# tychedelia/josefine

Hardware: NVIDIA H100
Metric: Raft-group ticks/sec @ 64Ki groups x 5 replicas (higher is better)
Workload: dtype u64

## Files before the change

josefine_b200/csrc/engine.cu:

```cuda
#include <algorithm>
#include <atomic>
#include <chrono>
#include <cstdarg>
#include <cstdio>
#include <cstdlib>
#include <cstring>
#include <condition_variable>
#include <mutex>
#include <new>
#include <thread>
#include <vector>

#include "raft_device.cuh"
#include "sym_fold.cuh"

using namespace jr;


#ifdef JR_EMU
#ifdef JR_EMU_BREAK_HANDOFF
#define JR_EMU_HANDOFF_ACQUIRE __ATOMIC_RELAXED
#define JR_EMU_HANDOFF_RELEASE __ATOMIC_RELAXED
#else
#define JR_EMU_HANDOFF_ACQUIRE __ATOMIC_ACQUIRE
// ... 1003 lines not shown
      if (last && id == last->id0 + last->count && addr == last->addr && last->count < FS_MAX_RUN &&
          (last->count == 1u || tok == last->tok0 + (unsigned long long)last->count * last->stride)) {
        if (last->count == 1u) last->stride = tok - last->tok0;
        last->count += 1u;
      } else {
        t[n++] = PnRun{id, 1u, addr, tok, 0ull};
        fit();
      }
    } else {
      while (a_e >= a_cnt && a_src <= d.R) {
        const uint32_t from = a_src < d.R ? a_src : r;
        if (a_k >= kept(from)) { ++a_src; a_k = 0; continue; }
        const uint4 h = rec_hdr(from, a_k++);
        if (mine(a_src, h)) { a_id0 = h.z; a_cnt = h.y >> 8; a_e = 0; }
      }
      if (a_e >= a_cnt) break;
      const uint32_t id = a_id0 + a_e++;
      if (id == 0u || skip) continue;
      const uint32_t k = find(id);
      if (k == n) continue;
      uint32_t addr;
      unsigned long long tok;
      take(k, id, addr, tok);
      if (o.count && id == o.id0 + o.count && addr == o.addr && o.count < FS_MAX_RUN &&
          (o.count == 1u || tok == o.tok0 + (unsigned long long)o.count * o.stride)) {
        if (o.count == 1u) o.stride = tok - o.tok0;
        o.count += 1u;
      } else {
        close();
        o = PnRun{id, 1u, addr, tok, 0ull};
      }
    }
  }
  close();
  for (uint32_t k = 0; k < n; ++k) {
    q.pn[(size_t)(2 * k) * plane + i] = make_uint4(t[k].id0, t[k].count, t[k].addr, 0u);
    q.pn[(size_t)(2 * k + 1) * plane + i] = make_uint4((uint32_t)t[k].tok0, (uint32_t)(t[k].tok0 >> 32), (uint32_t)t[k].stride,
                                                       (uint32_t)(t[k].stride >> 32));
  }
  q.pnc[i] = n;
  q.rc[i] = make_uint2(n_runs, n_resp);
  q.rd[i] = drop;
}

__global__ void fsm_copy_kernel(const uint4* __restrict__ src, const FsmHeader* __restrict__ hdr, uint4* __restrict__ dst,
                                FsmHeader* hdr_dst, uint32_t epoch) {
  const size_t n = (size_t)hdr->n_records * 2;
  for (size_t i = (size_t)blockIdx.x * blockDim.x + threadIdx.x; i < n; i += (size_t)gridDim.x * blockDim.x) dst[i] = src[i];
  if (blockIdx.x == 0 && threadIdx.x == 0) {
    FsmHeader h = *hdr;
    h.ready = epoch;
    *hdr_dst = h;
  }
}

__global__ void max_u32_kernel(const uint32_t* v, size_t n, uint32_t* out) {
  uint32_t m = 0;
  for (size_t i = (size_t)blockIdx.x * blockDim.x + threadIdx.x; i < n; i += (size_t)gridDim.x * blockDim.x)
    m = max(m, v[i]);
#ifndef JR_EMU
  for (int o = 16; o > 0; o >>= 1) m = max(m, __shfl_down_sync(0xffffffffu, m, o));
  if ((threadIdx.x & 31) == 0)
#endif
    atomicMax(out, m);
}


extern "C" { static jr_status stream_sums(jr_engine* e, uint64_t v[5]); }
static thread_local char g_err[512] = "";
static void set_err(const char* fmt, ...) {
  va_list ap;
  va_start(ap, fmt);
  vsnprintf(g_err, sizeof g_err, fmt, ap);
  va_end(ap);
}

#define CK(call)                                                                      \
  do {                                                                                \
    cudaError_t _e = (call);                                                          \
    if (_e != cudaSuccess) {                                                          \
      set_err("%s:%d %s: %s", __FILE__, __LINE__, #call, cudaGetErrorString(_e));     \
      return JR_E_CUDA;                                                               \
    }                                                                                 \
  } while (0)

struct jr_engine {
  jr_config cfg;
  Dev d;
  cudaStream_t stream = nullptr;
  cudaStream_t own_stream = nullptr;
  volatile uint32_t* h_scatter = nullptr;
  volatile uint32_t* h_unfolded = nullptr;
  uint32_t ticket_sum = 0;
  int force_sorted = 0;
  uint64_t launches_sorted = 0, launches_total = 0, launches_split = 0;
  uint32_t slots = 0;
  uint32_t sms = 0;
  uint32_t force_parts = 0;
  int cur = 0;
  uint64_t step_index = 0;
  std::vector<void*> allocs;
  unsigned long long* scratch = nullptr;
  jr_msg* inj_msgs = nullptr;
  uint4* inj_targets = nullptr;
  size_t inj_cap = 0;
  static constexpr int NBUF = JR_STAGING_DEPTH;
  jr_proposal* prop[NBUF] = {nullptr, nullptr};
  jr_leader_entry* leaders[NBUF] = {nullptr, nullptr};
  cudaStream_t h2d = nullptr, d2h = nullptr;
  cudaEvent_t prop_ready[NBUF] = {nullptr, nullptr};
  cudaEvent_t prop_free[NBUF] = {nullptr, nullptr};
  cudaEvent_t tab_ready[NBUF] = {nullptr, nullptr};
  cudaEvent_t tab_free[NBUF] = {nullptr, nullptr};
  bool prop_used[NBUF] = {false, false}, tab_used[NBUF] = {false, false};
  jr_proposal* batch[NBUF] = {nullptr, nullptr};
  size_t batch_cap[NBUF] = {0, 0};
  cudaEvent_t batch_ready[NBUF] = {nullptr, nullptr}, batch_free[NBUF] = {nullptr, nullptr};
  bool batch_used[NBUF] = {false, false};
  int batch_i = 0;
  unsigned long long* tokbuf[NBUF] = {nullptr, nullptr};
  size_t tok_cap[NBUF] = {0, 0};
  uint32_t* route = nullptr;
  int tab_pending[NBUF] = {0, 0};
  int tab_npending = 0;
  int prop_i = 0, tab_i = 0;
  void* many_buf = nullptr;
  size_t many_cap = 0;
  void* verify_buf = nullptr;
  size_t verify_cap = 0;
  static constexpr int NSLOT = NBUF + 1;
  unsigned long long* fsm_part = nullptr;
  uint32_t fsm_cap = 0;
  uint4* fsm_stage[NSLOT] = {};
  FsmHeader* fsm_stage_hdr[NSLOT] = {};
  uint4* fsm_host[NSLOT] = {};
  FsmHeader* fsm_host_hdr[NSLOT] = {};
  cudaEvent_t fsm_packed[NSLOT] = {};
  cudaEvent_t fsm_landed[NSLOT] = {};
  size_t fsm_copied[NSLOT] = {};
  size_t fsm_last_records = 0;
  int fsm_copy_by_sm = 0;
  bool fsm_used[NSLOT] = {};
  int fsm_i = 0, fsm_pending[NBUF] = {0, 0}, fsm_npending = 0;
  std::mutex qmu;
  uint32_t fsm_epoch = 0;
  RespPlanes rp = {nullptr, nullptr, nullptr, nullptr, nullptr, nullptr};
  uint32_t resp_cap = 0;
  size_t resp_copied[NSLOT] = {};
  size_t resp_last = 0;
  int resp_b = -1;
  uint8_t* symdone = nullptr;
  uint8_t* symblk = nullptr;
  uint32_t* symrec = nullptr;
  bool auto_trunc = false;
  uint32_t auto_trunc_margin = 0;
  int no_fold = 0;
  int no_parts_hint = 0;
  int sym_one_lane = 0;
  uint64_t launches_folded = 0;
  bool last_launch_folded = false;
};

template <typename T>
static jr_status dalloc(jr_engine* e, T** p, size_t n) {
  void* q = nullptr;
  cudaError_t err = cudaMalloc(&q, n * sizeof(T));
  if (err != cudaSuccess) {
    set_err("cudaMalloc(%zu bytes): %s", n * sizeof(T), cudaGetErrorString(err));
    return err == cudaErrorMemoryAllocation ? JR_E_NOMEM : JR_E_CUDA;
  }
  e->allocs.push_back(q);
  *p = (T*)q;
  return JR_OK;
}

#define DISPATCH_R(R_, CALL)           \
  switch (R_) {                        \
    case 1: { constexpr int RR = 1; CALL; } break; \
    case 2: { constexpr int RR = 2; CALL; } break; \
    case 3: { constexpr int RR = 3; CALL; } break; \
    case 4: { constexpr int RR = 4; CALL; } break; \
    case 5: { constexpr int RR = 5; CALL; } break; \
    case 6: { constexpr int RR = 6; CALL; } break; \
    case 7: { constexpr int RR = 7; CALL; } break; \
    default: { constexpr int RR = 8; CALL; } break; \
  }

template <int R>
static void launch_step_r(jr_engine* e, const StepParams& p, bool sorted, uint32_t grid, size_t smem) {
  auto kfn = sorted ? step_kernel<R, true> : step_kernel<R, false>;
  JR_LAUNCH_SMEM(kfn, grid, 32 * R, smem, e->stream, e->d, p);
}

template <int R>
static cudaError_t step_smem_attr_r(int smem) {
  cudaError_t a = cudaFuncSetAttribute(step_kernel<R, false>, cudaFuncAttributeMaxDynamicSharedMemorySize, smem);
  if (a != cudaSuccess) return a;
  return cudaFuncSetAttribute(step_kernel<R, true>, cudaFuncAttributeMaxDynamicSharedMemorySize, smem);
}

#ifndef JR_EMU
template <int R>
static cudaError_t step_occupancy_r(int* per_sm, int smem) {
  return cudaOccupancyMaxActiveBlocksPerMultiprocessor(per_sm, step_kernel<R, false>, 32 * R, (size_t)smem);
}
#endif

static size_t step_smem_bytes(const Dev& d) {
  return ((size_t)2 * d.Us + d.W) * d.R * 32 * sizeof(uint4) + (size_t)2 * d.R * 32 * sizeof(uint32_t) +
         (size_t)2 * d.R * d.R * 32 * sizeof(uint16_t);
}

static uint32_t choose_parts(const jr_engine* e, const StepParams& p, uint32_t n_blocks) {
  const uint32_t whole = PH_RESET_OUT | PH_DRAIN | PH_TICK;
  if ((p.phases & whole) != whole || p.n_ticks < 2) return 1;
  if (e->force_parts) return std::min<uint32_t>(e->force_parts, p.n_ticks);
  if (!e->slots || n_blocks <= e->slots) return 1;
  uint32_t best = 1;
  double best_rounds = (double)((n_blocks + e->slots - 1) / e->slots);
  for (uint32_t n = 2; n <= 8 && p.n_ticks / n >= 8; n *= 2) {
    const double rounds = (double)(((size_t)n_blocks * n + e->slots - 1) / e->slots) / n;
    if (rounds < best_rounds * 0.97) { best = n; best_rounds = rounds; }
  }
  return best;
}

static jr_status launch_step_once(jr_engine* e, const StepParams& p_in);

static jr_status launch_step(jr_engine* e, const StepParams& p_in) {
  const uint32_t limit = (e->d.flags & JR_F_CAPTURE_FSM) ? std::max(1u, e->d.Fr / 3u) : 0xffffffffu;
  if (p_in.n_ticks <= limit) return launch_step_once(e, p_in);
  StepParams p = p_in;
  for (uint32_t done = 0; done < p_in.n_ticks;) {
    p.n_ticks = std::min(limit, p_in.n_ticks - done);
    p.trunc = (p_in.trunc && done + p.n_ticks == p_in.n_ticks) ? 1u : 0u;
    jr_status st = launch_step_once(e, p);
    if (st != JR_OK) return st;
    done += p.n_ticks;
    p.now += (uint64_t)p.n_ticks * p.dt;
    p.step_index += p.n_ticks;
    p.cur ^= (int)(p.n_ticks & 1u);
    if (p.proposals) p.proposals += (size_t)p.n_ticks * p.prop_stride;
    p.tok_tick += p.n_ticks;
    p.phases = PH_RESET_OUT | PH_DRAIN | (p_in.phases & PH_PROPOSE) | PH_TICK;
  }
  return JR_OK;
}

template <int R>
static void launch_sym_r(jr_engine* e, const StepParams& p) {
  if constexpr (R >= 2) {
    JR_LAUNCH(sym_check_kernel<R>, (e->d.Gp + SYM_CHECK_THREADS - 1) / SYM_CHECK_THREADS, SYM_CHECK_THREADS, e->stream, e->d, p,
              e->symrec);
    if (e->sym_one_lane)
      JR_LAUNCH(sym_kernel<R>, (e->d.Gp + SYM_LANES - 1) / SYM_LANES, SYM_LANES, e->stream, e->d, p, e->symdone, e->symrec);
    else
      JR_LAUNCH_SMEM(sym2_kernel<R>, (e->d.Gp + SYM2_GROUPS - 1) / SYM2_GROUPS, 2 * SYM2_GROUPS,
                     (size_t)SYM2_UNITS * SYM2_GROUPS * sizeof(uint4), e->stream, e->d, p, e->symdone, e->symblk, e->symrec);
  }
}

static bool fold_eligible(const jr_engine* e, const StepParams& p) {
  const Dev& d = e->d;
  const uint32_t whole = PH_RESET_OUT | PH_DRAIN | PH_TICK;
  if (e->no_fold || (d.flags & (JR_F_STREAM_DIGEST | JR_F_SLED_COMMIT_KEY_STRICT | JR_F_NO_SYMMETRIC_FOLD))) return false;
  if (d.R < 2 || d.U < d.R + 7 || d.resident != 0xffu || p.dt == 0) return false;
  if ((p.phases & ~(uint32_t)PH_PROPOSE) != whole || p.n_ticks < 2) return false;
  if (p.proposals && p.prop_stride != d.G) return false;
  return true;
}

static jr_status launch_step_once(jr_engine* e, const StepParams& p_in) {
  const uint32_t n_blocks = e->d.Gp / GROUPS_PER_CTA;
  const size_t smem = step_smem_bytes(e->d);
  StepParams p = p_in;
  p.epoch = (uint32_t)(e->launches_total + 1) * 8u;
  if (fold_eligible(e, p)) {
    DISPATCH_R(e->cfg.n_replicas, (launch_sym_r<RR>(e, p)));
    CK(cudaGetLastError());
    if (e->sym_one_lane) {
      JR_LAUNCH(sym_blocks_kernel, (n_blocks + 127) / 128, 128, e->stream, e->symdone, e->symblk, n_blocks);
      CK(cudaGetLastError());
    }
    p.symdone = e->symdone;
    p.symblk = e->symblk;
    e->launches_folded += 1;
  }
  e->last_launch_folded = p.symdone != nullptr;
  p.n_parts = choose_parts(e, p, n_blocks);
  if (p.symdone && !e->sym_one_lane && e->h_unfolded && (*e->h_unfolded == 0 || p.epoch - *e->h_unfolded > 2u * 8u) && !e->force_parts)
    if (!e->no_parts_hint) p.n_parts = 1;
  p.part_ticks = (p.n_ticks + p.n_parts - 1) / p.n_parts;
  p.n_parts = (p.n_ticks + p.part_ticks - 1) / p.part_ticks;
  p.n_blocks = n_blocks;
  const uint32_t grid = n_blocks * p.n_parts;
  const bool sorted = e->force_sorted > 0 || (e->force_sorted == 0 && e->h_scatter && *e->h_scatter != 0 && p.epoch - *e->h_scatter <= 2u * 8u);
  p.ticket_base = e->ticket_sum;
  if (p.n_parts > 1) e->ticket_sum += grid;
  DISPATCH_R(e->cfg.n_replicas, (launch_step_r<RR>(e, p, sorted, grid, smem)));
  CK(cudaGetLastError());
  if (p.trunc) {
    JR_LAUNCH(truncate_kernel, (e->d.Gp + 127) / 128, 128, e->stream, e->d, p.trunc_margin,
              (const uint8_t*)((p.symdone && !e->sym_one_lane) ? p.symdone : nullptr));
    CK(cudaGetLastError());
  }
  e->launches_sorted += sorted ? 1 : 0;
  e->launches_split += p.n_parts > 1 ? 1 : 0;
  e->launches_total += 1;
  return JR_OK;
}

extern "C" {

#ifdef JR_EMU
int jr_is_emulation(void) { return 1; }
#endif

const char* jr_last_error(void) { return g_err; }

void jr_config_default(jr_config* cfg, uint32_t n_groups, uint32_t n_replicas) {
  if (!cfg) return;
  memset(cfg, 0, sizeof *cfg);
  cfg->abi_version = JR_ABI_VERSION;
  cfg->n_groups = n_groups;
  cfg->n_replicas = n_replicas;
  cfg->election_min_ms = 500;
  cfg->election_max_ms = 1000;
  cfg->heartbeat_ms = 100;
  cfg->chain_capacity = 4096;
  cfg->mailbox_units = 64;
  cfg->fsm_units = 64;
}

uint32_t jr_election_timeout(uint64_t seed, uint64_t group, uint32_t node, uint32_t draw, uint32_t mn,
                             uint32_t mx) {
  return election_timeout_draw(seed, group, node, draw, mn, mx);
}

jr_status jr_engine_create(const jr_config* cfg, jr_engine** out) {
  if (!cfg || !out) return JR_E_INVAL;
  if (cfg->abi_version != JR_ABI_VERSION) { set_err("abi_version mismatch"); return JR_E_INVAL; }
  if (cfg->n_replicas < 1 || cfg->n_replicas > JR_MAX_REPLICAS || cfg->n_groups < 1) { set_err("bad G/R"); return JR_E_INVAL; }
  if (cfg->election_max_ms <= cfg->election_min_ms) { set_err("empty election timeout range"); return JR_E_INVAL; }
  if (cfg->heartbeat_ms < 5) { set_err("heartbeat timeout is too low"); return JR_E_INVAL; }
  if (cfg->election_min_ms < 5) { set_err("election timeout is too low"); return JR_E_INVAL; }
  if (cfg->chain_capacity < 2 || cfg->chain_capacity > 0x40000000u) { set_err("chain_capacity out of range"); return JR_E_INVAL; }
  if (cfg->mailbox_units < 8 || cfg->fsm_units < 1) { set_err("mailbox_units >= 8, fsm_units >= 1"); return JR_E_INVAL; }
  if (cfg->fsm_units > (1u << 20) || cfg->fsm_raw_units > (1u << 20) || (cfg->fsm_raw_units && cfg->fsm_raw_units < 32)) {
    set_err("fsm_units <= 2^20, 32 <= fsm_raw_units <= 2^20");
    return JR_E_INVAL;
  }
  if ((cfg->flags & JR_F_CLIENT_RESPONSES) && !(cfg->flags & JR_F_CAPTURE_FSM)) {
    set_err("JR_F_CLIENT_RESPONSES requires JR_F_CAPTURE_FSM");
    return JR_E_INVAL;
  }
  int ndev = 0;
  if (cudaGetDeviceCount(&ndev) != cudaSuccess || ndev == 0) {
    set_err("no CUDA device; this library has no CPU fallback");
    return JR_E_NO_DEVICE;
  }
  if (cfg->device < 0 || cfg->device >= ndev) { set_err("device ordinal %d out of range", cfg->device); return JR_E_INVAL; }
  CK(cudaSetDevice(cfg->device));
  jr_engine* e = new (std::nothrow) jr_engine();
  if (!e) return JR_E_NOMEM;
  e->cfg = *cfg;
  Dev& d = e->d;
  memset(&d, 0, sizeof d);
  d.G = cfg->n_groups;
  d.Gp = (cfg->n_groups + GROUPS_PER_CTA - 1) / GROUPS_PER_CTA * GROUPS_PER_CTA;
  d.R = cfg->n_replicas;
  d.cap = cfg->chain_capacity;
  d.capm = 1;
  while (d.capm < d.cap) d.capm <<= 1;
  d.capm -= 1;
  d.U = cfg->mailbox_units;
  d.F = cfg->fsm_units;
  d.Fr = cfg->fsm_raw_units ? cfg->fsm_raw_units : 192u;
  d.flags = cfg->flags;
  d.emin = cfg->election_min_ms;
  d.emax = cfg->election_max_ms;
  d.hb = cfg->heartbeat_ms;
  d.seed = cfg->seed;
  d.goff = cfg->group_offset;
  d.Us = std::min<uint32_t>(cfg->mailbox_units, 6u);
  d.W = 4;
  d.use_index = getenv("JR_NO_INDEX") ? 0u : 1u;
  d.resident = cfg->resident_mask ? cfg->resident_mask : 0xffu;
  if (const char* ev = getenv("JR_SMEM_UNITS")) d.Us = std::min<uint32_t>(cfg->mailbox_units, (uint32_t)atoi(ev));
  if (const char* ev = getenv("JR_TABLE_CACHE")) { uint32_t w = (uint32_t)atoi(ev); d.W = (w & (w - 1)) ? 8 : w; }
  const size_t plane = (size_t)d.R * d.Gp;
  jr_status st = JR_OK;
#define A(ptr, n) if (st == JR_OK) st = dalloc(e, &(ptr), (n))
  A(d.p0, plane); A(d.p1, plane); A(d.p2, plane); A(d.p3, plane);
  A(d.pr, plane * ((d.R + 3) / 4));
  A(d.mk, plane);
  A(d.qt, plane * JR_CLIENT_QUEUE_CAP);
  A(d.dg, plane); A(d.cn, plane);
  A(d.cnext, plane * ((size_t)d.capm + 1));
  A(d.ctok, plane * ((size_t)d.capm + 1));
  A(d.ob[0], plane * (size_t)d.U); A(d.ob[1], plane * (size_t)d.U);
  A(d.oc[0], plane); A(d.oc[1], plane);
  A(d.fs, plane * (size_t)((d.flags & JR_F_CAPTURE_FSM) ? 2 * (size_t)d.F : 1));
  A(d.fc, plane);
  A(d.fq, plane);
  A(d.fr, plane * (size_t)((d.flags & JR_F_CAPTURE_FSM) ? d.Fr : 1));
  A(d.tb, d.Gp);
  A(e->symdone, d.Gp);
  A(e->symblk, d.Gp / GROUPS_PER_CTA);
  A(e->symrec, (size_t)sym_record_words(d.R) * d.Gp);
  if (d.flags & JR_F_CAPTURE_FSM) {
    const size_t reps = (size_t)cfg->n_groups * cfg->n_replicas;
    const size_t want = cfg->fsm_host_records ? cfg->fsm_host_records
                                              : std::max(3 * reps + 1024, std::min<size_t>(reps * cfg->fsm_units, 1u << 16));
    e->fsm_cap = (uint32_t)std::min<size_t>(want, 0x7fffffffu);
    if (d.flags & JR_F_CLIENT_RESPONSES) {
      e->resp_cap = e->fsm_cap;
      uint4* pn = nullptr;
      A(pn, pn_units(plane));
      e->rp.pn = pn;
      if (pn) {
        e->rp.pnc = reinterpret_cast<uint32_t*>(pn + 2 * (size_t)JR_NOTIFY_RUNS * plane);
        e->rp.rm = pn + 2 * (size_t)JR_NOTIFY_RUNS * plane + (plane + 3) / 4;
      }
      A(e->rp.rs, plane * 2 * (size_t)d.F);
      A(e->rp.rc, plane);
      A(e->rp.rd, plane);
    }
    const size_t n_hdr = e->resp_cap ? 2 : 1;
    A(e->fsm_part, 3 * plane);
    for (int i = 0; i < jr_engine::NSLOT; ++i) {
      A(e->fsm_stage[i], 2 * ((size_t)e->fsm_cap + e->resp_cap));
      A(e->fsm_stage_hdr[i], n_hdr);
    }
  }
  A(e->scratch, 8);
  A(d.scatter, 2);
  A(d.done, d.Gp / GROUPS_PER_CTA);
#ifdef JR_PROFILE
  A(d.prof, 3 * 16 * 2);
#endif
  for (int i = 0; i < jr_engine::NBUF; ++i) { A(e->prop[i], d.G); A(e->leaders[i], d.G); }
  A(e->route, d.G);
#undef A
  if (st != JR_OK) { jr_engine_destroy(e); return st; }
  if (cudaStreamCreateWithFlags(&e->own_stream, cudaStreamNonBlocking) != cudaSuccess) {
    set_err("cudaStreamCreate failed");
    jr_engine_destroy(e);
    return JR_E_CUDA;
  }
  e->stream = e->own_stream;
  {
    bool ok = cudaStreamCreateWithFlags(&e->h2d, cudaStreamNonBlocking) == cudaSuccess &&
              cudaStreamCreateWithFlags(&e->d2h, cudaStreamNonBlocking) == cudaSuccess;
    for (int i = 0; ok && i < jr_engine::NBUF; ++i)
      ok = cudaEventCreateWithFlags(&e->prop_ready[i], cudaEventDisableTiming) == cudaSuccess &&
           cudaEventCreateWithFlags(&e->prop_free[i], cudaEventDisableTiming) == cudaSuccess &&
           cudaEventCreateWithFlags(&e->tab_ready[i], cudaEventDisableTiming) == cudaSuccess &&
           cudaEventCreateWithFlags(&e->tab_free[i], cudaEventDisableTiming) == cudaSuccess &&
           cudaEventCreateWithFlags(&e->batch_ready[i], cudaEventDisableTiming) == cudaSuccess &&
           cudaEventCreateWithFlags(&e->batch_free[i], cudaEventDisableTiming) == cudaSuccess;
    for (int i = 0; ok && i < jr_engine::NSLOT; ++i)
      ok = cudaEventCreateWithFlags(&e->fsm_packed[i], cudaEventDisableTiming) == cudaSuccess &&
           cudaEventCreateWithFlags(&e->fsm_landed[i], cudaEventDisableTiming) == cudaSuccess;
    for (int i = 0; ok && e->fsm_cap && i < jr_engine::NSLOT; ++i)
      ok = cudaHostAlloc((void**)&e->fsm_host[i], ((size_t)e->fsm_cap + e->resp_cap) * sizeof(jr_fsm_record), cudaHostAllocMapped) == cudaSuccess &&
           cudaHostAlloc((void**)&e->fsm_host_hdr[i], (e->resp_cap ? 2 : 1) * sizeof(FsmHeader), cudaHostAllocMapped) == cudaSuccess;
    if (!ok) {
      set_err("copy streams / events could not be created");
      jr_engine_destroy(e);
      return JR_E_CUDA;
    }
  }
  {
    const int smem = (int)step_smem_bytes(d);
    cudaError_t aerr = cudaSuccess;
    DISPATCH_R(d.R, (aerr = step_smem_attr_r<RR>(smem)));
    if (aerr == cudaSuccess) aerr = cudaHostAlloc((void**)&e->h_scatter, sizeof(uint32_t), cudaHostAllocMapped);
    if (aerr == cudaSuccess) *e->h_scatter = 0;
    if (aerr == cudaSuccess) aerr = cudaHostGetDevicePointer((void**)&e->d.hscat, (void*)e->h_scatter, 0);
    if (aerr == cudaSuccess) aerr = cudaHostAlloc((void**)&e->h_unfolded, sizeof(uint32_t), cudaHostAllocMapped);
    if (aerr == cudaSuccess) *e->h_unfolded = 0;
    if (aerr == cudaSuccess) aerr = cudaHostGetDevicePointer((void**)&e->d.hunf, (void*)e->h_unfolded, 0);
    if (const char* ev = getenv("JR_NO_FOLD")) e->no_fold = atoi(ev);
    if (const char* ev = getenv("JR_SYM_ONE_LANE")) e->sym_one_lane = atoi(ev);
    if (const char* ev = getenv("JR_NO_PARTS_HINT")) e->no_parts_hint = atoi(ev);
    if (const char* ev = getenv("JR_FSM_COPY")) e->fsm_copy_by_sm = strcmp(ev, "sm") == 0;
    if (const char* ev = getenv("JR_PARTS")) e->force_parts = (uint32_t)std::min(std::max(atoi(ev), 0), 8);
#ifndef JR_EMU
    if (aerr == cudaSuccess) {
      int per_sm = 0, sms = 0;
      DISPATCH_R(d.R, (aerr = step_occupancy_r<RR>(&per_sm, smem)));
      if (aerr == cudaSuccess) aerr = cudaDeviceGetAttribute(&sms, cudaDevAttrMultiProcessorCount, cfg->device);
      e->slots = (uint32_t)(per_sm * sms);
      e->sms = (uint32_t)sms;
    }
#endif
    if (const char* ev = getenv("JR_STEP_VARIANT")) e->force_sorted = !strcmp(ev, "sorted") ? 1 : (!strcmp(ev, "plain") ? -1 : 0);
    if (aerr != cudaSuccess) {
      set_err("step kernel needs %d bytes of shared memory: %s", smem, cudaGetErrorString(aerr));
      jr_engine_destroy(e);
      return JR_E_CUDA;
    }
  }
  if (jr_engine_reset(e) != JR_OK) {
    jr_engine_destroy(e);
    return JR_E_CUDA;
  }
  *out = e;
  return JR_OK;
}

#ifdef JR_PROFILE
jr_status jr_profile_read(jr_engine* e, unsigned long long* out96) {
  if (!e || !out96) return JR_E_INVAL;
  CK(cudaStreamSynchronize(e->stream));
  CK(cudaMemcpyAsync(out96, e->d.prof, 96 * sizeof(unsigned long long), cudaMemcpyDeviceToHost, e->stream));
  CK(cudaMemsetAsync(e->d.prof, 0, 96 * sizeof(unsigned long long), e->stream));
  CK(cudaStreamSynchronize(e->stream));
  return JR_OK;
}
#endif

jr_status jr_engine_reset(jr_engine* e) {
  if (!e) return JR_E_INVAL;
  CK(cudaSetDevice(e->cfg.device));
  const Dev& d = e->d;
  const size_t plane = (size_t)d.R * d.Gp;
  CK(cudaMemsetAsync(d.cnext, 0xFF, plane * ((size_t)d.capm + 1) * sizeof(uint32_t), e->stream));
  CK(cudaMemsetAsync(d.pr, 0, plane * ((d.R + 3) / 4) * sizeof(uint4), e->stream));
  CK(cudaMemsetAsync(d.qt, 0, plane * JR_CLIENT_QUEUE_CAP * sizeof(uint4), e->stream));
  CK(cudaMemsetAsync(e->route, 0, (size_t)d.G * sizeof(uint32_t), e->stream));
  CK(cudaMemsetAsync(d.done, 0, (size_t)(d.Gp / GROUPS_PER_CTA) * sizeof(uint32_t), e->stream));
  CK(cudaMemsetAsync(d.scatter, 0, 2 * sizeof(uint32_t), e->stream));
  e->ticket_sum = 0;
  if (e->rp.pnc)
    CK(cudaMemsetAsync(e->rp.pnc, 0, ((plane + 3) / 4 + plane) * sizeof(uint4), e->stream));
  e->resp_b = -1;
  JR_LAUNCH(init_kernel, (unsigned)((plane + 255) / 256), 256, e->stream, d);
  CK(cudaGetLastError());
  CK(cudaStreamSynchronize(e->stream));
  e->cur = 0;
  e->step_index = 0;
#ifdef JR_PROFILE
  CK(cudaMemsetAsync(e->d.prof, 0, 96 * sizeof(unsigned long long), e->stream));
#endif
  return JR_OK;
}

void jr_engine_destroy(jr_engine* e) {
  if (!e) return;
  if (getenv("JR_DEBUG_VARIANT"))
    fprintf(stderr, "[jr] engine %p: %llu step launches, %llu role-sorted, %llu split, %llu offered to the fold; %u CTA slots\n",
            (void*)e, (unsigned long long)e->launches_total, (unsigned long long)e->launches_sorted,
            (unsigned long long)e->launches_split, (unsigned long long)e->launches_folded, e->slots);
  cudaSetDevice(e->cfg.device);
  if (e->stream) cudaStreamSynchronize(e->stream);
  for (void* p : e->allocs) cudaFree(p);
  if (e->inj_msgs) cudaFree(e->inj_msgs);
  if (e->inj_targets) cudaFree(e->inj_targets);
  if (e->many_buf) cudaFree(e->many_buf);
  if (e->verify_buf) cudaFree(e->verify_buf);
  if (e->h2d) { cudaStreamSynchronize(e->h2d); cudaStreamDestroy(e->h2d); }
  if (e->d2h) { cudaStreamSynchronize(e->d2h); cudaStreamDestroy(e->d2h); }
  for (int i = 0; i < jr_engine::NBUF; ++i) {
    if (e->prop_ready[i]) cudaEventDestroy(e->prop_ready[i]);
    if (e->prop_free[i]) cudaEventDestroy(e->prop_free[i]);
    if (e->tab_ready[i]) cudaEventDestroy(e->tab_ready[i]);
    if (e->tab_free[i]) cudaEventDestroy(e->tab_free[i]);
    if (e->batch_ready[i]) cudaEventDestroy(e->batch_ready[i]);
    if (e->batch_free[i]) cudaEventDestroy(e->batch_free[i]);
    if (e->batch[i]) cudaFree(e->batch[i]);
    if (e->tokbuf[i]) cudaFree(e->tokbuf[i]);
  }
  for (int i = 0; i < jr_engine::NSLOT; ++i) {
    if (e->fsm_packed[i]) cudaEventDestroy(e->fsm_packed[i]);
    if (e->fsm_landed[i]) cudaEventDestroy(e->fsm_landed[i]);
    if (e->fsm_host[i]) cudaFreeHost(e->fsm_host[i]);
    if (e->fsm_host_hdr[i]) cudaFreeHost(e->fsm_host_hdr[i]);
  }
  if (e->h_scatter) cudaFreeHost((void*)e->h_scatter);
  if (e->h_unfolded) cudaFreeHost((void*)e->h_unfolded);
  if (e->own_stream) cudaStreamDestroy(e->own_stream);
  delete e;
}

jr_status jr_engine_set_stream(jr_engine* e, void* s) {
  if (!e) return JR_E_INVAL;
  CK(cudaStreamSynchronize(e->stream));
  e->stream = s ? (cudaStream_t)s : e->own_stream;
  return JR_OK;
}

jr_status jr_engine_sync(jr_engine* e) {
  if (!e) return JR_E_INVAL;
  CK(cudaStreamSynchronize(e->h2d));
  CK(cudaStreamSynchronize(e->stream));
  CK(cudaStreamSynchronize(e->d2h));
  return JR_OK;
}


static void decode_unit(const uint4& h, uint32_t group, uint32_t sender, const uint4* blocks, size_t stride,
                        std::vector<jr_msg>& out) {
  const uint32_t kind = h.x & 15u, flag = (h.x >> 4) & 1u, aux = (h.x >> 8) & 255u, to = h.x >> 16;
  jr_msg m;
  memset(&m, 0, sizeof m);
  m.group = group;
  m.from_kind = JR_ADDR_PEER;
  m.from_id = sender;
  m.to_kind = to == TO_PEERS ? JR_ADDR_PEERS : (to == TO_CLIENT ? JR_ADDR_CLIENT : JR_ADDR_PEER);
  m.to_id = m.to_kind == JR_ADDR_PEER ? to : 0;
  m.kind = (uint8_t)kind;
  const uint64_t t = (uint64_t)h.y | ((uint64_t)h.z << 32);
  uint32_t copies = 1;
  switch (kind) {
    case JR_CMD_VOTE_REQUEST: m.term = t; m.node_id = sender; m.last_term = t; m.block = h.w; copies = aux; break;
    case JR_CMD_VOTE_RESPONSE: m.term = t; m.node_id = sender; m.flag = flag; break;
    case JR_CMD_APPEND_ENTRIES:
      m.term = t; m.node_id = sender; m.n_blocks = (uint8_t)aux;
      for (uint32_t k = 0; k < aux && k < JR_MAX_AE_BLOCKS; ++k) {
        const uint4& b = blocks[(size_t)k * stride];
        m.blocks[k] = jr_block{b.x, b.y, (uint64_t)b.z | ((uint64_t)b.w << 32)};
      }
      break;
    case JR_CMD_APPEND_RESPONSE: m.node_id = sender; m.term = t; m.block = h.w; m.flag = flag; break;
    case JR_CMD_HEARTBEAT: m.term = t; m.block = h.w; m.node_id = sender; break;
    case JR_CMD_HEARTBEAT_RESPONSE: m.block = h.w; m.flag = flag; break;
    case JR_CMD_CLIENT_REQUEST: m.token = t; m.client_kind = (uint8_t)(h.w >> 16); m.client_id = h.w & 0xffffu; break;
    case JR_CMD_CLIENT_RESPONSE: m.token = t; break;
    default: break;
  }
  for (uint32_t k = 0; k < copies; ++k) out.push_back(m);
}

static jr_status device_max(jr_engine* e, const uint32_t* v, size_t n, uint32_t* out) {
  uint32_t* s = reinterpret_cast<uint32_t*>(e->scratch);
  CK(cudaMemsetAsync(s, 0, sizeof(uint32_t), e->stream));
  JR_LAUNCH(max_u32_kernel, 64, 256, e->stream, v, n, s);
  CK(cudaGetLastError());
  CK(cudaMemcpyAsync(out, s, sizeof(uint32_t), cudaMemcpyDeviceToHost, e->stream));
  CK(cudaStreamSynchronize(e->stream));
  return JR_OK;
}

static jr_status capture_messages(jr_engine* e, int buf, std::vector<jr_msg>& out) {
  const Dev& d = e->d;
  const size_t plane = (size_t)d.R * d.Gp;
  uint32_t mx = 0;
  jr_status st = device_max(e, d.oc[buf], plane, &mx);
  if (st != JR_OK) return st;
  std::vector<uint32_t> cnt(plane);
  CK(cudaMemcpyAsync(cnt.data(), d.oc[buf], plane * sizeof(uint32_t), cudaMemcpyDeviceToHost, e->stream));
  std::vector<uint4> units((size_t)mx * plane);
  if (mx) CK(cudaMemcpyAsync(units.data(), d.ob[buf], units.size() * sizeof(uint4), cudaMemcpyDeviceToHost, e->stream));
  CK(cudaStreamSynchronize(e->stream));
  for (uint32_t g = 0; g < d.G; ++g)
    for (uint32_t r = 0; r < d.R; ++r) {
      const size_t i = (size_t)r * d.Gp + g;
      for (uint32_t u = 0; u < cnt[i];) {
        const uint4& h = units[(size_t)u * plane + i];
        const uint32_t kind = h.x & 15u, aux = (h.x >> 8) & 255u;
        const bool ae = kind == JR_CMD_APPEND_ENTRIES, ref = ae && ((h.x >> 4) & 1u);
        const uint32_t span = 1 + ((ae && !ref) ? aux : 0u);
        const uint32_t first = ref ? h.w : u + 1;
        decode_unit(h, g, r + 1, (ae && aux) ? &units[(size_t)first * plane + i] : nullptr, plane, out);
        u += span;
      }
    }
  return JR_OK;
}


static jr_status fsm_records_enqueue(jr_engine* e) {
  const Dev& d = e->d;
  if (!(d.flags & JR_F_CAPTURE_FSM)) { set_err("engine created without JR_F_CAPTURE_FSM"); return JR_E_INVAL; }
  size_t last_records, last_resp;
  {
    std::lock_guard<std::mutex> l(e->qmu);
    if (e->fsm_npending == jr_engine::NBUF) { set_err("%d batches outstanding: call jr_fsm_records_wait first", jr_engine::NBUF); return JR_E_INVAL; }
    last_records = e->fsm_last_records;
    last_resp = e->resp_last;
  }
  const int b = e->fsm_i;
  e->fsm_i = (b + 1) % jr_engine::NSLOT;
  const size_t plane = (size_t)d.R * d.Gp;
  if (e->fsm_used[b]) CK(cudaStreamWaitEvent(e->stream, e->fsm_landed[b], 0));
  const uint32_t epoch = ++e->fsm_epoch;
#ifdef JR_EMU
  const uint32_t T = 1, Ts = 1;
#else
  const uint32_t T = 256, Ts = SCAN_THREADS;
#endif
  const uint32_t n_ctas = (uint32_t)((plane + T - 1) / T);
  JR_LAUNCH(fsm_count_kernel, n_ctas, T, e->stream, d, d.fc, nullptr, e->fsm_part, n_ctas);
  CK(cudaGetLastError());
  JR_LAUNCH(fsm_scan_kernel, 1, Ts, e->stream, e->fsm_part, n_ctas, e->fsm_stage_hdr[b], e->fsm_cap, false);
  CK(cudaGetLastError());
  if (e->resp_cap) {
    JR_LAUNCH(fsm_respond_kernel, n_ctas, T, e->stream, d, e->rp, e->fsm_stage_hdr[b], e->fsm_cap);
    CK(cudaGetLastError());
  }
  JR_LAUNCH(fsm_pack_kernel, n_ctas, T, e->stream, d, d.fs, d.fc, e->fsm_part, e->fsm_stage_hdr[b], e->fsm_stage[b], e->fsm_cap,
            false);
  CK(cudaGetLastError());
  uint4* const resp_stage = e->fsm_stage[b] + 2 * (size_t)e->fsm_cap;
  if (e->resp_cap) {
    JR_LAUNCH(fsm_count_kernel, n_ctas, T, e->stream, d, e->rp.rc, e->rp.rd, e->fsm_part, n_ctas);
    CK(cudaGetLastError());
    JR_LAUNCH(fsm_scan_kernel, 1, Ts, e->stream, e->fsm_part, n_ctas, e->fsm_stage_hdr[b] + 1, e->resp_cap, true);
    CK(cudaGetLastError());
    JR_LAUNCH(fsm_pack_kernel, n_ctas, T, e->stream, d, e->rp.rs, e->rp.rc, e->fsm_part, e->fsm_stage_hdr[b] + 1, resp_stage,
              e->resp_cap, true);
    CK(cudaGetLastError());
  }
  CK(cudaEventRecord(e->fsm_packed[b], e->stream));
  CK(cudaStreamWaitEvent(e->d2h, e->fsm_packed[b], 0));
  if (e->fsm_copy_by_sm) {
    JR_LAUNCH(fsm_copy_kernel, 32, 256, e->d2h, e->fsm_stage[b], e->fsm_stage_hdr[b], e->fsm_host[b], e->fsm_host_hdr[b], epoch);
    CK(cudaGetLastError());
    e->fsm_copied[b] = e->fsm_cap;
    if (e->resp_cap) {
      JR_LAUNCH(fsm_copy_kernel, 32, 256, e->d2h, resp_stage, e->fsm_stage_hdr[b] + 1, e->fsm_host[b] + 2 * (size_t)e->fsm_cap,
                e->fsm_host_hdr[b] + 1, epoch);
      CK(cudaGetLastError());
      e->resp_copied[b] = e->resp_cap;
    }
  } else {
    const size_t guess = std::min<size_t>(e->fsm_cap, std::max<size_t>(last_records + last_records / 8 + 1024, 16384));
    if (guess) CK(cudaMemcpyAsync(e->fsm_host[b], e->fsm_stage[b], guess * sizeof(jr_fsm_record), cudaMemcpyDeviceToHost, e->d2h));
    CK(cudaMemcpyAsync(e->fsm_host_hdr[b], e->fsm_stage_hdr[b], sizeof(FsmHeader), cudaMemcpyDeviceToHost, e->d2h));
    e->fsm_copied[b] = guess;
    if (e->resp_cap) {
      const size_t rg = std::min<size_t>(e->resp_cap, std::max<size_t>(last_resp + last_resp / 8 + 1024, 16384));
      CK(cudaMemcpyAsync(e->fsm_host[b] + 2 * (size_t)e->fsm_cap, resp_stage, rg * sizeof(jr_fsm_record), cudaMemcpyDeviceToHost, e->d2h));
      CK(cudaMemcpyAsync(e->fsm_host_hdr[b] + 1, e->fsm_stage_hdr[b] + 1, sizeof(FsmHeader), cudaMemcpyDeviceToHost, e->d2h));
      e->resp_copied[b] = rg;
    }
  }
  CK(cudaEventRecord(e->fsm_landed[b], e->d2h));
  e->fsm_used[b] = true;
  std::lock_guard<std::mutex> l(e->qmu);
  e->fsm_pending[e->fsm_npending++] = b;
  return JR_OK;
}

static jr_status fsm_records_take(jr_engine* e, const jr_fsm_record** recs, jr_fsm_batch* batch) {
  int b;
  {
    std::lock_guard<std::mutex> l(e->qmu);
    if (e->fsm_npending == 0) { set_err("no batch outstanding"); return JR_E_INVAL; }
    b = e->fsm_pending[0];
    for (int k = 0; k + 1 < jr_engine::NBUF; ++k) e->fsm_pending[k] = e->fsm_pending[k + 1];
    --e->fsm_npending;
  }
  CK(cudaEventSynchronize(e->fsm_landed[b]));
  const FsmHeader& h = *e->fsm_host_hdr[b];
  if (h.n_records > e->fsm_copied[b]) {
    const size_t have = e->fsm_copied[b];
    CK(cudaMemcpyAsync(reinterpret_cast<jr_fsm_record*>(e->fsm_host[b]) + have, reinterpret_cast<const jr_fsm_record*>(e->fsm_stage[b]) + have,
                       ((size_t)h.n_records - have) * sizeof(jr_fsm_record), cudaMemcpyDeviceToHost, e->d2h));
    CK(cudaEventRecord(e->fsm_landed[b], e->d2h));
    CK(cudaEventSynchronize(e->fsm_landed[b]));
    e->fsm_copied[b] = h.n_records;
  }
  size_t n_resp = 0;
  if (e->resp_cap) {
    const FsmHeader& hr = e->fsm_host_hdr[b][1];
    n_resp = hr.n_records;
    if (hr.n_records > e->resp_copied[b]) {
      const size_t have = e->resp_copied[b];
      jr_fsm_record* dst = reinterpret_cast<jr_fsm_record*>(e->fsm_host[b] + 2 * (size_t)e->fsm_cap);
      const jr_fsm_record* src = reinterpret_cast<const jr_fsm_record*>(e->fsm_stage[b] + 2 * (size_t)e->fsm_cap);
      CK(cudaMemcpyAsync(dst + have, src + have, ((size_t)hr.n_records - have) * sizeof(jr_fsm_record), cudaMemcpyDeviceToHost, e->d2h));
      CK(cudaEventRecord(e->fsm_landed[b], e->d2h));
      CK(cudaEventSynchronize(e->fsm_landed[b]));
      e->resp_copied[b] = hr.n_records;
    }
  }
  {
    std::lock_guard<std::mutex> l(e->qmu);
    e->fsm_last_records = h.n_records;
    if (e->resp_cap) { e->resp_last = n_resp; e->resp_b = b; }
  }
  if (recs) *recs = reinterpret_cast<const jr_fsm_record*>(e->fsm_host[b]);
  if (batch) {
    memset(batch, 0, sizeof *batch);
    batch->n_records = h.n_records;
    batch->n_dropped = h.n_dropped;
    batch->n_instructions = h.n_instructions;
    for (uint32_t r = 0; r <= JR_MAX_REPLICAS; ++r) batch->node_offset[r] = r <= e->d.R ? h.node_offset[r] : h.node_offset[e->d.R];
  }
  if (h.n_dropped) {
    set_err("%llu Instruction records were dropped (raise fsm_units / fsm_host_records, or drain more often)",
            (unsigned long long)h.n_dropped);
    return JR_E_CAPACITY;
  }
  return JR_OK;
}

static jr_status capture_fsm(jr_engine* e, std::vector<jr_fsm_instr>& out) {
  const Dev& d = e->d;
  if (!(d.flags & JR_F_CAPTURE_FSM)) return JR_OK;
  if (e->fsm_npending) { set_err("jr_fsm_records_async batches are outstanding"); return JR_E_INVAL; }
  jr_status st = fsm_records_enqueue(e);
  if (st != JR_OK) return st;
  const jr_fsm_record* recs = nullptr;
  jr_fsm_batch batch;
  const jr_status took = fsm_records_take(e, &recs, &batch);
  if (took != JR_OK) return took;
  size_t n = 0;
  st = jr_fsm_expand(recs, batch.n_records, d.G, d.R, nullptr, 0, &n);
  if (st != JR_OK && st != JR_E_CAPACITY) return st;
  out.resize(n);
  if (n && (st = jr_fsm_expand(recs, batch.n_records, d.G, d.R, out.data(), n, &n)) != JR_OK) return st;
  return took;
}


jr_status jr_step(jr_engine* e, jr_step_args* a) {
  if (!e || !a) return JR_E_INVAL;
  CK(cudaSetDevice(e->cfg.device));
  const Dev& d = e->d;
  const uint32_t R = d.R, G = d.G;
  if (a->n_synth > 8) { set_err("n_synth <= 8"); return JR_E_INVAL; }
  if ((a->out_msgs && !(d.flags & JR_F_CAPTURE_MESSAGES)) || (a->out_fsm && !(d.flags & JR_F_CAPTURE_FSM))) {
    set_err("output buffer given but capture flag not set at create");
    return JR_E_INVAL;
  }
  std::vector<jr_msg> sorted;
  std::vector<uint4> targets;
  if (a->n_inject) {
    if (!a->inject) return JR_E_INVAL;
    std::vector<uint32_t> order(a->n_inject);
    for (size_t i = 0; i < a->n_inject; ++i) {
      const jr_msg& m = a->inject[i];
      if (m.group >= G || m.to_kind != JR_ADDR_PEER) { set_err("inject[%zu]: bad group / to_kind", i); return JR_E_INVAL; }
      if (m.to_id < 1 || m.to_id > R) return JR_E_UNKNOWN_NODE;
      if (m.node_id > JR_MAX_NODE_ID || m.from_id > JR_MAX_NODE_ID || m.client_id > JR_MAX_NODE_ID) return JR_E_INVAL;
      if (m.kind == JR_CMD_VOTE_RESPONSE && (m.node_id < 1 || m.node_id > 32)) return JR_E_UNKNOWN_NODE;
      if (m.n_blocks > JR_MAX_AE_BLOCKS) return JR_E_INVAL;
      if (m.block >= 0xffffffffull) { set_err("inject[%zu]: block id >= 2^32-1 (D4)", i); return JR_E_INVAL; }
      for (unsigned k = 0; k < m.n_blocks; ++k)
        if (m.blocks[k].id >= 0xffffffffull || m.blocks[k].next >= 0xffffffffull) return JR_E_INVAL;
      order[i] = (uint32_t)i;
    }
    std::stable_sort(order.begin(), order.end(), [&](uint32_t x, uint32_t y) {
      const jr_msg &p = a->inject[x], &q = a->inject[y];
      return p.group != q.group ? p.group < q.group : p.to_id < q.to_id;
    });
    sorted.reserve(a->n_inject);
    for (uint32_t idx : order) {
      const jr_msg& m = a->inject[idx];
      if (targets.empty() || targets.back().x != m.group || targets.back().y != m.to_id - 1)
        targets.push_back(make_uint4(m.group, m.to_id - 1, (uint32_t)sorted.size(), 0));
      targets.back().w++;
      sorted.push_back(m);
    }
  }
  if (a->proposals && !(a->flags & JR_STEP_TRUSTED_PROPOSALS))
    for (uint32_t g = 0; g < G; ++g)
      if (a->proposals[g].node > R) return JR_E_UNKNOWN_NODE;

  StepParams p;
  p.now = a->now_ms;
  p.step_index = e->step_index;
  p.n_synth = (a->flags & JR_STEP_SYNTH_PROPOSALS) ? a->n_synth : 0;
  p.cur = e->cur;
  p.n_ticks = 1;
  p.dt = 0;
  p.prop_stride = 0;
  p.proposals = nullptr;
  int staged = -1;
  if (a->proposals) {
    const int b = e->prop_i;
    e->prop_i = (b + 1) % jr_engine::NBUF;
    if (e->prop_used[b]) CK(cudaStreamWaitEvent(e->h2d, e->prop_free[b], 0));
    CK(cudaMemcpyAsync(e->prop[b], a->proposals, (size_t)G * sizeof(jr_proposal), cudaMemcpyHostToDevice, e->h2d));
    CK(cudaEventRecord(e->prop_ready[b], e->h2d));
    CK(cudaStreamWaitEvent(e->stream, e->prop_ready[b], 0));
    p.proposals = e->prop[b];
    staged = b;
  }
  if (e->rp.rm) {
    const size_t plane = (size_t)R * d.Gp;
    JR_LAUNCH(restart_marks_rebase_kernel, (unsigned)((plane + 255) / 256), 256, e->stream, d, e->rp.rm);
    CK(cudaGetLastError());
  }
  const uint32_t ph_first = PH_RESET_OUT | PH_RESET_FSM | ((a->flags & JR_STEP_DELIVER) ? PH_DRAIN : 0u);
  const uint32_t ph_last = ((p.proposals || p.n_synth) ? PH_PROPOSE : 0u) | ((a->flags & JR_STEP_TICK) ? PH_TICK : 0u);
  jr_status st;
  if (targets.empty()) {
    p.phases = ph_first | ph_last;
    if ((st = launch_step(e, p)) != JR_OK) return st;
  } else {
    if (sorted.size() > e->inj_cap) {
      if (e->inj_msgs) cudaFree(e->inj_msgs);
      if (e->inj_targets) cudaFree(e->inj_targets);
      e->inj_msgs = nullptr; e->inj_targets = nullptr;
      e->inj_cap = std::max<size_t>(sorted.size() * 2, 64);
      CK(cudaMalloc(&e->inj_msgs, e->inj_cap * sizeof(jr_msg)));
      CK(cudaMalloc(&e->inj_targets, e->inj_cap * sizeof(uint4)));
    }
    CK(cudaMemcpyAsync(e->inj_msgs, sorted.data(), sorted.size() * sizeof(jr_msg), cudaMemcpyHostToDevice, e->stream));
    CK(cudaMemcpyAsync(e->inj_targets, targets.data(), targets.size() * sizeof(uint4), cudaMemcpyHostToDevice, e->stream));
    p.phases = ph_first;
    if ((st = launch_step(e, p)) != JR_OK) return st;
    const uint32_t nt = (uint32_t)targets.size();
    DISPATCH_R(R, (JR_LAUNCH(inject_kernel<RR>, (nt + 63) / 64, 64, e->stream, e->d, p, e->inj_msgs, e->inj_targets, nt)));
    CK(cudaGetLastError());
    if (ph_last) {
      p.phases = ph_last;
      if ((st = launch_step(e, p)) != JR_OK) return st;
    }
    CK(cudaStreamSynchronize(e->stream));
  }
  if (staged >= 0) {
    CK(cudaEventRecord(e->prop_free[staged], e->stream));
    e->prop_used[staged] = true;
    CK(cudaEventSynchronize(e->prop_ready[staged]));
  }
  const int written = e->cur;
  e->cur ^= 1;
  e->step_index++;

  a->n_msgs = 0;
  a->n_fsm = 0;
  bool ovf = false;
  if (a->out_msgs) {
    std::vector<jr_msg> msgs;
    if ((st = capture_messages(e, written, msgs)) != JR_OK) return st;
    a->n_msgs = msgs.size();
    memcpy(a->out_msgs, msgs.data(), std::min(msgs.size(), a->cap_msgs) * sizeof(jr_msg));
    ovf |= msgs.size() > a->cap_msgs;
  }
  if (a->out_fsm) {
    std::vector<jr_fsm_instr> fsm;
    st = capture_fsm(e, fsm);
    if (st != JR_OK && st != JR_E_CAPACITY) return st;
    a->n_fsm = fsm.size();
    memcpy(a->out_fsm, fsm.data(), std::min(fsm.size(), a->cap_fsm) * sizeof(jr_fsm_instr));
    ovf |= fsm.size() > a->cap_fsm || st == JR_E_CAPACITY;
  }
  if (a->flags & JR_STEP_REPORT_FAULTS) {
    uint64_t v[5];
    if ((st = stream_sums(e, v)) != JR_OK) return st;
    a->n_faulted = v[4];
  }
  return ovf ? JR_E_CAPACITY : JR_OK;
}

jr_status jr_run(jr_engine* e, uint64_t now0, uint32_t dt, uint32_t n_steps, uint32_t n_synth) {
  if (!e) return JR_E_INVAL;
  if (n_synth > 8) { set_err("n_synth <= 8"); return JR_E_INVAL; }
  CK(cudaSetDevice(e->cfg.device));
  if (n_steps == 0) return JR_OK;
  StepParams p;
  p.now = now0;
  p.step_index = e->step_index;
  p.n_synth = n_synth;
  p.n_ticks = n_steps;
  p.dt = dt;
  p.cur = e->cur;
  p.proposals = nullptr;
  p.prop_stride = 0;
  p.phases = PH_RESET_OUT | PH_DRAIN | (n_synth ? PH_PROPOSE : 0u) | PH_TICK;
  p.trunc = e->auto_trunc ? 1u : 0u;
  p.trunc_margin = e->auto_trunc_margin;
  jr_status st = launch_step(e, p);
  if (st != JR_OK) return st;
  e->cur ^= (int)(n_steps & 1u);
  e->step_index += n_steps;
  return JR_OK;
}

static jr_status batch_reserve(jr_engine* e, int b, size_t n) {
  if (e->batch_used[b]) CK(cudaStreamWaitEvent(e->h2d, e->batch_free[b], 0));
  if (n > e->batch_cap[b]) {
    if (e->batch_used[b]) CK(cudaEventSynchronize(e->batch_free[b]));
    if (e->batch[b]) cudaFree(e->batch[b]);
    e->batch[b] = nullptr;
    e->batch_cap[b] = 0;
    CK(cudaMalloc(&e->batch[b], n * sizeof(jr_proposal)));
    e->batch_cap[b] = n;
  }
  return JR_OK;
}

static jr_status batch_launch(jr_engine* e, int b, uint64_t now0, uint32_t dt, uint32_t n_steps) {
  StepParams p;
  p.now = now0;
  p.step_index = e->step_index;
  p.n_synth = 0;
  p.n_ticks = n_steps;
  p.dt = dt;
  p.cur = e->cur;
  p.proposals = e->batch[b];
  p.prop_stride = e->d.G;
  p.phases = PH_RESET_OUT | PH_DRAIN | PH_PROPOSE | PH_TICK;
  p.trunc = e->auto_trunc ? 1u : 0u;
  p.trunc_margin = e->auto_trunc_margin;
  jr_status st = launch_step(e, p);
  if (st != JR_OK) return st;
  CK(cudaEventRecord(e->batch_free[b], e->stream));
  e->batch_used[b] = true;
  e->cur ^= (int)(n_steps & 1u);
  e->step_index += n_steps;
  return JR_OK;
}

jr_status jr_run_proposals(jr_engine* e, uint64_t now0, uint32_t dt, uint32_t n_steps, const jr_proposal* proposals,
                           uint32_t flags) {
  if (!e || !proposals) return JR_E_INVAL;
  if (n_steps == 0) return JR_OK;
  CK(cudaSetDevice(e->cfg.device));
  const uint32_t G = e->d.G, R = e->d.R;
  const size_t n = (size_t)n_steps * G;
  if (!(flags & JR_STEP_TRUSTED_PROPOSALS))
    for (size_t i = 0; i < n; ++i)
      if (proposals[i].node > R) return JR_E_UNKNOWN_NODE;
  const int b = e->batch_i;
  e->batch_i = (b + 1) % jr_engine::NBUF;
  jr_status st = batch_reserve(e, b, n);
  if (st != JR_OK) return st;
  CK(cudaMemcpyAsync(e->batch[b], proposals, n * sizeof(jr_proposal), cudaMemcpyHostToDevice, e->h2d));
  CK(cudaEventRecord(e->batch_ready[b], e->h2d));
  CK(cudaStreamWaitEvent(e->stream, e->batch_ready[b], 0));
  return batch_launch(e, b, now0, dt, n_steps);
}

jr_status jr_run_tokens(jr_engine* e, uint64_t now0, uint32_t dt, uint32_t n_steps, const uint64_t* tokens) {
  if (!e || !tokens) return JR_E_INVAL;
  if (n_steps == 0) return JR_OK;
  CK(cudaSetDevice(e->cfg.device));
  const uint32_t G = e->d.G;
  const size_t n = (size_t)n_steps * G;
  const int b = e->batch_i;
  e->batch_i = (b + 1) % jr_engine::NBUF;
  jr_status st = batch_reserve(e, b, n);
  if (st != JR_OK) return st;
  if (n > e->tok_cap[b]) {
    if (e->batch_used[b]) CK(cudaEventSynchronize(e->batch_free[b]));
    if (e->tokbuf[b]) cudaFree(e->tokbuf[b]);
    e->tokbuf[b] = nullptr;
    e->tok_cap[b] = 0;
    CK(cudaMalloc(&e->tokbuf[b], n * sizeof(unsigned long long)));
    e->tok_cap[b] = n;
  }
  CK(cudaMemcpyAsync(e->tokbuf[b], tokens, n * sizeof(unsigned long long), cudaMemcpyHostToDevice, e->h2d));
  CK(cudaEventRecord(e->batch_ready[b], e->h2d));
  CK(cudaStreamWaitEvent(e->stream, e->batch_ready[b], 0));
  const unsigned blocks = (unsigned)std::min<size_t>((n + 255) / 256, (size_t)std::max(e->sms, 1u) * 16);
  JR_LAUNCH(route_tokens_kernel, blocks, 256, e->stream, e->tokbuf[b], e->route, e->batch[b], G, n);
  CK(cudaGetLastError());
  return batch_launch(e, b, now0, dt, n_steps);
}

jr_status jr_run_token_runs(jr_engine* e, uint64_t now0, uint32_t dt, uint32_t n_steps, const jr_token_run* runs) {
  if (!e || !runs) return JR_E_INVAL;
  if (n_steps == 0) return JR_OK;
  CK(cudaSetDevice(e->cfg.device));
  const uint32_t G = e->d.G;
  const int b = e->batch_i;
  e->batch_i = (b + 1) % jr_engine::NBUF;
  jr_status st = batch_reserve(e, b, G);
  if (st != JR_OK) return st;
  CK(cudaMemcpyAsync(e->batch[b], runs, (size_t)G * sizeof(jr_token_run), cudaMemcpyHostToDevice, e->h2d));
  CK(cudaEventRecord(e->batch_ready[b], e->h2d));
  CK(cudaStreamWaitEvent(e->stream, e->batch_ready[b], 0));
  StepParams p;
  p.now = now0;
  p.step_index = e->step_index;
  p.n_synth = 0;
  p.n_ticks = n_steps;
  p.dt = dt;
  p.cur = e->cur;
  p.proposals = nullptr;
  p.prop_stride = 0;
  p.tok_runs = reinterpret_cast<const uint4*>(e->batch[b]);
  p.tok_route = e->route;
  p.tok_tick = 0;
  p.phases = PH_RESET_OUT | PH_DRAIN | PH_PROPOSE | PH_TICK;
  p.trunc = e->auto_trunc ? 1u : 0u;
  p.trunc_margin = e->auto_trunc_margin;
  st = launch_step(e, p);
  if (st != JR_OK) return st;
  CK(cudaEventRecord(e->batch_free[b], e->stream));
  e->batch_used[b] = true;
  e->cur ^= (int)(n_steps & 1u);
  e->step_index += n_steps;
  return JR_OK;
}

jr_status jr_drain_fsm(jr_engine* e, jr_fsm_instr* out, size_t cap, size_t* n) {
  if (!e || !n) return JR_E_INVAL;
  CK(cudaSetDevice(e->cfg.device));
  if (!(e->d.flags & JR_F_CAPTURE_FSM)) { *n = 0; return JR_OK; }
  std::vector<jr_fsm_instr> fsm;
  jr_status st = capture_fsm(e, fsm);
  if (st != JR_OK && st != JR_E_CAPACITY) return st;
  *n = fsm.size();
  if (out) memcpy(out, fsm.data(), std::min(fsm.size(), cap) * sizeof(jr_fsm_instr));
  return ((out && fsm.size() > cap) || st == JR_E_CAPACITY) ? JR_E_CAPACITY : JR_OK;
}

jr_status jr_fsm_fold(const jr_fsm_record* recs, size_t n, uint32_t G, uint32_t R, uint32_t* applied_hi, uint64_t* totals) {
  if ((!recs && n) || !applied_hi || !totals || R < 1 || R > JR_MAX_REPLICAS) return JR_E_INVAL;
  uint64_t na = 0, nn = 0;
  for (size_t i = 0; i < n; ++i) {
    const jr_fsm_record& rc = recs[i];
    const uint32_t kind = JR_FSMR_KIND(rc.hdr), node = JR_FSMR_NODE(rc.hdr), count = JR_FSMR_COUNT(rc.hdr);
    if (rc.group >= G || node > R) return JR_E_INVAL;
    if (kind == JR_FSMR_APPLY) {
      if (rc.addr) {
        if (rc.addr >> R) return JR_E_INVAL;
        for (uint32_t n = 0; n < R; ++n)
          if ((rc.addr >> n) & 1u) {
            uint32_t& hi = applied_hi[(size_t)n * G + rc.group];
            hi = std::max(hi, rc.id0 + count - 1);
            na += count;
          }
      } else {
        uint32_t& hi = applied_hi[(size_t)(node - 1) * G + rc.group];
        hi = std::max(hi, rc.id0 + count - 1);
        na += count;
      }
    } else if (kind == JR_FSMR_NOTIFY) {
      nn += count;
    }
  }
  totals[0] += na;
  totals[1] += nn;
  totals[2] += n;
  return JR_OK;
}

namespace {
struct FoldJob {
  const jr_fsm_record* recs = nullptr;
  size_t n = 0;
  uint32_t G = 0, R = 0, parts = 0;
  uint32_t* applied = nullptr;
  size_t sec[JR_MAX_REPLICAS + 1];
  uint64_t na[64], nn[64];
  int bad[64];
};
inline uint64_t rec_key(const jr_fsm_record& rc) { return ((uint64_t)JR_FSMR_NODE(rc.hdr) << 32) | rc.group; }
size_t lower_bound_key(const jr_fsm_record* recs, size_t lo, size_t hi, uint64_t key) {
  while (lo < hi) {
    const size_t mid = lo + (hi - lo) / 2;
    if (rec_key(recs[mid]) < key) lo = mid + 1;
    else hi = mid;
  }
  return lo;
}
void fold_slice(FoldJob& j, uint32_t t) {
  const uint32_t g_lo = (uint32_t)((uint64_t)j.G * t / j.parts), g_hi = (uint32_t)((uint64_t)j.G * (t + 1) / j.parts);
  uint64_t na = 0, nn = 0;
  for (uint32_t node = 1; node <= j.R; ++node) {
    const size_t lo = lower_bound_key(j.recs, j.sec[node - 1], j.sec[node], ((uint64_t)node << 32) | g_lo);
    const size_t hi = lower_bound_key(j.recs, lo, j.sec[node], ((uint64_t)node << 32) | g_hi);
    for (size_t i = lo; i < hi; ++i) {
      const jr_fsm_record& rc = j.recs[i];
      const uint32_t kind = JR_FSMR_KIND(rc.hdr), count = JR_FSMR_COUNT(rc.hdr);
      if (kind == JR_FSMR_APPLY) {
        if (rc.addr) {
          if (rc.addr >> j.R) { j.bad[t] = 1; return; }
          for (uint32_t k = 0; k < j.R; ++k)
            if ((rc.addr >> k) & 1u) {
              uint32_t& hi_w = j.applied[(size_t)k * j.G + rc.group];
              hi_w = std::max(hi_w, rc.id0 + count - 1);
              na += count;
            }
        } else {
          uint32_t& hi_w = j.applied[(size_t)(node - 1) * j.G + rc.group];
          hi_w = std::max(hi_w, rc.id0 + count - 1);
          na += count;
        }
      } else if (kind == JR_FSMR_NOTIFY) {
        nn += count;
      }
    }
  }
  j.na[t] = na;
  j.nn[t] = nn;
}
class FoldPool {
  static constexpr long long SPIN_NS = 2'000'000;
 public:
  static FoldPool& get() { static FoldPool* p = new FoldPool(); return *p; }
  void run(FoldJob& j) {
    {
      std::lock_guard<std::mutex> l(m_);
      while (n_workers_ + 1 < j.parts) {
        const uint32_t k = n_workers_++;
        std::thread th([this, k] { loop(k); });
        th.detach();
      }
      job_ = &j;
      left_.store(j.parts - 1, std::memory_order_relaxed);
      state_.store(((state_.load(std::memory_order_relaxed) >> 8) + 1) << 8 | j.parts, std::memory_order_release);
    }
    if (sleepers_.load(std::memory_order_acquire)) cv_.notify_all();
    fold_slice(j, 0);
    const auto t0 = std::chrono::steady_clock::now();
    while (left_.load(std::memory_order_acquire) != 0) {
      if (std::chrono::steady_clock::now() - t0 > std::chrono::nanoseconds(SPIN_NS)) {
        std::unique_lock<std::mutex> l(m_);
        done_.wait(l, [this] { return left_.load(std::memory_order_acquire) == 0; });
        break;
      }
      cpu_relax();
    }
  }
 private:
  static void cpu_relax() {
#if defined(__x86_64__) || defined(__i386__)
    __builtin_ia32_pause();
#endif
  }
  void loop(uint32_t k) {
    uint64_t seen = 0;
    for (;;) {
      uint64_t st = state_.load(std::memory_order_acquire);
      const auto t0 = std::chrono::steady_clock::now();
      while ((st >> 8) == seen) {
        if (std::chrono::steady_clock::now() - t0 > std::chrono::nanoseconds(SPIN_NS)) {
          std::unique_lock<std::mutex> l(m_);
          sleepers_.fetch_add(1, std::memory_order_acq_rel);
          cv_.wait(l, [&] { return (state_.load(std::memory_order_acquire) >> 8) != seen; });
          sleepers_.fetch_sub(1, std::memory_order_acq_rel);
        } else {
          cpu_relax();
        }
        st = state_.load(std::memory_order_acquire);
      }
      seen = st >> 8;
      if (k + 1 >= (uint32_t)(st & 255u)) continue;
      fold_slice(*job_, k + 1);
      if (left_.fetch_sub(1, std::memory_order_acq_rel) == 1) {
        std::lock_guard<std::mutex> l(m_);
        done_.notify_all();
      }
    }
  }
  std::mutex m_;
  std::condition_variable cv_, done_;
  uint32_t n_workers_ = 0;
  FoldJob* job_ = nullptr;
  std::atomic<uint32_t> left_{0}, sleepers_{0};
  std::atomic<uint64_t> state_{0};
};
}

jr_status jr_fsm_fold_mt(const jr_fsm_record* recs, size_t n, uint32_t G, uint32_t R, uint32_t* applied_hi, uint64_t* totals,
                         uint32_t n_threads) {
  if (n_threads <= 1 || n < 4096) return jr_fsm_fold(recs, n, G, R, applied_hi, totals);
  if ((!recs && n) || !applied_hi || !totals || R < 1 || R > JR_MAX_REPLICAS) return JR_E_INVAL;
  FoldJob j;
  j.recs = recs; j.n = n; j.G = G; j.R = R; j.applied = applied_hi;
  j.parts = std::min<uint32_t>(n_threads, 64);
  j.sec[0] = 0;
  for (uint32_t node = 1; node <= R; ++node) j.sec[node] = lower_bound_key(recs, j.sec[node - 1], n, (uint64_t)(node + 1) << 32);
  bool sorted = j.sec[R] == n && recs[n - 1].group < G;
  for (size_t probe = 1; sorted && probe < 64; ++probe) {
    const size_t i = n * probe / 64;
    sorted = i == 0 || rec_key(recs[i - 1]) <= rec_key(recs[i]);
  }
  if (!sorted) return jr_fsm_fold(recs, n, G, R, applied_hi, totals);
  static std::mutex* one_at_a_time = new std::mutex();
  std::lock_guard<std::mutex> guard(*one_at_a_time);
  for (uint32_t t = 0; t < j.parts; ++t) { j.na[t] = j.nn[t] = 0; j.bad[t] = 0; }
  FoldPool::get().run(j);
  for (uint32_t t = 0; t < j.parts; ++t) {
    if (j.bad[t]) return JR_E_INVAL;
    totals[0] += j.na[t];
    totals[1] += j.nn[t];
  }
  totals[2] += n;
  return JR_OK;
}

jr_status jr_fsm_records_async(jr_engine* e) {
  if (!e) return JR_E_INVAL;
  CK(cudaSetDevice(e->cfg.device));
  return fsm_records_enqueue(e);
}

jr_status jr_fsm_records_wait(jr_engine* e, const jr_fsm_record** records, jr_fsm_batch* batch) {
  if (!e) return JR_E_INVAL;
  CK(cudaSetDevice(e->cfg.device));
  return fsm_records_take(e, records, batch);
}

jr_status jr_fsm_responses(jr_engine* e, const jr_fsm_record** responses, jr_fsm_batch* batch) {
  if (!e) return JR_E_INVAL;
  if (!e->resp_cap) { set_err("engine created without JR_F_CLIENT_RESPONSES"); return JR_E_INVAL; }
  int b;
  { std::lock_guard<std::mutex> l(e->qmu); b = e->resp_b; }
  if (b < 0) { set_err("no batch has been taken yet"); return JR_E_INVAL; }
  const FsmHeader& h = e->fsm_host_hdr[b][1];
  if (responses) *responses = reinterpret_cast<const jr_fsm_record*>(e->fsm_host[b] + 2 * (size_t)e->fsm_cap);
  if (batch) {
    memset(batch, 0, sizeof *batch);
    batch->n_records = h.n_records;
    batch->n_dropped = h.n_dropped;
    batch->n_instructions = h.n_instructions;
    for (uint32_t r = 0; r <= JR_MAX_REPLICAS; ++r) batch->node_offset[r] = r <= e->d.R ? h.node_offset[r] : h.node_offset[e->d.R];
  }
  if (h.n_dropped) {
    set_err("%llu notifications / responses were dropped (JR_NOTIFY_RUNS, fsm_units or lost records)", (unsigned long long)h.n_dropped);
    return JR_E_CAPACITY;
  }
  return JR_OK;
}

jr_status jr_fsm_expand(const jr_fsm_record* recs, size_t n_records, uint32_t G, uint32_t R, jr_fsm_instr* out, size_t cap,
                        size_t* n_out) {
  if (!n_out || (!recs && n_records) || R < 1 || R > JR_MAX_REPLICAS || G < 1) return JR_E_INVAL;
  const size_t nb = (size_t)G * R;
  std::vector<uint32_t> start(nb + 1, 0u);
  auto masked = [&](const jr_fsm_record& rc) { return JR_FSMR_KIND(rc.hdr) == JR_FSMR_APPLY && rc.addr != 0; };
  for (size_t i = 0; i < n_records; ++i) {
    const uint32_t node = JR_FSMR_NODE(recs[i].hdr);
    if (recs[i].group >= G || node > R || JR_FSMR_KIND(recs[i].hdr) > JR_FSMR_PATTERN) return JR_E_INVAL;
    if (masked(recs[i])) {
      if (recs[i].addr >> R) return JR_E_INVAL;
      for (uint32_t n = 0; n < R; ++n)
        if ((recs[i].addr >> n) & 1u) ++start[(size_t)recs[i].group * R + n + 1];
    } else {
      ++start[(size_t)recs[i].group * R + (node - 1) + 1];
    }
  }
  for (size_t b = 0; b < nb; ++b) start[b + 1] += start[b];
  std::vector<uint32_t> order(start[nb]), fill(start.begin(), start.end() - 1);
  for (int pass = 0; pass < 2; ++pass)
    for (size_t i = 0; i < n_records; ++i) {
      if (masked(recs[i]) != (pass == 0)) continue;
      if (pass == 0) {
        for (uint32_t n = 0; n < R; ++n)
          if ((recs[i].addr >> n) & 1u) order[fill[(size_t)recs[i].group * R + n]++] = (uint32_t)i;
      } else {
        order[fill[(size_t)recs[i].group * R + (JR_FSMR_NODE(recs[i].hdr) - 1)]++] = (uint32_t)i;
      }
    }
  size_t k = 0;
  std::vector<uint64_t> is_notify;
  for (size_t b = 0; b < nb; ++b) {
    const uint32_t lo = start[b], hi = start[b + 1];
    if (lo == hi) continue;
    const uint32_t g = (uint32_t)(b / R), node = (uint32_t)(b % R) + 1;
    size_t n_apply = 0, n_note = 0;
    for (uint32_t j = lo; j < hi; ++j) {
      const jr_fsm_record& rc = recs[order[j]];
      if (JR_FSMR_KIND(rc.hdr) == JR_FSMR_APPLY) n_apply += JR_FSMR_COUNT(rc.hdr);
      else if (JR_FSMR_KIND(rc.hdr) == JR_FSMR_NOTIFY) n_note += JR_FSMR_COUNT(rc.hdr);
    }
    const size_t total = n_apply + n_note;
    is_notify.assign((total + 63) / 64, 0ull);
    size_t marked = 0;
    for (uint32_t j = lo; j < hi; ++j) {
      const jr_fsm_record& rc = recs[order[j]];
      if (JR_FSMR_KIND(rc.hdr) != JR_FSMR_PATTERN) continue;
      const uint32_t nbits = JR_FSMR_COUNT(rc.hdr);
      if (nbits > 160) return JR_E_INVAL;
      for (uint32_t bit = 0; bit < nbits; ++bit)
        if ((bit < 64 ? rc.tok0 >> bit : bit < 128 ? rc.stride >> (bit - 64) : (uint64_t)rc.addr >> (bit - 128)) & 1ull) {
          const size_t pos = (size_t)rc.id0 + bit;
          if (pos >= total || ((is_notify[pos >> 6] >> (pos & 63)) & 1ull)) return JR_E_INVAL;
          is_notify[pos >> 6] |= 1ull << (pos & 63);
          ++marked;
        }
    }
    if (marked != n_note) return JR_E_INVAL;
    uint32_t ja = lo, jn = lo, ia = 0, in_ = 0;
    for (size_t pos = 0; pos < total; ++pos) {
      const bool note = (is_notify[pos >> 6] >> (pos & 63)) & 1ull;
      uint32_t& j = note ? jn : ja;
      uint32_t& i = note ? in_ : ia;
      const uint32_t want = note ? JR_FSMR_NOTIFY : JR_FSMR_APPLY;
      while (JR_FSMR_KIND(recs[order[j]].hdr) != want || i >= JR_FSMR_COUNT(recs[order[j]].hdr)) { ++j; i = 0; }
      const jr_fsm_record& rc = recs[order[j]];
      if (out && k < cap) {
        jr_fsm_instr f;
        memset(&f, 0, sizeof f);
        f.group = g;
        f.node = node;
        if (note) {
          f.kind = JR_FSM_NOTIFY;
          f.client_kind = (uint8_t)(rc.addr >> 16);
          f.client_id = rc.addr & 0xffffu;
          f.block = jr_block{(uint64_t)(rc.id0 + i), 0, rc.tok0 + (uint64_t)i * rc.stride};
        } else {
          f.kind = JR_FSM_APPLY;
          const uint32_t bid = rc.id0 + i;
          if (JR_FSMR_COUNT(rc.hdr) == 1) f.block = jr_block{bid, (uint32_t)rc.stride, rc.tok0};
          else f.block = jr_block{bid, bid - 1u, rc.tok0 + (uint64_t)i * rc.stride};
        }
        out[k] = f;
      }
      ++k;
      ++i;
    }
  }
  *n_out = k;
  return (out && k > cap) || (!out && k) ? JR_E_CAPACITY : JR_OK;
}


static jr_status scratch_reserve(void** buf, size_t* cap, size_t bytes) {
  if (bytes <= *cap) return JR_OK;
  if (*buf) cudaFree(*buf);
  *buf = nullptr;
  *cap = 0;
  const size_t want = std::max<size_t>(bytes * 2, 4096);
  CK(cudaMalloc(buf, want));
  *cap = want;
  return JR_OK;
}

static jr_status many_reserve(jr_engine* e, size_t bytes) { return scratch_reserve(&e->many_buf, &e->many_cap, bytes); }

jr_status jr_query_many(jr_engine* e, const uint32_t* groups, const uint32_t* nodes, size_t n, jr_replica_state* out) {
  if (!e || !out || !groups || !nodes) return JR_E_INVAL;
  if (n == 0) return JR_OK;
  if (n > 0x7fffffffu) return JR_E_INVAL;
  for (size_t i = 0; i < n; ++i)
    if (groups[i] >= e->d.G || nodes[i] < 1 || nodes[i] > e->d.R) return JR_E_INVAL;
  CK(cudaSetDevice(e->cfg.device));
  const size_t idx = ((n * 2 * sizeof(uint32_t)) + 15) / 16 * 16;
  jr_status st = many_reserve(e, idx + n * sizeof(jr_replica_state));
  if (st != JR_OK) return st;
  uint32_t* dg = (uint32_t*)e->many_buf;
  uint32_t* dn = dg + n;
  jr_replica_state* ds = (jr_replica_state*)((char*)e->many_buf + idx);
  CK(cudaMemcpyAsync(dg, groups, n * sizeof(uint32_t), cudaMemcpyHostToDevice, e->stream));
  CK(cudaMemcpyAsync(dn, nodes, n * sizeof(uint32_t), cudaMemcpyHostToDevice, e->stream));
  JR_LAUNCH(query_kernel, (unsigned)((n + 127) / 128), 128, e->stream, e->d, dg, dn, (uint32_t)n, ds);
  CK(cudaGetLastError());
  CK(cudaMemcpyAsync(out, ds, n * sizeof(jr_replica_state), cudaMemcpyDeviceToHost, e->stream));
  CK(cudaStreamSynchronize(e->stream));
  return JR_OK;
}

jr_status jr_query(jr_engine* e, uint32_t group, uint32_t node, jr_replica_state* out) {
  return jr_query_many(e, &group, &node, 1, out);
}

jr_status jr_chain_read_many(jr_engine* e, const uint32_t* groups, const uint32_t* nodes, const uint64_t* first_id,
                             const uint32_t* count, size_t n, jr_block* out, uint8_t* present) {
  if (!e || !groups || !nodes || !first_id || !count) return JR_E_INVAL;
  if (n == 0) return JR_OK;
  if (n > 0x7fffffffu) return JR_E_INVAL;
  std::vector<uint4> reqs(n);
  size_t total = 0;
  for (size_t i = 0; i < n; ++i) {
    if (groups[i] >= e->d.G || nodes[i] < 1 || nodes[i] > e->d.R) return JR_E_INVAL;
    if (first_id[i] + count[i] > 0xffffffffull) return JR_E_INVAL;
    reqs[i] = make_uint4(groups[i], nodes[i] - 1, (uint32_t)first_id[i], (uint32_t)total);
    total += count[i];
    if (total > 0xffffffffull) return JR_E_INVAL;
  }
  if (total == 0) return JR_OK;
  CK(cudaSetDevice(e->cfg.device));
  const size_t o_cnt = n * sizeof(uint4), o_blk = (o_cnt + n * sizeof(uint32_t) + 15) / 16 * 16;
  const size_t o_pre = o_blk + total * sizeof(jr_block);
  jr_status st = many_reserve(e, o_pre + total);
  if (st != JR_OK) return st;
  char* base = (char*)e->many_buf;
  CK(cudaMemcpyAsync(base, reqs.data(), n * sizeof(uint4), cudaMemcpyHostToDevice, e->stream));
  CK(cudaMemcpyAsync(base + o_cnt, count, n * sizeof(uint32_t), cudaMemcpyHostToDevice, e->stream));
  JR_LAUNCH(chain_read_kernel, (unsigned)n, 128, e->stream, e->d, (const uint4*)base, (const uint32_t*)(base + o_cnt),
            (jr_block*)(base + o_blk), (uint8_t*)(base + o_pre));
  CK(cudaGetLastError());
  if (out) CK(cudaMemcpyAsync(out, base + o_blk, total * sizeof(jr_block), cudaMemcpyDeviceToHost, e->stream));
  if (present) CK(cudaMemcpyAsync(present, base + o_pre, total, cudaMemcpyDeviceToHost, e->stream));
  CK(cudaStreamSynchronize(e->stream));
  return JR_OK;
}

jr_status jr_chain_read(jr_engine* e, uint32_t group, uint32_t node, uint64_t first, uint32_t n, jr_block* out,
                        uint8_t* present) {
  if (n == 0) return (!e || group >= e->d.G || node < 1 || node > e->d.R) ? JR_E_INVAL : JR_OK;
  return jr_chain_read_many(e, &group, &node, &first, &n, 1, out, present);
}

jr_status jr_state_digest(jr_engine* e, uint64_t* out) {
  if (!e || !out) return JR_E_INVAL;
  CK(cudaSetDevice(e->cfg.device));
  const size_t plane = (size_t)e->d.R * e->d.Gp;
  CK(cudaMemsetAsync(e->scratch, 0, 8 * sizeof(unsigned long long), e->stream));
  JR_LAUNCH(state_digest_kernel, (unsigned)((plane + 255) / 256), 256, e->stream, e->d, e->scratch);
  CK(cudaGetLastError());
  CK(cudaMemcpyAsync(out, e->scratch, sizeof(uint64_t), cudaMemcpyDeviceToHost, e->stream));
  CK(cudaStreamSynchronize(e->stream));
  return JR_OK;
}

static jr_status stream_sums(jr_engine* e, uint64_t v[5]) {
  CK(cudaSetDevice(e->cfg.device));
  const size_t plane = (size_t)e->d.R * e->d.Gp;
  CK(cudaMemsetAsync(e->scratch, 0, 8 * sizeof(unsigned long long), e->stream));
  JR_LAUNCH(stream_digest_kernel, (unsigned)((plane + 255) / 256), 256, e->stream, e->d, e->scratch);
  CK(cudaGetLastError());
  CK(cudaMemcpyAsync(v, e->scratch, 5 * sizeof(uint64_t), cudaMemcpyDeviceToHost, e->stream));
  CK(cudaStreamSynchronize(e->stream));
  return JR_OK;
}

jr_status jr_stream_digest(jr_engine* e, uint64_t* md, uint64_t* fd, uint64_t* nm, uint64_t* nf) {
  if (!e) return JR_E_INVAL;
  if (!(e->d.flags & JR_F_STREAM_DIGEST)) { set_err("engine created without JR_F_STREAM_DIGEST"); return JR_E_INVAL; }
  uint64_t v[5];
  jr_status st = stream_sums(e, v);
  if (st != JR_OK) return st;
  if (md) *md = v[0];
  if (fd) *fd = v[1];
  if (nm) *nm = v[2];
  if (nf) *nf = v[3];
  return JR_OK;
}

jr_status jr_fold_count(jr_engine* e, uint64_t* n) {
  if (!e || !n) return JR_E_INVAL;
  *n = 0;
  if (!e->last_launch_folded) return JR_OK;
  CK(cudaSetDevice(e->cfg.device));
  std::vector<uint8_t> h(e->d.Gp);
  CK(cudaMemcpyAsync(h.data(), e->symdone, h.size(), cudaMemcpyDeviceToHost, e->stream));
  CK(cudaStreamSynchronize(e->stream));
  for (uint32_t g = 0; g < e->d.G; ++g) *n += h[g];
  return JR_OK;
}

jr_status jr_fault_count(jr_engine* e, uint64_t* n) {
  if (!e || !n) return JR_E_INVAL;
  uint64_t v[5];
  jr_status st = stream_sums(e, v);
  if (st != JR_OK) return st;
  *n = v[4];
  return JR_OK;
}


jr_status jr_compact(jr_engine* e) {
  if (!e) return JR_E_INVAL;
  CK(cudaSetDevice(e->cfg.device));
  const size_t plane = (size_t)e->d.R * e->d.Gp;
  JR_LAUNCH(compact_kernel, (unsigned)((plane + 127) / 128), 128, e->stream, e->d);
  CK(cudaGetLastError());
  return JR_OK;
}

jr_status jr_truncate(jr_engine* e, uint32_t margin) {
  if (!e) return JR_E_INVAL;
  CK(cudaSetDevice(e->cfg.device));
  JR_LAUNCH(truncate_kernel, (e->d.Gp + 127) / 128, 128, e->stream, e->d, margin, (const uint8_t*)nullptr);
  CK(cudaGetLastError());
  return JR_OK;
}

jr_status jr_host_alloc(size_t bytes, void** out) {
  if (!out || !bytes) return JR_E_INVAL;
  *out = nullptr;
  cudaError_t err = cudaHostAlloc(out, bytes, 0);
  if (err != cudaSuccess) {
    set_err("cudaHostAlloc(%zu bytes): %s", bytes, cudaGetErrorString(err));
    return err == cudaErrorMemoryAllocation ? JR_E_NOMEM : JR_E_CUDA;
  }
  return JR_OK;
}

void jr_host_free(void* p) {
  if (p) cudaFreeHost(p);
}

jr_status jr_set_auto_truncate(jr_engine* e, int enabled, uint32_t margin) {
  if (!e) return JR_E_INVAL;
  e->auto_trunc = enabled != 0;
  e->auto_trunc_margin = margin;
  return JR_OK;
}

jr_status jr_chain_export_many(jr_engine* e, const uint32_t* groups, const uint32_t* nodes, size_t n,
                               jr_persisted_chain* out, jr_block* blocks, size_t cap_blocks, size_t* n_blocks) {
  if (!e || !n_blocks || (n && (!groups || !nodes || !out))) return JR_E_INVAL;
  *n_blocks = 0;
  if (n == 0) return JR_OK;
  if (n > 0x7fffffffu) return JR_E_INVAL;
  std::vector<uint2> targets(n);
  for (size_t k = 0; k < n; ++k) {
    if (groups[k] >= e->d.G || nodes[k] < 1 || nodes[k] > e->d.R) {
      set_err("target %zu: group or node out of range", k);
      return JR_E_INVAL;
    }
    targets[k] = make_uint2(groups[k], nodes[k] - 1);
  }
  CK(cudaSetDevice(e->cfg.device));
  const size_t o_desc = (n * sizeof(uint2) + 15) / 16 * 16;
  jr_status st = many_reserve(e, o_desc + n * sizeof(jr_persisted_chain));
  if (st != JR_OK) return st;
  char* base = (char*)e->many_buf;
  CK(cudaMemcpyAsync(base, targets.data(), n * sizeof(uint2), cudaMemcpyHostToDevice, e->stream));
  JR_LAUNCH(export_count_kernel, (unsigned)((n + 127) / 128), 128, e->stream, e->d, (const uint2*)base, (uint32_t)n,
            (jr_persisted_chain*)(base + o_desc));
  CK(cudaGetLastError());
  CK(cudaMemcpyAsync(out, base + o_desc, n * sizeof(jr_persisted_chain), cudaMemcpyDeviceToHost, e->stream));
  CK(cudaStreamSynchronize(e->stream));
  uint64_t total = 0;
  for (size_t k = 0; k < n; ++k) {
    out[k].first_block = total;
    total += out[k].n_blocks;
  }
  *n_blocks = (size_t)total;
  if (!blocks || cap_blocks < total) return JR_E_CAPACITY;
  if (total == 0) return JR_OK;
  const size_t o_blk = (n * sizeof(jr_persisted_chain) + 15) / 16 * 16;
  if ((st = many_reserve(e, o_blk + total * sizeof(jr_block))) != JR_OK) return st;
  base = (char*)e->many_buf;
  CK(cudaMemcpyAsync(base, out, n * sizeof(jr_persisted_chain), cudaMemcpyHostToDevice, e->stream));
  JR_LAUNCH(export_pack_kernel, (unsigned)((n + 127) / 128), 128, e->stream, e->d, (const jr_persisted_chain*)base,
            (uint32_t)n, (jr_block*)(base + o_blk));
  CK(cudaGetLastError());
  CK(cudaMemcpyAsync(blocks, base + o_blk, total * sizeof(jr_block), cudaMemcpyDeviceToHost, e->stream));
  CK(cudaStreamSynchronize(e->stream));
  return JR_OK;
}

jr_status jr_node_restart_many(jr_engine* e, uint64_t now_ms, const jr_persisted_chain* chains, size_t n,
                               const jr_block* blocks, size_t n_blocks) {
  if (!e || (n && !chains) || (n_blocks && !blocks)) return JR_E_INVAL;
  if (n == 0) return JR_OK;
  if (n > 0x7fffffffu) return JR_E_INVAL;
  const Dev& d = e->d;
  uint32_t g_lo = 0xffffffffu, g_hi = 0;
  for (size_t k = 0; k < n; ++k) {
    if (chains[k].group >= d.G || chains[k].node < 1 || chains[k].node > d.R) {
      set_err("chains[%zu]: group or node out of range", k);
      return JR_E_INVAL;
    }
    g_lo = std::min(g_lo, chains[k].group);
    g_hi = std::max(g_hi, chains[k].group);
  }
  const size_t span = (size_t)g_hi - g_lo + 1;
  std::vector<uint8_t> seen(span * d.R, 0);
  bool host_blocks = false;
  for (size_t k = 0; k < n; ++k) {
    const jr_persisted_chain& c = chains[k];
    uint8_t& s = seen[(size_t)(c.node - 1) * span + (c.group - g_lo)];
    if (s) {
      set_err("chains[%zu]: replica (%u, %u) appears twice", k, c.group, c.node);
      return JR_E_INVAL;
    }
    s = 1;
    if (c.n_blocks == JR_RESTART_IN_PLACE) continue;
    if (c.n_blocks > d.cap || c.first_block > n_blocks || n_blocks - c.first_block < c.n_blocks || c.commit >= 0xffffffffull) {
      set_err("chains[%zu]: slice outside blocks[0, %zu), more than chain_capacity blocks, or commit >= 2^32-1", k, n_blocks);
      return JR_E_INVAL;
    }
    host_blocks |= c.n_blocks > 0;
  }
  CK(cudaSetDevice(e->cfg.device));
  if (host_blocks) {
    std::vector<uint32_t> floor(span);
    CK(cudaMemcpyAsync(floor.data(), d.tb + g_lo, span * sizeof(uint32_t), cudaMemcpyDeviceToHost, e->stream));
    CK(cudaStreamSynchronize(e->stream));
    for (size_t k = 0; k < n; ++k) {
      const jr_persisted_chain& c = chains[k];
      if (c.n_blocks == JR_RESTART_IN_PLACE) continue;
      const uint64_t lo = floor[c.group - g_lo];
      for (uint32_t j = 0; j < c.n_blocks; ++j) {
        const jr_block& b = blocks[c.first_block + j];
        if (b.id < lo || b.id - lo >= d.cap || b.next >= 0xffffffffull || (j && b.id <= blocks[c.first_block + j - 1].id)) {
          set_err("chains[%zu] block %u: id not ascending or outside [floor, floor + chain_capacity), or next >= 2^32-1 (D4, D7)", k, j);
          return JR_E_INVAL;
        }
      }
    }
  }
  const size_t o_blk = (n * sizeof(jr_persisted_chain) + 15) / 16 * 16;
  jr_status st = many_reserve(e, o_blk + n_blocks * sizeof(jr_block));
  if (st != JR_OK) return st;
  char* base = (char*)e->many_buf;
  CK(cudaMemcpyAsync(base, chains, n * sizeof(jr_persisted_chain), cudaMemcpyHostToDevice, e->stream));
  if (n_blocks) CK(cudaMemcpyAsync(base + o_blk, blocks, n_blocks * sizeof(jr_block), cudaMemcpyHostToDevice, e->stream));
  JR_LAUNCH(node_restart_kernel, (unsigned)((n + 127) / 128), 128, e->stream, d, now_ms, (const jr_persisted_chain*)base,
            (uint32_t)n, (const jr_block*)(base + o_blk), e->rp.rm);
  CK(cudaGetLastError());
  CK(cudaStreamSynchronize(e->stream));
  return JR_OK;
}

jr_status jr_node_restart(jr_engine* e, uint32_t group, uint32_t node, uint64_t now_ms, const jr_block* blocks,
                          size_t n_blocks, uint64_t commit, int commit_key) {
  if (!e || group >= e->d.G || node < 1 || node > e->d.R || (n_blocks && !blocks)) return JR_E_INVAL;
  if (n_blocks > e->d.cap || commit >= 0xffffffffull) return JR_E_INVAL;
  std::vector<jr_block> v(blocks, blocks + n_blocks);
  std::stable_sort(v.begin(), v.end(), [](const jr_block& a, const jr_block& b) { return a.id < b.id; });
  size_t m = 0;
  for (size_t k = 0; k < v.size(); ++k)
    if (k + 1 == v.size() || v[k + 1].id != v[k].id) v[m++] = v[k];
  jr_persisted_chain c;
  c.group = group;
  c.node = node;
  c.commit = commit;
  c.first_block = 0;
  c.n_blocks = (uint32_t)m;
  c.commit_key = commit_key ? 1u : 0u;
  return jr_node_restart_many(e, now_ms, &c, 1, v.data(), m);
}

jr_status jr_verify_groups(jr_engine* e, const uint32_t* groups, size_t n_groups, jr_verify_report* report,
                           jr_verify_finding* findings, size_t cap, size_t* n_findings) {
  if (!e || !report || !n_findings || (n_groups && !groups)) return JR_E_INVAL;
  const Dev& d = e->d;
  const size_t n = groups ? n_groups : d.G;
  std::vector<uint32_t> list;
  if (groups) {
    std::vector<uint8_t> seen(d.G, 0);
    for (size_t k = 0; k < n; ++k) {
      if (groups[k] >= d.G || seen[groups[k]]) {
        set_err("groups[%zu]: out of range or named twice", k);
        return JR_E_INVAL;
      }
      seen[groups[k]] = 1;
    }
    list.assign(groups, groups + n);
    std::sort(list.begin(), list.end());
  }
  memset(report, 0, sizeof *report);
  report->groups_checked = n;
  *n_findings = 0;
  if (n == 0) return JR_OK;
  CK(cudaSetDevice(e->cfg.device));
#ifdef JR_EMU
  const uint32_t T = 1;
#else
  const uint32_t T = 256;
#endif
  const size_t reps = (size_t)d.R * n;
  const uint32_t n_ctas = (uint32_t)((n + T - 1) / T);
  const size_t o_part = 16 * sizeof(unsigned long long), o_list = o_part + ((size_t)n_ctas * 8 + 15) / 16 * 16;
  const size_t o_vw = o_list + (n * 4 + 15) / 16 * 16, o_vf = o_vw + reps * sizeof(uint2);
  jr_status st = scratch_reserve(&e->verify_buf, &e->verify_cap, o_vf + reps * sizeof(uint2));
  if (st != JR_OK) return st;
  char* base = (char*)e->verify_buf;
  unsigned long long* rep = (unsigned long long*)base;
  unsigned long long* part = (unsigned long long*)(base + o_part);
  const uint32_t* dlist = groups ? (const uint32_t*)(base + o_list) : nullptr;
  uint2* vw = (uint2*)(base + o_vw);
  uint2* vf = (uint2*)(base + o_vf);
  CK(cudaMemsetAsync(rep, 0, VERIFY_COUNTS * sizeof(unsigned long long), e->stream));
  if (groups) CK(cudaMemcpyAsync(base + o_list, list.data(), n * 4, cudaMemcpyHostToDevice, e->stream));
  const unsigned grid = (unsigned)((reps + 255) / 256);
  JR_LAUNCH(verify_walk_kernel, grid, 256, e->stream, d, dlist, (uint32_t)n, vw);
  CK(cudaGetLastError());
  JR_LAUNCH(verify_judge_kernel, grid, 256, e->stream, d, dlist, (uint32_t)n, (const uint2*)vw, vf, rep);
  CK(cudaGetLastError());
  unsigned long long cnt[VERIFY_COUNTS];
  CK(cudaMemcpyAsync(cnt, rep, sizeof cnt, cudaMemcpyDeviceToHost, e->stream));
  CK(cudaStreamSynchronize(e->stream));
  report->replicas_checked = cnt[0];
  report->replicas_skipped = cnt[1];
  report->below_floor = cnt[2];
  report->commit_absent = cnt[3];
  report->chain_broken = cnt[4];
  report->diverged = cnt[5];
  report->leader_conflicts = cnt[6];
  const size_t total = (size_t)(cnt[2] + cnt[3] + cnt[4] + cnt[5] + cnt[6]);
  *n_findings = total;
  if (total == 0) return JR_OK;
  if (!findings || cap < total) return JR_E_CAPACITY;
  if ((st = many_reserve(e, total * sizeof(jr_verify_finding))) != JR_OK) return st;
  jr_verify_finding* out = (jr_verify_finding*)e->many_buf;
  JR_LAUNCH(verify_count_kernel, n_ctas, T, e->stream, d, (uint32_t)n, (const uint2*)vf, part);
  CK(cudaGetLastError());
  JR_LAUNCH(verify_scan_kernel, 1, 1, e->stream, part, n_ctas);
  CK(cudaGetLastError());
  JR_LAUNCH(verify_pack_kernel, n_ctas, T, e->stream, d, dlist, (uint32_t)n, (const uint2*)vf, (const unsigned long long*)part, out);
  CK(cudaGetLastError());
  CK(cudaMemcpyAsync(findings, out, total * sizeof(jr_verify_finding), cudaMemcpyDeviceToHost, e->stream));
  CK(cudaStreamSynchronize(e->stream));
  return JR_OK;
}

namespace {
struct SaveHeader {
  uint64_t magic, bytes;
  jr_config cfg;
  uint32_t cur, route_valid;
  uint64_t step_index;
};
constexpr uint64_t SAVE_MAGIC = 0x4a52454e47494e32ull;
struct Segment { void* p; size_t n; };
std::vector<Segment> save_segments(jr_engine* e) {
  const Dev& d = e->d;
  const size_t plane = (size_t)d.R * d.Gp;
  const size_t rows = (size_t)d.capm + 1;
  std::vector<Segment> v = {
      {d.p0, plane * sizeof(uint4)}, {d.p1, plane * sizeof(uint4)}, {d.p2, plane * sizeof(uint4)}, {d.p3, plane * sizeof(uint4)},
      {d.pr, plane * ((d.R + 3) / 4) * sizeof(uint4)}, {d.mk, plane * sizeof(uint32_t)},
      {d.qt, plane * JR_CLIENT_QUEUE_CAP * sizeof(uint4)}, {d.dg, plane * sizeof(uint4)}, {d.cn, plane * sizeof(uint2)},
      {d.cnext, plane * rows * sizeof(uint32_t)}, {d.ctok, plane * rows * sizeof(unsigned long long)},
      {d.ob[0], plane * (size_t)d.U * sizeof(uint4)}, {d.ob[1], plane * (size_t)d.U * sizeof(uint4)},
      {d.oc[0], plane * sizeof(uint32_t)}, {d.oc[1], plane * sizeof(uint32_t)},
      {d.fs, plane * ((d.flags & JR_F_CAPTURE_FSM) ? 2 * (size_t)d.F : 1) * sizeof(uint4)}, {d.fc, plane * sizeof(uint2)},
      {d.tb, (size_t)d.Gp * sizeof(uint32_t)}, {e->route, (size_t)d.G * sizeof(uint32_t)}};
  if (e->rp.pn)
    v.push_back({e->rp.pn, pn_units(plane) * sizeof(uint4)});
  return v;
}
}

jr_status jr_engine_save_size(jr_engine* e, size_t* bytes) {
  if (!e || !bytes) return JR_E_INVAL;
  size_t n = sizeof(SaveHeader);
  for (const Segment& sg : save_segments(e)) n += sg.n;
  *bytes = n;
  return JR_OK;
}

jr_status jr_engine_save(jr_engine* e, void* buf, size_t cap) {
  if (!e || !buf) return JR_E_INVAL;
  size_t need = 0;
  jr_engine_save_size(e, &need);
  if (cap < need) return JR_E_CAPACITY;
  CK(cudaSetDevice(e->cfg.device));
  jr_status st = jr_engine_sync(e);
  if (st != JR_OK) return st;
  SaveHeader h;
  memset(&h, 0, sizeof h);
  h.magic = SAVE_MAGIC;
  h.bytes = need;
  h.cfg = e->cfg;
  h.cur = (uint32_t)e->cur;
  h.step_index = e->step_index;
  memcpy(buf, &h, sizeof h);
  char* at = (char*)buf + sizeof h;
  for (const Segment& sg : save_segments(e)) {
    CK(cudaMemcpyAsync(at, sg.p, sg.n, cudaMemcpyDeviceToHost, e->stream));
    at += sg.n;
  }
  CK(cudaStreamSynchronize(e->stream));
  return JR_OK;
}

jr_status jr_engine_restore(jr_engine* e, const void* buf, size_t bytes) {
  if (!e || !buf || bytes < sizeof(SaveHeader)) return JR_E_INVAL;
  SaveHeader h;
  memcpy(&h, buf, sizeof h);
  size_t need = 0;
  jr_engine_save_size(e, &need);
  jr_config a = h.cfg, b = e->cfg;
  a.device = b.device = 0;
  if (h.magic != SAVE_MAGIC || h.bytes != need || bytes < need || memcmp(&a, &b, sizeof a) != 0) {
    set_err("checkpoint does not match this engine's configuration");
    return JR_E_INVAL;
  }
  CK(cudaSetDevice(e->cfg.device));
  jr_status st = jr_engine_sync(e);
  if (st != JR_OK) return st;
  const char* at = (const char*)buf + sizeof h;
  for (const Segment& sg : save_segments(e)) {
    CK(cudaMemcpyAsync(sg.p, at, sg.n, cudaMemcpyHostToDevice, e->stream));
    at += sg.n;
  }
  CK(cudaStreamSynchronize(e->stream));
  e->cur = (int)h.cur;
  e->step_index = h.step_index;
  e->fsm_npending = 0;
  e->resp_b = -1;
  return JR_OK;
}

jr_status jr_set_alive(jr_engine* e, uint32_t group, uint32_t node, int alive) {
  if (!e || group >= e->d.G || node < 1 || node > e->d.R) return JR_E_INVAL;
  CK(cudaSetDevice(e->cfg.device));
  JR_LAUNCH(set_alive_kernel, 1, 1, e->stream, e->d, group, node - 1, alive);
  CK(cudaGetLastError());
  return JR_OK;
}

jr_status jr_kill_leaders(jr_engine* e, uint64_t salt, uint32_t permille, uint64_t* n_killed) {
  if (!e) return JR_E_INVAL;
  CK(cudaSetDevice(e->cfg.device));
  CK(cudaMemsetAsync(e->scratch, 0, sizeof(unsigned long long), e->stream));
  JR_LAUNCH(kill_leaders_kernel, (e->d.G + 127) / 128, 128, e->stream, e->d, mix64(e->d.seed ^ salt), permille, e->scratch);
  CK(cudaGetLastError());
  uint64_t k = 0;
  CK(cudaMemcpyAsync(&k, e->scratch, sizeof k, cudaMemcpyDeviceToHost, e->stream));
  CK(cudaStreamSynchronize(e->stream));
  if (n_killed) *n_killed = k;
  return JR_OK;
}

jr_status jr_leader_table_device(jr_engine* e, void* dev_out) {
  if (!e || !dev_out) return JR_E_INVAL;
  CK(cudaSetDevice(e->cfg.device));
  JR_LAUNCH(leader_table_kernel, (e->d.G + 127) / 128, 128, e->stream, e->d, (jr_leader_entry*)dev_out, e->route);
  CK(cudaGetLastError());
  return JR_OK;
}

jr_status jr_leader_table_async(jr_engine* e, jr_leader_entry* host_out) {
  if (!e || !host_out) return JR_E_INVAL;
  const int b = e->tab_i;
  e->tab_i = (b + 1) % jr_engine::NBUF;
  if (e->tab_used[b]) CK(cudaStreamWaitEvent(e->stream, e->tab_free[b], 0));
  jr_status st = jr_leader_table_device(e, e->leaders[b]);
  if (st != JR_OK) return st;
  CK(cudaEventRecord(e->tab_ready[b], e->stream));
  CK(cudaStreamWaitEvent(e->d2h, e->tab_ready[b], 0));
  CK(cudaMemcpyAsync(host_out, e->leaders[b], (size_t)e->d.G * sizeof(jr_leader_entry), cudaMemcpyDeviceToHost, e->d2h));
  CK(cudaEventRecord(e->tab_free[b], e->d2h));
  e->tab_used[b] = true;
  std::lock_guard<std::mutex> l(e->qmu);
  if (e->tab_npending == jr_engine::NBUF) {
    for (int k = 0; k + 1 < jr_engine::NBUF; ++k) e->tab_pending[k] = e->tab_pending[k + 1];
    --e->tab_npending;
  }
  e->tab_pending[e->tab_npending++] = b;
  return JR_OK;
}

jr_status jr_leader_table_wait(jr_engine* e) {
  if (!e) return JR_E_INVAL;
  CK(cudaSetDevice(e->cfg.device));
  int b;
  {
    std::lock_guard<std::mutex> l(e->qmu);
    if (e->tab_npending == 0) return JR_OK;
    b = e->tab_pending[0];
    for (int k = 0; k + 1 < jr_engine::NBUF; ++k) e->tab_pending[k] = e->tab_pending[k + 1];
    --e->tab_npending;
  }
  CK(cudaEventSynchronize(e->tab_free[b]));
  return JR_OK;
}

jr_status jr_leader_table(jr_engine* e, jr_leader_entry* host_out) {
  jr_status st = jr_leader_table_async(e, host_out);
  if (st != JR_OK) return st;
  CK(cudaStreamSynchronize(e->d2h));
  std::lock_guard<std::mutex> l(e->qmu);
  e->tab_npending = 0;
  return JR_OK;
}

}
```

josefine_b200/csrc/raft_device.cuh:

```cuda
#pragma once
#include <stdint.h>

#include "jr_cuda.h"

#include "../../include/josefine_raft_abi.h"

namespace jr {

constexpr uint32_t ABSENT = 0xFFFFFFFFu;
constexpr uint32_t TO_PEERS = 0u;
constexpr uint32_t TO_CLIENT = 0xFFFFu;
constexpr uint32_t GROUPS_PER_CTA = 32;

enum : uint32_t {
  PH_RESET_OUT = 1u << 0,
  PH_RESET_FSM = 1u << 1,
  PH_DRAIN = 1u << 2,
  PH_PROPOSE = 1u << 3,
  PH_TICK = 1u << 4
};

__host__ __device__ inline uint32_t unit_hdr(uint32_t kind, uint32_t flag, uint32_t aux, uint32_t to) {
  return (kind & 15u) | ((flag & 1u) << 4) | ((aux & 255u) << 8) | (to << 16);
}

struct Dev {
  uint4 *p0, *p1, *p2, *p3, *pr;
  uint32_t* mk;
  uint4* qt;
  uint4* dg;
  uint2* cn;
  uint32_t* cnext;
  unsigned long long* ctok;
  uint32_t* tb;
  uint4* ob[2];
  uint32_t* oc[2];
  uint4* fs;
  uint4* fr;
  uint2* fc;
  uint32_t* fq;
  uint32_t G, Gp, R, cap, capm, U, F, Fr, flags;
  uint32_t emin, emax, hb;
  uint32_t Us, W;
  uint32_t use_index;
  uint32_t resident;
  uint32_t* hunf;
  uint32_t* hscat;
  uint32_t* scatter;
  uint32_t* done;
  unsigned long long* prof;
  uint64_t seed, goff;
};

struct Local {
  uint4* in;
  uint4* out;
  uint32_t* cin;
  uint32_t* cout;
  uint4* tc;
  uint16_t* mk_in;
  uint16_t* mk_out;
  uint32_t Us, W, lane;
};
constexpr uint32_t MK_SCAN = 0x8000u;
constexpr uint32_t MK_SLOTS = 15u;

struct StepParams {
  uint64_t now;
  uint64_t step_index;
  uint32_t phases;
  uint32_t n_synth;
  uint32_t n_ticks;
  uint32_t dt;
  int cur;
  const jr_proposal* proposals;
  uint32_t prop_stride;
  uint32_t n_parts = 1, part_ticks = 0, n_blocks = 0, epoch = 0;
  uint32_t trunc = 0, trunc_margin = 0;
  uint32_t ticket_base = 0;
  const uint8_t* symdone = nullptr;
  const uint8_t* symblk = nullptr;
  const uint4* tok_runs = nullptr;
  const uint32_t* tok_route = nullptr;
  uint32_t tok_tick = 0;
};

__host__ __device__ inline uint64_t mix64(uint64_t x) {
  x += 0x9e3779b97f4a7c15ull;
  x = (x ^ (x >> 30)) * 0xbf58476d1ce4e5b9ull;
  x = (x ^ (x >> 27)) * 0x94d049bb133111ebull;
  return x ^ (x >> 31);
}
__host__ __device__ inline uint64_t fold(uint64_t h, uint64_t w) { return mix64(h ^ w); }

__host__ __device__ inline uint32_t election_timeout_draw(uint64_t seed, uint64_t group, uint32_t node,
                                                          uint32_t draw, uint32_t mn, uint32_t mx) {
  uint64_t x = mix64(seed ^ 0x6a09e667f3bcc908ull);
  x = mix64(x + group);
  x = mix64(x + (((uint64_t)node << 32) | draw));
  return mn + (uint32_t)(((x >> 32) * (uint64_t)(mx - mn)) >> 32);
}

__host__ __device__ inline uint64_t synth_token(uint64_t step_index, uint32_t i, uint64_t g_global) {
  return ((step_index * 8 + i + 1) << 32) | (g_global & 0xffffffffull);
}

struct Cmd {
  uint32_t kind, flag, node_id, nblk;
  uint32_t block;
  uint64_t term;
  uint64_t last_term;
  uint32_t blk_s, blk_at;
  const jr_msg* host_msg;
};

#ifdef JR_DEVICE_CODE

__device__ __noinline__ uint64_t digest_message_fn(uint64_t h, uint32_t kind, uint32_t to, uint32_t flag,
                                                   uint32_t nblk, uint32_t node_id, uint64_t t,
                                                   uint64_t last_term, uint64_t block, uint64_t token,
                                                   uint32_t addr) {
  uint32_t to_kind = to == TO_PEERS ? JR_ADDR_PEERS : (to == TO_CLIENT ? JR_ADDR_CLIENT : JR_ADDR_PEER);
  uint32_t to_id = to_kind == JR_ADDR_PEER ? to : 0u;
  h = fold(h, (uint64_t)kind | ((uint64_t)to_kind << 8) | ((uint64_t)(flag & 1u) << 16) |
                  ((uint64_t)nblk << 24) | ((uint64_t)to_id << 32));
  h = fold(h, node_id);
  h = fold(h, t);
  h = fold(h, last_term);
  h = fold(h, block);
  h = fold(h, token);
  h = fold(h, (uint64_t)(addr >> 16) | ((uint64_t)(addr & 0xffffu) << 8));
  return h;
}

__device__ __noinline__ uint64_t digest_send_fn(uint64_t h, uint32_t self, uint32_t kind, uint32_t to,
                                                uint32_t flag, uint32_t aux, uint64_t t, uint32_t w,
                                                uint32_t* n_out) {
  uint32_t n = 1;
  switch (kind) {
    case JR_CMD_VOTE_REQUEST:
      n = aux;
      for (uint32_t k = 0; k < aux; ++k) h = digest_message_fn(h, kind, to, 0, 0, self, t, t, w, 0, 0);
      break;
    case JR_CMD_VOTE_RESPONSE: h = digest_message_fn(h, kind, to, flag, 0, self, t, 0, 0, 0, 0); break;
    case JR_CMD_APPEND_RESPONSE: h = digest_message_fn(h, kind, to, flag, 0, self, t, 0, w, 0, 0); break;
    case JR_CMD_HEARTBEAT: h = digest_message_fn(h, kind, to, 0, 0, self, t, 0, w, 0, 0); break;
    case JR_CMD_HEARTBEAT_RESPONSE: h = digest_message_fn(h, kind, to, flag, 0, 0, 0, 0, w, 0, 0); break;
    case JR_CMD_CLIENT_REQUEST: h = digest_message_fn(h, kind, to, 0, 0, 0, 0, 0, 0, t, w); break;
    default: h = digest_message_fn(h, kind, to, 0, 0, 0, 0, 0, 0, t, 0); break;
  }
  *n_out = n;
  return h;
}

__device__ __noinline__ uint64_t digest_fsm_fn(uint64_t h, bool notify, uint32_t bid, uint32_t next_or_addr,
                                               uint64_t tok) {
  if (notify) {
    h = fold(h, (uint64_t)JR_FSM_NOTIFY | ((uint64_t)(next_or_addr >> 16) << 8) |
                    ((uint64_t)(next_or_addr & 0xffffu) << 32));
    h = fold(h, bid);
    h = fold(h, 0);
  } else {
    h = fold(h, (uint64_t)JR_FSM_APPLY);
    h = fold(h, bid);
    h = fold(h, next_or_addr);
  }
  return fold(h, tok);
}

#ifdef JR_PROFILE
__device__ __forceinline__ unsigned long long* jr_prof_smem() {
  __shared__ unsigned long long acc[8 * 3 * 16 * 2];
  return acc;
}
#define JR_PROF_T0(var) long long var = clock64()
#define JR_PROF_ADD(role, slot, var) do { long long _n = clock64(); if ((threadIdx.x & 31u) == 0) { unsigned long long* _p = jr_prof_smem() + (((threadIdx.x >> 5) * 3 + (role)) * 16 + (slot)) * 2; _p[0] += (unsigned long long)(_n - var); _p[1] += 1ull; } var = clock64(); } while (0)
#else
#define JR_PROF_T0(var) do { } while (0)
#define JR_PROF_ADD(role, slot, var) do { } while (0)
#endif


constexpr uint32_t FSR_APPLY = 0u, FSR_NOTIFY = 1u, FSR_PATTERN = 2u;
constexpr uint32_t FSR_CLIENT = (uint32_t)JR_ADDR_CLIENT << 16;
constexpr uint32_t FS_MAX_RUN = 0xffffffu;
constexpr uint32_t FS_PATTERN_BITS = 160u;
constexpr uint32_t FS_NOTIFY_BIT = 0x80000000u;

struct FsmOut {
  uint4* slot0;
  size_t plane;
  uint32_t F, g, r;
  uint32_t mask = 0;
};

struct FsmRun {
  uint32_t next_id, count;
  uint64_t last, stride;
};

__device__ __forceinline__ uint32_t fsm_put_record(uint32_t nrec, const FsmOut& o, uint32_t kind, uint32_t count, uint32_t id0,
                                                   uint32_t addr, uint64_t tok0, uint64_t stride) {
  if (nrec < o.F) {
    o.slot0[(size_t)(2 * nrec) * o.plane] = make_uint4(o.g, kind | (o.r << 2) | (count << 8), id0, addr);
    o.slot0[(size_t)(2 * nrec + 1) * o.plane] =
        make_uint4((uint32_t)tok0, (uint32_t)(tok0 >> 32), (uint32_t)stride, (uint32_t)(stride >> 32));
  }
  return nrec + 1;
}

__device__ __forceinline__ uint32_t fsm_close_run(uint32_t nrec, const FsmOut& o, bool notify, const FsmRun& run) {
  const uint32_t c = run.count;
  if (!c) return nrec;
  const uint64_t tok0 = c > 1 ? run.last - (uint64_t)(c - 1) * run.stride : run.last;
  const uint32_t addr = notify ? (c > 1 ? FSR_CLIENT : (uint32_t)run.stride) : o.mask;
  return fsm_put_record(nrec, o, notify ? FSR_NOTIFY : FSR_APPLY, c, run.next_id - c, addr, tok0,
                        (notify && c == 1) ? 0ull : run.stride);
}

struct FsmEnc {
  uint32_t nrec, seq;
  uint32_t wseq, pb2;
  uint64_t pb0, pb1;
  FsmRun ra, rn;
};

__device__ __forceinline__ void fsm_enc_begin(FsmEnc& s, uint2 c) {
  s.nrec = c.x; s.seq = s.wseq = c.y;
  s.pb0 = s.pb1 = 0; s.pb2 = 0;
  s.ra = FsmRun{0, 0, 0, 0};
  s.rn = FsmRun{0, 0, 0, 0};
}

template <bool NOTIFY>
// ... 898 lines not shown
```

josefine_b200/csrc/sym_fold.cuh:

```cuda
#pragma once
#include "raft_device.cuh"

namespace jr {
#ifdef JR_DEVICE_CODE

struct SymMail {
  uint32_t hb, hb_commit;
  uint32_t ae, ae_nb, ae_id[JR_MAX_AE_BLOCKS];
  uint32_t mk;
  uint32_t hbr, hbr_commit, hbr_has;
  uint32_t ar, ar_head;
  __device__ __forceinline__ uint32_t id(uint32_t k) const {
    uint32_t v = ae_id[0];
#pragma unroll
    for (uint32_t j = 1; j < JR_MAX_AE_BLOCKS; ++j)
      if (k == j) v = ae_id[j];
    return v;
  }
  __device__ __forceinline__ void set_id(uint32_t k, uint32_t v) {
#pragma unroll
    for (uint32_t j = 0; j < JR_MAX_AE_BLOCKS; ++j)
      if (k == j) ae_id[j] = v;
  }
};

constexpr uint32_t SYM_ROWS = 8;
#ifndef JR_SYM_LANES
#define JR_SYM_LANES 128
#endif
constexpr uint32_t SYM_LANES = JR_SYM_LANES;
constexpr uint32_t SYM_ENC_L = 5, SYM_ENC_F = 3;
constexpr uint32_t SYM_SMEM_UNITS = 2 * SYM_ROWS + SYM_ENC_L + SYM_ENC_F;
constexpr uint32_t SYM2_GROUPS = 64;
constexpr uint32_t SYM2_UNITS = SYM_SMEM_UNITS + 2 * 2 + 2 * 1;
constexpr uint32_t SYM2_ABORT = 1u << 8, SYM2_IDS = 1u << 9, SYM2_MODE = 1u << 10;
enum : uint32_t {
  SP_MAIL_IN = 0,
  SP_AR = 1,
  SP_CLIENT = 2,
  SP_ENC_NOTIFY = 3,
  SP_ENC_APPLY = 4,
  SP_MAIL_OUT = 5,
  SP_BARRIER = 6,
  SP_HB = 7,
  SP_SCAN = 8,
  SP_EXTEND = 9,
  SP_ENTER = 10, SP_FILL = 11, SP_LEAVE = 12, SP_TRUNC = 13,
};

template <int R, bool SPLIT = false, bool CHECK = false>
struct SymGroup {
  static constexpr uint32_t STRIDE = SPLIT ? SYM2_GROUPS : SYM_LANES;
  const Dev& d;
  const uint32_t g;
  const size_t plane;
  uint32_t L;
  uint32_t F0;
  uint64_t term, hbtime, now;
  uint32_t head, commit, idgen, maxkey, ckey, ph_self, mode_self, ph_f, mode_f;
  uint32_t fhead, fcommit, fmaxkey, fckey;
  uint32_t n_hb;
  uint64_t last_hb;
  uint32_t tbase;
  uint32_t flo;
  uint4* rows;
  uint4* enc;
  uint32_t lcnt, fcnt;
  uint32_t lwend, fwend;
  uint32_t n_app;
  bool abort;
  bool share;
#ifdef JR_PROFILE
  long long pt;
  uint32_t prole, pslot;
  __device__ __forceinline__ uint32_t phase(uint32_t slot) {
    const uint32_t o = pslot;
    if constexpr (SPLIT) {
      JR_PROF_ADD(prole, o, pt);
      pslot = slot;
    }
    return o;
  }
#else
  __device__ __forceinline__ uint32_t phase(uint32_t) const { return 0; }
#endif

  __device__ __forceinline__ SymGroup(const Dev& dv, uint32_t g_) : d(dv), g(g_), plane((size_t)R * dv.Gp) {
#ifdef JR_PROFILE
    pt = 0; prole = JR_ROLE_CANDIDATE; pslot = 0;
#endif
  }
  __device__ __forceinline__ size_t rg(uint32_t r) const { return (size_t)r * d.Gp + g; }
  __device__ __forceinline__ size_t row(uint32_t r, uint32_t bid) const { return (size_t)(bid & d.capm) * plane + rg(r); }
  __device__ __forceinline__ bool in_window(uint32_t bid) const { return bid - tbase < d.cap; }
  __device__ __forceinline__ uint4& slot(uint32_t r, uint32_t bid) const { return rows[((r == L ? 0u : SYM_ROWS) + (bid % SYM_ROWS)) * STRIDE]; }
  __device__ __forceinline__ void cache_put(uint32_t r, uint32_t bid, uint32_t nx, uint64_t tk) const {
    slot(r, bid) = make_uint4(bid, nx, (uint32_t)tk, (uint32_t)(tk >> 32));
  }
  __device__ __forceinline__ void fetch(uint32_t r, uint32_t bid, uint32_t& next, uint64_t& tok) {
    if (!in_window(bid)) { next = ABSENT; tok = 0; return; }
    if (CHECK) { next = d.cnext[row(r, bid)]; tok = d.ctok[row(r, bid)]; return; }
    const uint4 e = slot(r, bid);
    if (e.x == bid) { next = e.y; tok = (uint64_t)e.z | ((uint64_t)e.w << 32); return; }
    next = __ldcg(d.cnext + row(r, bid));
    tok = __ldcg(d.ctok + row(r, bid));
    if (!SPLIT) cache_put(r, bid, next, tok);
  }
  __device__ __forceinline__ void fetch_sent(uint32_t bid, uint32_t mk_sent, uint32_t n_app, uint32_t& next, uint64_t& tok) {
    if (!SPLIT) { fetch(L, bid, next, tok); return; }
    if (!in_window(bid)) { next = ABSENT; tok = 0; return; }
    if (bid + SYM_ROWS > mk_sent + n_app) {
      const uint4 e = slot(L, bid);
      if (e.x == bid) { next = e.y; tok = (uint64_t)e.z | ((uint64_t)e.w << 32); return; }
    }
    next = __ldcg(d.cnext + row(L, bid));
    tok = __ldcg(d.ctok + row(L, bid));
  }
  __device__ __forceinline__ void cache_clear(uint32_t first = 0, uint32_t n = 2 * SYM_ROWS) const {
#pragma unroll
    for (uint32_t k = 0; k < 2 * SYM_ROWS; ++k)
      if (k >= first && k < first + n) rows[k * STRIDE] = make_uint4(ABSENT, ABSENT, 0u, 0u);
  }
  __device__ __forceinline__ void cache_fill(uint32_t r, uint32_t top) const {
    uint32_t nx[SYM_ROWS];
    uint64_t tk[SYM_ROWS];
#pragma unroll
    for (uint32_t j = 0; j < SYM_ROWS; ++j)
      if (j <= top && in_window(top - j)) {
        nx[j] = d.cnext[row(r, top - j)];
        tk[j] = d.ctok[row(r, top - j)];
      }
#pragma unroll
    for (uint32_t j = 0; j < SYM_ROWS; ++j)
      if (j <= top && in_window(top - j)) cache_put(r, top - j, nx[j], tk[j]);
  }
  __device__ __forceinline__ bool has(uint32_t r, uint32_t bid) {
    uint32_t n; uint64_t t;
    fetch(r, bid, n, t);
    return n != ABSENT;
  }
  __device__ __forceinline__ void fetch_f(uint32_t bid, uint32_t& next, uint64_t& tok) {
    if (in_window(bid) && bid < flo) { abort = true; next = ABSENT; tok = 0; return; }
    fetch(F0, bid, next, tok);
  }
  __device__ __forceinline__ bool has_f(uint32_t bid) {
    uint32_t n; uint64_t t;
    fetch_f(bid, n, t);
    return n != ABSENT;
  }

  __device__ __forceinline__ uint4& eq(uint32_t k) const { return enc[k * STRIDE]; }
  __device__ __forceinline__ FsmOut leader_out() const { return FsmOut{d.fs + rg(L), plane, d.F, g, L}; }
  __device__ __forceinline__ FsmOut followers_out() const {
    return FsmOut{d.fs + rg(F0), plane, d.F, g, F0, ((1u << R) - 1u) & ~(1u << L)};
  }
  __device__ __forceinline__ void enc_init_leader(uint2 leader_fc) {
    eq(0) = make_uint4(leader_fc.x, leader_fc.y, leader_fc.y, 0u);
#pragma unroll
    for (uint32_t k = 1; k < SYM_ENC_L; ++k) eq(k) = make_uint4(0u, 0u, 0u, 0u);
    lwend = FS_PATTERN_BITS;
  }
  __device__ __forceinline__ void enc_init_followers() {
#pragma unroll
    for (uint32_t k = SYM_ENC_L; k < SYM_ENC_L + SYM_ENC_F; ++k) eq(k) = make_uint4(0u, 0u, 0u, 0u);
    fwend = FS_PATTERN_BITS;
  }
  template <bool NOTIFY>
  __device__ __forceinline__ bool run_extend(uint4& q, uint2& qs, uint32_t bid, uint32_t nxa, uint64_t tok) const {
    const uint4 r = q;
    if (!r.y || bid != r.x || r.y >= FS_MAX_RUN || nxa != (NOTIFY ? FSR_CLIENT : bid - 1u)) return false;
    const uint2 st = qs;
    const uint64_t step = tok - ((uint64_t)r.z | ((uint64_t)r.w << 32));
    if (r.y == 1u) {
      if (st.x != (NOTIFY ? FSR_CLIENT : bid - 2u)) return false;
      qs = make_uint2((uint32_t)step, (uint32_t)(step >> 32));
    } else if (step != ((uint64_t)st.x | ((uint64_t)st.y << 32))) {
      return false;
    }
    q = make_uint4(bid + 1u, r.y + 1u, (uint32_t)tok, (uint32_t)(tok >> 32));
    return true;
  }
  template <bool NOTIFY>
  __device__ __forceinline__ void emit_leader(uint32_t bid, uint32_t nxa, uint64_t tok) {
    if (!(d.flags & JR_F_CAPTURE_FSM)) return;
    if (lcnt >= d.Fr) { abort = true; return; }
    const uint32_t outer = phase(NOTIFY ? SP_ENC_NOTIFY : SP_ENC_APPLY);
    if (lcnt + 1u != lwend &&
        run_extend<NOTIFY>(eq(NOTIFY ? 4 : 2), reinterpret_cast<uint2*>(&eq(3))[NOTIFY ? 1 : 0], bid, nxa, tok)) {
      if (NOTIFY) {
        const uint32_t b = lcnt + FS_PATTERN_BITS - lwend;
        uint32_t* w = b < 128u ? reinterpret_cast<uint32_t*>(&eq(1)) + (b >> 5) : &eq(0).w;
        *w |= 1u << (b & 31u);
      }
      ++lcnt;
      phase(outer);
      return;
    }
    FsmEnc e;
    const uint4 q0 = eq(0);
    e.nrec = q0.x; e.seq = q0.y + lcnt; e.wseq = q0.z; e.pb2 = q0.w;
    ++lcnt;
    const bool window = NOTIFY || e.seq + 1u - e.wseq == FS_PATTERN_BITS;
    uint4 q1 = make_uint4(0u, 0u, 0u, 0u);
    if (window) q1 = eq(1);
    e.pb0 = (uint64_t)q1.x | ((uint64_t)q1.y << 32);
    e.pb1 = (uint64_t)q1.z | ((uint64_t)q1.w << 32);
    const uint4 qr = eq(NOTIFY ? 4 : 2), qs = eq(3);
    FsmRun& run = NOTIFY ? e.rn : e.ra;
    run.next_id = qr.x; run.count = qr.y;
    run.last = (uint64_t)qr.z | ((uint64_t)qr.w << 32);
    run.stride = NOTIFY ? ((uint64_t)qs.z | ((uint64_t)qs.w << 32)) : ((uint64_t)qs.x | ((uint64_t)qs.y << 32));
    fsm_enc_push<NOTIFY>(e, leader_out(), bid, nxa, tok);
    if (e.nrec != q0.x || e.wseq != q0.z || e.pb2 != q0.w) eq(0) = make_uint4(e.nrec, q0.y, e.wseq, e.pb2);
    if (window) eq(1) = make_uint4((uint32_t)e.pb0, (uint32_t)(e.pb0 >> 32), (uint32_t)e.pb1, (uint32_t)(e.pb1 >> 32));
    eq(NOTIFY ? 4 : 2) = make_uint4(run.next_id, run.count, (uint32_t)run.last, (uint32_t)(run.last >> 32));
    uint2* st = reinterpret_cast<uint2*>(&eq(3)) + (NOTIFY ? 1 : 0);
    *st = make_uint2((uint32_t)run.stride, (uint32_t)(run.stride >> 32));
// ... 20 lines not shown
      FsmEnc e;
      const uint4 q0 = eq(SYM_ENC_L), q1 = eq(SYM_ENC_L + 1);
      const uint2 q2 = *reinterpret_cast<const uint2*>(&eq(SYM_ENC_L + 2));
      e.nrec = q0.x; e.seq = q0.y + fcnt; e.wseq = q0.z; e.pb2 = 0;
      e.pb0 = e.pb1 = 0;
      e.ra = FsmRun{q1.x, q1.y, (uint64_t)q1.z | ((uint64_t)q1.w << 32), (uint64_t)q2.x | ((uint64_t)q2.y << 32)};
      fsm_enc_push<false>(e, followers_out(), bid, next, tok);
      if (e.nrec != q0.x || e.wseq != q0.z) eq(SYM_ENC_L) = make_uint4(e.nrec, q0.y, e.wseq, 0u);
      eq(SYM_ENC_L + 1) = make_uint4(e.ra.next_id, e.ra.count, (uint32_t)e.ra.last, (uint32_t)(e.ra.last >> 32));
      *reinterpret_cast<uint2*>(&eq(SYM_ENC_L + 2)) = make_uint2((uint32_t)e.ra.stride, (uint32_t)(e.ra.stride >> 32));
      fwend = e.wseq - q0.y + FS_PATTERN_BITS;
    } else {
      const uint4 e = make_uint4(bid, next, (uint32_t)tok, (uint32_t)(tok >> 32));
#pragma unroll
      for (int r = 0; r < R; ++r)
        if ((uint32_t)r != L) d.fr[(size_t)fcnt * plane + rg(r)] = e;
    }
    ++fcnt;
    phase(outer);
  }
  __device__ __forceinline__ uint2 followers_end() {
    FsmEnc e;
    const uint4 q0 = eq(SYM_ENC_L), q1 = eq(SYM_ENC_L + 1), q2 = eq(SYM_ENC_L + 2);
    e.nrec = q0.x; e.seq = q0.y + fcnt; e.wseq = q0.z; e.pb2 = 0;
    e.pb0 = e.pb1 = 0;
    e.ra = FsmRun{q1.x, q1.y, (uint64_t)q1.z | ((uint64_t)q1.w << 32), (uint64_t)q2.x | ((uint64_t)q2.y << 32)};
    e.rn = FsmRun{0, 0, 0, 0};
    return fsm_enc_end(e, followers_out());
  }

  __device__ __forceinline__ uint32_t committed_index(uint32_t v_new, uint32_t n_new, uint32_t v_old) const {
    uint32_t v[R];
    v[0] = ph_self;
#pragma unroll
    for (int i = 1; i < R; ++i) v[i] = (uint32_t)i <= n_new ? v_new : v_old;
#pragma unroll
    for (int i = 0; i < R; ++i)
#pragma unroll
      for (int j = 0; j + 1 < R - i; ++j) {
        const uint32_t a = v[j], b = v[j + 1];
        v[j] = max(a, b);
        v[j + 1] = min(a, b);
      }
    return v[R / 2];
  }
  __device__ __forceinline__ void leader_commit(uint32_t v_new, uint32_t n_new, uint32_t v_old) {
    const uint32_t above = (ph_self > commit ? 1u : 0u) + (v_new > commit ? n_new : 0u) + (v_old > commit ? (uint32_t)(R - 1) - n_new : 0u);
    if (above < (uint32_t)(R / 2 + 1)) return;
    const uint32_t q = committed_index(v_new, n_new, v_old);
    if (q <= commit) return;
    if (!has(L, q)) { abort = true; return; }
    const uint32_t prev = commit;
    ckey = 1;
    commit = q;
    bool first = true;
    for (uint32_t b = max(prev, tbase); b <= q; ++b) {
      uint32_t nx; uint64_t tk;
      fetch(L, b, nx, tk);
      if (nx == ABSENT) continue;
      if (first) { first = false; continue; }
      emit_leader<false>(b, nx, tk);
    }
  }
  __device__ __forceinline__ void client_request(uint64_t tok) {
    const uint32_t bid = idgen++;
    if (!(bid > head) || !in_window(bid)) { abort = true; return; }
    d.cnext[row(L, bid)] = head;
    d.ctok[row(L, bid)] = tok;
    cache_put(L, bid, head, tok);
    if (bid > maxkey) maxkey = bid;
    head = bid;
    emit_leader<true>(bid, FSR_CLIENT, tok);
    mode_self = ph_self < head ? 1u : 0u;
    if (ph_self < head) ph_self = head;
    leader_commit(ph_f, R - 1, ph_f);
  }

  __device__ __forceinline__ void leader_tick(const SymMail& in, SymMail& out, uint64_t dense_tok, uint32_t n_synth,
                                              uint64_t step_index) {
    if (in.hbr && !in.hbr_has && in.hbr_commit > 0) { abort = true; return; }
    if (in.ar) {
      phase(SP_AR);
      const uint32_t old = ph_f, v = in.ar_head;
      const bool inc = old < v;
      const uint32_t nw = inc ? v : old;
      for (uint32_t j = 1; j <= (uint32_t)(R - 1) && !abort; ++j) leader_commit(nw, j, old);
      ph_f = nw;
      mode_f = inc ? 1u : 0u;
      if (abort) return;
    }
    phase(SP_CLIENT);
    if (dense_tok) client_request(dense_tok);
    for (uint32_t i = 0; i < n_synth && !abort; ++i) client_request(synth_token(step_index, i, d.goff + g));
    if (abort) return;
    phase(SP_MAIL_OUT);
    const uint64_t el = now >= hbtime ? now - hbtime : 0;
    if (el > (uint64_t)d.hb) {
      out.hb = 1;
      out.hb_commit = commit;
      hbtime = now;
    }
    out.ae = 1;
    out.mk = maxkey;
    if (!SPLIT) replicate(ph_f, mode_f, maxkey, out);
  }
  __device__ __forceinline__ void replicate(uint32_t phf, uint32_t modef, uint32_t mk, SymMail& out) {
    const uint32_t take = modef ? JR_MAX_AE_BLOCKS : 1u;
    uint32_t bid = max(phf, tbase), pulled = 0, nb = 0;
    while (pulled < 1 + take) {
      uint32_t nx = ABSENT; uint64_t tk = 0;
      while (bid <= mk) {
        fetch(L, bid, nx, tk);
        if (nx != ABSENT) break;
        ++bid;
      }
      if (bid > mk) break;
      if (pulled >= 1) out.set_id(nb++, bid);
      ++pulled;
      ++bid;
    }
    out.ae_nb = nb;
  }

  __device__ __forceinline__ void follower_heartbeat(const SymMail& in, SymMail& out) {
    phase(SP_HB);
    ++n_hb;
    last_hb = now;
    const uint32_t c = in.hb_commit;
    const bool hasc = has_f(c);
    if (hasc && c > fcommit) {
      const uint32_t prev = fcommit;
      fckey = 1;
      fcommit = c;
      for (uint32_t b = max(prev, tbase); b < c; ++b) {
        uint32_t nx; uint64_t tk;
        fetch_f(b, nx, tk);
        if (nx != ABSENT) emit_followers(b, nx, tk);
      }
    }
    out.hbr = 1;
    out.hbr_commit = fcommit;
    out.hbr_has = hasc ? 1u : 0u;
  }
  __device__ __forceinline__ void follower_extend(uint32_t bid, uint32_t nx, uint64_t tk) {
    const uint32_t outer = phase(SP_EXTEND);
    if (nx == ABSENT || !has_f(nx) || !in_window(bid)) { abort = true; return; }
#pragma unroll
    for (int r = 0; r < R; ++r)
      if ((uint32_t)r != L) {
        d.cnext[row(r, bid)] = nx;
        d.ctok[row(r, bid)] = tk;
      }
    cache_put(F0, bid, nx, tk);
    if (bid > fmaxkey) fmaxkey = bid;
    fhead = bid;
    phase(outer);
  }
  __device__ __forceinline__ void follower_tick(const SymMail& in, SymMail& out) {
    if (in.hb) follower_heartbeat(in, out);
    if (in.ae) {
      phase(SP_SCAN);
      for (uint32_t k = 0; k < in.ae_nb && !abort; ++k) {
        const uint32_t bid = in.id(k);
        uint32_t nx; uint64_t tk;
        fetch_sent(bid, in.mk, n_app, nx, tk);
        follower_extend(bid, nx, tk);
      }
      if (abort) return;
      if (in.ae_nb) {
        out.ar = 1;
        out.ar_head = fhead;
      }
    }
  }
  __device__ __forceinline__ void follower_tick_view(const SymMail& in, uint32_t phf, uint32_t modef, uint32_t mk, SymMail& out) {
    if (in.hb) follower_heartbeat(in, out);
    if (!in.ae || abort) return;
    phase(SP_SCAN);
    const uint32_t take = modef ? JR_MAX_AE_BLOCKS : 1u;
    uint32_t bid = max(phf, tbase), pulled = 0, nb = 0;
    while (pulled < 1 + take) {
      uint32_t nx = ABSENT; uint64_t tk = 0;
      while (bid <= mk) {
        fetch_sent(bid, mk, n_app, nx, tk);
        if (nx != ABSENT) break;
        ++bid;
      }
      if (bid > mk) break;
      if (pulled >= 1) {
        follower_extend(bid, nx, tk);
        if (abort) return;
        ++nb;
      }
      ++pulled;
      ++bid;
    }
    if (nb) {
      out.ar = 1;
      out.ar_head = fhead;
    }
  }
};

template <int R>
__device__ __forceinline__ bool sym_enter(SymGroup<R, false, true>& s, SymMail& m, const StepParams& p, int prv) {
  const Dev& d = s.d;
  if (s.g >= d.G) return false;
  uint32_t L = R, nlead = 0;
  uint4 p2[R];
#pragma unroll
  for (int r = 0; r < R; ++r) {
    p2[r] = d.p2[s.rg(r)];
    const uint32_t meta = p2[r].w;
    if (((meta >> 8) & 255u) || ((meta >> 27) & 1u)) return false;
    if ((meta & 255u) == JR_ROLE_LEADER) { L = r; ++nlead; }
    else if ((meta & 255u) != JR_ROLE_FOLLOWER) return false;
    if ((meta >> 24) & 7u) return false;
  }
  if (nlead != 1) return false;
  s.L = L;
  s.F0 = L == 0 ? 1u : 0u;
  const uint4 l0 = d.p0[s.rg(L)];
  s.term = (uint64_t)l0.x | ((uint64_t)l0.y << 32);
  s.tbase = d.tb[s.g];
  uint4 pl = p2[0], pf = p2[0];
  const uint32_t f0i = L == 0 ? 1u : 0u;
#pragma unroll
  for (int r = 0; r < R; ++r) {
    if ((uint32_t)r == L) pl = p2[r];
    if ((uint32_t)r == f0i) pf = p2[r];
  }
  s.head = pl.x; s.commit = pl.y; s.idgen = pl.z;
  s.ckey = (pl.w >> 28) & 1u;
  s.maxkey = d.mk[s.rg(L)];
  if (!(s.idgen > s.head)) return false;
  const uint4 l3 = d.p3[s.rg(L)];
  s.hbtime = (uint64_t)l3.x | ((uint64_t)l3.y << 32);
  const uint32_t f0 = s.F0;
  s.fhead = pf.x; s.fcommit = pf.y; s.fckey = (pf.w >> 28) & 1u;
  s.fmaxkey = d.mk[s.rg(f0)];
  const uint64_t hbgap = ((uint64_t)d.hb / p.dt + 1) * p.dt;
#pragma unroll
  for (int r = 0; r < R; ++r) {
    if ((uint32_t)r == L) continue;
    const uint4 a = d.p0[s.rg(r)];
    if (((uint64_t)a.x | ((uint64_t)a.y << 32)) != s.term || a.z != L + 1 || a.w != L + 1) return false;
    if (p2[r].x != s.fhead || p2[r].y != s.fcommit || ((p2[r].w >> 28) & 1u) != s.fckey) return false;
    if (d.mk[s.rg(r)] != s.fmaxkey) return false;
  }
  if ((uint64_t)d.emin <= hbgap || s.hbtime > p.now) return false;
  uint32_t ph[R];
#pragma unroll
  for (int q = 0; q < (R + 3) / 4; ++q) {
    const uint4 v = d.pr[(size_t)q * s.plane + s.rg(L)];
    if (q * 4 + 0 < R) ph[q * 4 + 0] = v.x;
    if (q * 4 + 1 < R) ph[q * 4 + 1] = v.y;
    if (q * 4 + 2 < R) ph[q * 4 + 2] = v.z;
    if (q * 4 + 3 < R) ph[q * 4 + 3] = v.w;
  }
  const uint32_t prmask = (pl.w >> 16) & 255u;
  s.ph_self = 0; s.ph_f = 0;
#pragma unroll
  for (int r = 0; r < R; ++r) {
    if ((uint32_t)r == L) s.ph_self = ph[r];
    if ((uint32_t)r == f0) s.ph_f = ph[r];
  }
  s.mode_self = (prmask >> L) & 1u;
  s.mode_f = (prmask >> f0) & 1u;
#pragma unroll
  for (int r = 0; r < R; ++r)
    if ((uint32_t)r != L && (ph[r] != s.ph_f || ((prmask >> r) & 1u) != s.mode_f)) return false;
  constexpr uint32_t SYM_WINDOW = 16;
  const uint32_t top = min(s.maxkey, s.fmaxkey);
  const uint32_t lo_min = max(top > SYM_WINDOW - 1u ? top - (SYM_WINDOW - 1u) : 0u, s.tbase);
  if (top < s.tbase || s.ph_f < lo_min || s.fcommit < lo_min || s.commit < lo_min || s.fhead < lo_min || s.fmaxkey > s.maxkey) return false;
  const uint32_t lo = min(min(s.ph_f, s.fcommit), min(s.commit, s.fhead));
  s.flo = lo;
  const uint64_t grow = (uint64_t)p.n_ticks * (1u + p.n_synth) + 2u;
  if ((uint64_t)s.maxkey + grow >= (uint64_t)s.tbase + d.cap || (uint64_t)s.maxkey + grow >= FS_NOTIFY_BIT) return false;
  {
    constexpr uint32_t B = 4;
    bool same = true;
    for (uint32_t b0 = lo; b0 <= s.fmaxkey && same; b0 += B) {
      uint32_t n0[B];
      unsigned long long t0[B];
#pragma unroll
      for (uint32_t j = 0; j < B; ++j) {
        const uint32_t b = min(b0 + j, s.fmaxkey);
        n0[j] = d.cnext[s.row(f0, b)];
        t0[j] = d.ctok[s.row(f0, b)];
      }
#pragma unroll
      for (int r = 0; r < R; ++r) {
        if ((uint32_t)r == L || (uint32_t)r == f0) continue;
#pragma unroll
        for (uint32_t j = 0; j < B; ++j) {
          const uint32_t b = min(b0 + j, s.fmaxkey);
          const uint32_t n = d.cnext[s.row(r, b)];
          const unsigned long long t = d.ctok[s.row(r, b)];
          same = same && n == n0[j] && (n0[j] == ABSENT || t == t0[j]);
        }
      }
    }
    if (!same) return false;
  }
  m = SymMail{};
  if (p.phases & PH_DRAIN) {
  {
    const uint32_t cnt = d.oc[prv][s.rg(L)];
    uint32_t u = 0;
    auto unit = [&](uint32_t k) { return d.ob[prv][((size_t)k * R + L) * d.Gp + s.g]; };
    if (cnt > (uint32_t)(1 + JR_MAX_AE_BLOCKS + R)) return false;
    if (u < cnt) {
      const uint4 h = unit(u);
      if ((h.x & 15u) == JR_CMD_HEARTBEAT) {
        if ((h.x >> 16) != TO_PEERS || ((uint64_t)h.y | ((uint64_t)h.z << 32)) != s.term) return false;
        m.hb = 1; m.hb_commit = h.w;
        ++u;
      }
    }
    if (u < cnt) {
      uint32_t first = 0;
      for (int r = 0; r < R; ++r) {
        if ((uint32_t)r == L) continue;
        if (u >= cnt) return false;
        const uint4 h = unit(u);
        if ((h.x & 15u) != JR_CMD_APPEND_ENTRIES || (h.x >> 16) != (uint32_t)r + 1u ||
            ((uint64_t)h.y | ((uint64_t)h.z << 32)) != s.term) return false;
        const uint32_t nb = (h.x >> 8) & 255u, ref = (h.x >> 4) & 1u;
        if (!m.ae) {
          if (ref || nb > JR_MAX_AE_BLOCKS || h.w != u + 1 || u + 1 + nb > cnt) return false;
          m.ae = 1; m.ae_nb = nb; first = u + 1;
          for (uint32_t k = 0; k < nb; ++k) {
            const uint4 bu = unit(first + k);
            uint32_t nx; uint64_t tk;
            s.fetch(L, bu.x, nx, tk);
            if (nx != bu.y || tk != ((uint64_t)bu.z | ((uint64_t)bu.w << 32))) return false;
            m.set_id(k, bu.x);
          }
          u += 1 + nb;
        } else {
          if (!ref || nb != m.ae_nb || h.w != first) return false;
          ++u;
        }
      }
    }
    if (u != cnt) return false;
  }
  {
    const uint32_t cnt = d.oc[prv][s.rg(f0)];
    if (cnt > 2) return false;
    uint4 want[2] = {make_uint4(0, 0, 0, 0), make_uint4(0, 0, 0, 0)};
    for (uint32_t u = 0; u < cnt; ++u) want[u] = d.ob[prv][((size_t)u * R + f0) * d.Gp + s.g];
#pragma unroll
    for (int r = 0; r < R; ++r) {
      if ((uint32_t)r == L || (uint32_t)r == f0) continue;
      if (d.oc[prv][s.rg(r)] != cnt) return false;
      for (uint32_t u = 0; u < cnt; ++u) {
        const uint4 v = d.ob[prv][((size_t)u * R + r) * d.Gp + s.g];
        if (v.x != want[u].x || v.y != want[u].y || v.z != want[u].z || v.w != want[u].w) return false;
      }
    }
    uint32_t u = 0;
    if (u < cnt && (want[u].x & 15u) == JR_CMD_HEARTBEAT_RESPONSE) {
      if ((want[u].x >> 16) != L + 1) return false;
      m.hbr = 1; m.hbr_has = (want[u].x >> 4) & 1u; m.hbr_commit = want[u].w;
      ++u;
    }
    if (u < cnt && (want[u].x & 15u) == JR_CMD_APPEND_RESPONSE) {
      if ((want[u].x >> 16) != L + 1 || ((uint64_t)want[u].y | ((uint64_t)want[u].z << 32)) != s.term) return false;
      m.ar = 1; m.ar_head = want[u].w;
      ++u;
    }
    if (u != cnt) return false;
  }
  }
  uint64_t t_arr = 0;
  if (!m.hb) {
    const uint64_t due = s.hbtime + (uint64_t)d.hb + 1;
    t_arr = (due > p.now ? (due - p.now + p.dt - 1) / p.dt : 0) + 1;
  }
  const uint64_t checked = t_arr < p.n_ticks ? t_arr : p.n_ticks;
  if (checked) {
    const uint64_t t_last = p.now + (checked - 1) * p.dt;
#pragma unroll
    for (int r = 0; r < R; ++r) {
      if ((uint32_t)r == L) continue;
      const uint4 b = d.p1[s.rg(r)];
      const uint64_t etime = (uint64_t)b.x | ((uint64_t)b.y << 32);
      if (t_last >= etime && t_last - etime > (uint64_t)b.z) return false;
    }
  }
  return true;
}

enum : uint32_t {
  SR_FLAGS = 0, SR_TBASE,
  SR_HEAD, SR_COMMIT, SR_IDGEN, SR_MAXKEY, SR_PH_SELF, SR_PH_F, SR_HBTIME, SR_HB_COMMIT = SR_HBTIME + 2,
  SR_AE_ID, SR_FC_L = SR_AE_ID + JR_MAX_AE_BLOCKS,
  SR_FHEAD = SR_FC_L + 2, SR_FCOMMIT, SR_FMAXKEY, SR_FLO, SR_HBR_COMMIT, SR_AR_HEAD,
  SR_TERM, SR_P2W = SR_TERM + 2,
};
__host__ __device__ constexpr uint32_t sr_draws(uint32_t R) { return SR_P2W + (R + 1) / 2; }
__host__ __device__ constexpr uint32_t sr_idgen(uint32_t R) { return sr_draws(R) + R - 1; }
__host__ __device__ constexpr uint32_t sym_record_words(uint32_t R) { return sr_idgen(R) + R - 1; }

#ifndef JR_SYM_CHECK_MINCTAS
#define JR_SYM_CHECK_MINCTAS 5
#endif
constexpr uint32_t SYM_CHECK_THREADS = 128;
template <int R>
__global__ void __launch_bounds__(SYM_CHECK_THREADS, JR_SYM_CHECK_MINCTAS) sym_check_kernel(const Dev d, const StepParams p, uint32_t* rec) {
  const uint32_t g = blockIdx.x * blockDim.x + threadIdx.x;
  if (g >= d.Gp) return;
  const size_t n = d.Gp;
  uint32_t* w = rec + g;
  SymGroup<R, false, true> s(d, g);
  SymMail m;
  if (!sym_enter(s, m, p, 1 - p.cur)) { w[SR_FLAGS * n] = 0u; return; }
  const uint32_t L = s.L;
  const bool cap = (d.flags & JR_F_CAPTURE_FSM) != 0;
  bool share = cap;
  uint32_t hw[(R + 1) / 2];
#pragma unroll
  for (int k = 0; k < (R + 1) / 2; ++k) hw[k] = 0;
#pragma unroll
  for (int r = 0; r < R; ++r) {
    const uint4 c = d.p2[s.rg(r)];
    hw[r / 2] |= ((c.w >> 16) & ~(1u << 12)) << (16 * (r & 1));
    if ((uint32_t)r == L) continue;
    const uint32_t k = (uint32_t)r - ((uint32_t)r > L ? 1u : 0u);
    const uint2 fc = d.fc[s.rg(r)];
    if (fc.x | fc.y) share = false;
    w[(sr_draws(R) + k) * n] = d.p1[s.rg(r)].w;
    w[(sr_idgen(R) + k) * n] = c.z;
  }
  const uint2 fcl = cap ? d.fc[s.rg(L)] : make_uint2(0u, 0u);
  w[SR_FLAGS * n] = 1u | (L << 1) | (s.ckey << 4) | (s.fckey << 5) | (s.mode_self << 6) | (s.mode_f << 7) | (m.hb << 8) |
                    (m.ae << 9) | (m.ae_nb << 10) | (m.hbr << 13) | (m.hbr_has << 14) | (m.ar << 15) | ((share ? 1u : 0u) << 16);
  w[SR_TBASE * n] = s.tbase;
  w[SR_HEAD * n] = s.head; w[SR_COMMIT * n] = s.commit; w[SR_IDGEN * n] = s.idgen; w[SR_MAXKEY * n] = s.maxkey;
  w[SR_PH_SELF * n] = s.ph_self; w[SR_PH_F * n] = s.ph_f;
  w[SR_HBTIME * n] = (uint32_t)s.hbtime; w[(SR_HBTIME + 1) * n] = (uint32_t)(s.hbtime >> 32);
  w[SR_HB_COMMIT * n] = m.hb_commit;
#pragma unroll
  for (uint32_t k = 0; k < JR_MAX_AE_BLOCKS; ++k) w[(SR_AE_ID + k) * n] = m.ae_id[k];
  w[SR_FC_L * n] = fcl.x; w[(SR_FC_L + 1) * n] = fcl.y;
  w[SR_FHEAD * n] = s.fhead; w[SR_FCOMMIT * n] = s.fcommit; w[SR_FMAXKEY * n] = s.fmaxkey; w[SR_FLO * n] = s.flo;
  w[SR_HBR_COMMIT * n] = m.hbr_commit; w[SR_AR_HEAD * n] = m.ar_head;
  w[SR_TERM * n] = (uint32_t)s.term; w[(SR_TERM + 1) * n] = (uint32_t)(s.term >> 32);
#pragma unroll
  for (int k = 0; k < (R + 1) / 2; ++k) w[(SR_P2W + k) * n] = hw[k];
}

template <bool LEAD, bool FOLLOW, int R, bool SPLIT>
__device__ __forceinline__ bool sym_load(SymGroup<R, SPLIT>& s, SymMail& m, const uint32_t* rec, uint2& fc) {
  const uint32_t* w = rec + s.g;
  const size_t n = s.d.Gp;
  const uint32_t f = __ldg(w + SR_FLAGS * n);
  uint32_t v[SR_TERM];
  if (LEAD) {
#pragma unroll
    for (uint32_t k = SR_TBASE; k < SR_FHEAD; ++k) v[k] = __ldg(w + k * n);
  }
  if (FOLLOW) {
#pragma unroll
    for (uint32_t k = SR_FHEAD; k < SR_TERM; ++k) v[k] = __ldg(w + k * n);
    if (!LEAD) v[SR_TBASE] = __ldg(w + SR_TBASE * n);
  }
  if (!(f & 1u)) return false;
  s.L = (f >> 1) & 7u;
  s.F0 = s.L == 0 ? 1u : 0u;
  s.tbase = v[SR_TBASE];
  m = SymMail{};
  if (LEAD) {
    s.ckey = (f >> 4) & 1u; s.mode_self = (f >> 6) & 1u; s.mode_f = (f >> 7) & 1u;
    s.head = v[SR_HEAD]; s.commit = v[SR_COMMIT]; s.idgen = v[SR_IDGEN]; s.maxkey = v[SR_MAXKEY];
    s.ph_self = v[SR_PH_SELF]; s.ph_f = v[SR_PH_F];
    s.hbtime = (uint64_t)v[SR_HBTIME] | ((uint64_t)v[SR_HBTIME + 1] << 32);
    m.hb = (f >> 8) & 1u; m.ae = (f >> 9) & 1u; m.ae_nb = (f >> 10) & 7u;
    m.hb_commit = v[SR_HB_COMMIT];
#pragma unroll
    for (uint32_t k = 0; k < JR_MAX_AE_BLOCKS; ++k) m.ae_id[k] = v[SR_AE_ID + k];
    fc = make_uint2(v[SR_FC_L], v[SR_FC_L + 1]);
  }
  if (FOLLOW) {
    s.fckey = (f >> 5) & 1u;
    s.share = (f >> 16) & 1u;
    s.fhead = v[SR_FHEAD]; s.fcommit = v[SR_FCOMMIT]; s.fmaxkey = v[SR_FMAXKEY]; s.flo = v[SR_FLO];
    m.hbr = (f >> 13) & 1u; m.hbr_has = (f >> 14) & 1u; m.ar = (f >> 15) & 1u;
    m.hbr_commit = v[SR_HBR_COMMIT]; m.ar_head = v[SR_AR_HEAD];
  }
  return true;
}

template <int R, bool SPLIT>
__device__ __forceinline__ void sym_leave_leader(SymGroup<R, SPLIT>& s, const SymMail& last, int cur_last, const uint32_t* rec) {
  const Dev& d = s.d;
  const uint32_t L = s.L;
  {
    const size_t i = s.rg(L);
    const uint32_t* w = rec + s.g;
    const size_t n = d.Gp;
    const uint32_t t0 = __ldg(w + SR_TERM * n), t1 = __ldg(w + (SR_TERM + 1) * n), hw = __ldg(w + (SR_P2W + L / 2) * n);
    s.term = (uint64_t)t0 | ((uint64_t)t1 << 32);
    uint32_t prmask = 0;
#pragma unroll
    for (int r = 0; r < R; ++r) prmask |= (((uint32_t)r == L ? s.mode_self : s.mode_f) & 1u) << r;
    const uint32_t keep = (JR_ROLE_LEADER | (((hw >> (16 * (L & 1u))) & 0xffffu) << 16)) & ~((255u << 16) | (1u << 28));
    d.p2[i] = make_uint4(s.head, s.commit, s.idgen, keep | (prmask << 16) | (s.ckey << 28));
    d.p3[i] = make_uint4((uint32_t)s.hbtime, (uint32_t)(s.hbtime >> 32), 0u, 0u);
#pragma unroll
    for (int q = 0; q < (R + 3) / 4; ++q) {
      uint32_t v[4] = {0, 0, 0, 0};
#pragma unroll
      for (int k = 0; k < 4; ++k)
        if (q * 4 + k < R) v[k] = (uint32_t)(q * 4 + k) == L ? s.ph_self : s.ph_f;
      d.pr[(size_t)q * s.plane + i] = make_uint4(v[0], v[1], v[2], v[3]);
    }
    d.mk[i] = s.maxkey;
    uint32_t u = 0;
    auto put = [&](uint32_t k, uint4 v) { d.ob[cur_last][((size_t)k * R + L) * d.Gp + s.g] = v; };
    if (last.hb) put(u++, make_uint4(unit_hdr(JR_CMD_HEARTBEAT, 0, 0, TO_PEERS), (uint32_t)s.term, (uint32_t)(s.term >> 32), last.hb_commit));
    if (last.ae) {
      uint32_t first = 0;
      bool have = false;
#pragma unroll
      for (int r = 0; r < R; ++r) {
        if ((uint32_t)r == L) continue;
        if (!have) {
          first = u + 1;
          put(u, make_uint4(unit_hdr(JR_CMD_APPEND_ENTRIES, 0, last.ae_nb, r + 1), (uint32_t)s.term, (uint32_t)(s.term >> 32), first));
          for (uint32_t k = 0; k < last.ae_nb; ++k) {
            const uint32_t bid = last.id(k);
            uint32_t nx; uint64_t tk;
            s.fetch(L, bid, nx, tk);
            put(first + k, make_uint4(bid, nx, (uint32_t)tk, (uint32_t)(tk >> 32)));
          }
          u += 1 + last.ae_nb;
          have = true;
        } else {
          put(u++, make_uint4(unit_hdr(JR_CMD_APPEND_ENTRIES, 1, last.ae_nb, r + 1), (uint32_t)s.term, (uint32_t)(s.term >> 32), first));
        }
      }
    }
    d.oc[cur_last][i] = u;
    if ((d.flags & JR_F_CAPTURE_FSM) && s.lcnt) d.fc[i] = s.leader_end();
  }
}

template <int R, bool SPLIT>
__device__ __forceinline__ void sym_leave_followers(SymGroup<R, SPLIT>& s, const SymMail& last, int cur_last, const uint32_t* rec) {
  const Dev& d = s.d;
  const uint32_t L = s.L;
  const bool shared_records = s.share;
  const uint32_t* w = rec + s.g;
  const size_t n = d.Gp;
  const uint32_t t0 = __ldg(w + SR_TERM * n), t1 = __ldg(w + (SR_TERM + 1) * n);
  uint32_t hw[(R + 1) / 2], draws0[R], idgen[R];
#pragma unroll
  for (int k = 0; k < (R + 1) / 2; ++k) hw[k] = __ldg(w + (SR_P2W + k) * n);
#pragma unroll
  for (int r = 0; r < R; ++r) {
    if ((uint32_t)r == L) continue;
    const uint32_t k = (uint32_t)r - ((uint32_t)r > L ? 1u : 0u);
    draws0[r] = __ldg(w + (sr_draws(R) + k) * n);
    idgen[r] = __ldg(w + (sr_idgen(R) + k) * n);
  }
  s.term = (uint64_t)t0 | ((uint64_t)t1 << 32);
#pragma unroll
  for (int r = 0; r < R; ++r) {
    if ((uint32_t)r == L) continue;
    const size_t i = s.rg(r);
    if (s.n_hb) {
      const uint32_t draws = draws0[r] + s.n_hb;
      d.p1[i] = make_uint4((uint32_t)s.last_hb, (uint32_t)(s.last_hb >> 32),
                           election_timeout_draw(d.seed, d.goff + s.g, r + 1, draws - 1, d.emin, d.emax), draws);
    }
    const uint32_t upper = (hw[r / 2] >> (16 * (r & 1))) & 0xffffu;
    d.p2[i] = make_uint4(s.fhead, s.fcommit, idgen[r], (JR_ROLE_FOLLOWER | (upper << 16)) | (s.fckey << 28));
    d.mk[i] = s.fmaxkey;
    uint32_t u = 0;
    if (last.hbr)
      d.ob[cur_last][((size_t)u++ * R + r) * d.Gp + s.g] =
          make_uint4(unit_hdr(JR_CMD_HEARTBEAT_RESPONSE, last.hbr_has, 0, L + 1), 0u, 0u, last.hbr_commit);
    if (last.ar)
      d.ob[cur_last][((size_t)u++ * R + r) * d.Gp + s.g] =
          make_uint4(unit_hdr(JR_CMD_APPEND_RESPONSE, 1, 0, L + 1), (uint32_t)s.term, (uint32_t)(s.term >> 32), last.ar_head);
    d.oc[cur_last][i] = u;
    if ((d.flags & JR_F_CAPTURE_FSM) && s.fcnt) {
      if (!shared_records) fsm_flush(d.fr + i, s.fcnt, d.Fr, FsmOut{d.fs + i, s.plane, d.F, s.g, (uint32_t)r}, d.fc + i);
      else if ((uint32_t)r == s.F0) d.fc[i] = s.followers_end();
      else d.fc[i] = make_uint2(0u, s.fcnt);
    }
  }
}

template <int R>
__global__ void __launch_bounds__(SYM_LANES, 512 / SYM_LANES) sym_kernel(const Dev d, const StepParams p, uint8_t* symdone,
                                                                        const uint32_t* rec) {
  const uint32_t g = blockIdx.x * blockDim.x + threadIdx.x;
  if (g >= d.Gp) return;
  SymGroup<R> s(d, g);
  SymMail a, b;
  s.abort = false;
  s.lcnt = s.fcnt = 0;
  s.n_hb = 0;
  s.last_hb = 0;
  s.share = false;
  s.n_app = 1u + p.n_synth;
  __shared__ uint4 lane_smem[SYM_SMEM_UNITS * SYM_LANES];
  s.rows = lane_smem + threadIdx.x;
  s.enc = lane_smem + 2 * SYM_ROWS * SYM_LANES + threadIdx.x;
  s.cache_clear();
  uint2 fcl;
  bool ok = sym_load<true, true>(s, a, rec, fcl);
  if (ok) {
    s.cache_fill(s.L, s.maxkey);
    s.cache_fill(s.F0, s.fmaxkey);
    s.enc_init_leader(fcl);
    s.enc_init_followers();
    const jr_proposal* props = p.proposals;
    s.now = p.now;
    for (uint32_t t = 0; t < p.n_ticks && !s.abort; ++t) {
      b = SymMail{};
      uint64_t tok = 0;
      if ((p.phases & PH_PROPOSE) && (props || p.tok_runs)) {
        uint4 pr;
        if (p.tok_runs) {
          const uint4 rn = __ldg(p.tok_runs + g);
          const uint64_t base = (uint64_t)rn.x | ((uint64_t)rn.y << 32);
          const uint64_t tk = base + (uint64_t)(p.tok_tick + t) * ((uint64_t)rn.z | ((uint64_t)rn.w << 32));
          pr = make_uint4((uint32_t)tk, (uint32_t)(tk >> 32), base ? __ldg(p.tok_route + g) : 0u, 0u);
        } else {
          pr = __ldg(reinterpret_cast<const uint4*>(props) + g);
          props += p.prop_stride;
        }
        if (pr.z == s.L + 1) tok = (uint64_t)pr.x | ((uint64_t)pr.y << 32);
        else if (pr.z != 0) s.abort = true;
      }
      if (s.abort) break;
      s.leader_tick(a, b, tok, (p.phases & PH_PROPOSE) ? p.n_synth : 0u, p.step_index + t);
      if (s.abort) break;
      s.follower_tick(a, b);
      a = b;
      s.now += p.dt;
    }
    ok = !s.abort;
    if (ok) {
      const int cur_last = p.cur ^ (int)((p.n_ticks - 1) & 1u);
      sym_leave_leader(s, a, cur_last, rec);
      sym_leave_followers(s, a, cur_last, rec);
    }
  }
  symdone[g] = ok ? 1 : 0;
}

#ifndef JR_SYM2_MINCTAS
#define JR_SYM2_MINCTAS 4
#endif
#ifndef JR_SYM2_ROLES
#define JR_SYM2_ROLES 3
#endif
template <int R>
__global__ void __launch_bounds__(2 * SYM2_GROUPS, JR_SYM2_MINCTAS) sym2_kernel(const Dev d, const StepParams p, uint8_t* symdone, uint8_t* symblk,
                                                                                      const uint32_t* rec) {
  JR_DYN_SMEM(uint4, smem);
  auto pair_sync = [] { __syncthreads(); };
  constexpr uint32_t S = SYM2_GROUPS;
  const uint32_t w = threadIdx.x >> 5, lane = threadIdx.x & 31u;
  const bool lead = ((w ^ blockIdx.x) & 1u) == 0;
  const uint32_t gi = (w >> 1) * 32u + lane;
  const uint32_t g = blockIdx.x * S + gi;
  SymGroup<R, true> s(d, g);
  s.abort = false;
  s.lcnt = s.fcnt = 0;
  s.n_hb = 0;
  s.last_hb = 0;
  s.share = false;
  s.n_app = 1u + p.n_synth;
  s.rows = smem + gi;
  s.enc = smem + 2 * SYM_ROWS * S + gi;
  uint4* mail = smem + SYM_SMEM_UNITS * S + gi;
#ifdef JR_PROFILE
  for (uint32_t i = threadIdx.x; i < 8 * 3 * 16 * 2; i += blockDim.x) jr_prof_smem()[i] = 0;
  s.prole = lead ? JR_ROLE_LEADER : JR_ROLE_FOLLOWER;
  s.pslot = SP_ENTER;
  s.pt = clock64();
#endif
  s.cache_clear(lead ? 0u : SYM_ROWS, SYM_ROWS);
  const uint32_t blk = g / GROUPS_PER_CTA;
  if (lead && lane == 0 && g < d.Gp) symblk[blk] = 1;
  SymMail a;
  uint2 fcl;
  bool dead = g >= d.Gp || !(lead ? sym_load<true, false>(s, a, rec, fcl) : sym_load<false, true>(s, a, rec, fcl));
  s.phase(SP_FILL);
  if (!dead) {
    if (lead) {
      s.cache_fill(s.L, s.maxkey);
      s.enc_init_leader(fcl);
      mail[2 * S] = make_uint4(a.hb | (a.ae << 1) | (a.ae_nb << 4) | SYM2_IDS, a.hb_commit, s.maxkey, a.ae_id[0]);
      mail[3 * S] = make_uint4(a.ae_id[1], a.ae_id[2], a.ae_id[3], a.ae_id[4]);
    } else {
      s.cache_fill(s.F0, s.fmaxkey);
      s.enc_init_followers();
      mail[5 * S] = make_uint4(a.hbr | (a.hbr_has << 1) | (a.ar << 2), a.hbr_commit, a.ar_head, 0u);
    }
  }
  pair_sync();
  const jr_proposal* props = p.proposals;
  s.now = p.now;
  uint32_t cur = 0;
  for (uint32_t t = 0; t < p.n_ticks; ++t) {
    s.phase(SP_MAIL_IN);
    if (lead && (JR_SYM2_ROLES & 1)) {
      if (!dead) {
        const uint4 c = mail[(4 + (1 - cur)) * S];
        if (c.x & SYM2_ABORT) dead = true;
        else {
          SymMail in{}, out{};
          in.hbr = c.x & 1u; in.hbr_has = (c.x >> 1) & 1u; in.ar = (c.x >> 2) & 1u;
          in.hbr_commit = c.y; in.ar_head = c.z;
          uint64_t tok = 0;
          if ((p.phases & PH_PROPOSE) && (props || p.tok_runs)) {
            uint4 pr;
            if (p.tok_runs) {
              const uint4 rn = __ldg(p.tok_runs + g);
              const uint64_t base = (uint64_t)rn.x | ((uint64_t)rn.y << 32);
              const uint64_t tk = base + (uint64_t)(p.tok_tick + t) * ((uint64_t)rn.z | ((uint64_t)rn.w << 32));
              pr = make_uint4((uint32_t)tk, (uint32_t)(tk >> 32), base ? __ldg(p.tok_route + g) : 0u, 0u);
            } else {
              pr = __ldg(reinterpret_cast<const uint4*>(props + (size_t)t * p.prop_stride) + g);
            }
            if (pr.z == s.L + 1) tok = (uint64_t)pr.x | ((uint64_t)pr.y << 32);
            else if (pr.z != 0) s.abort = true;
          }
          if (!s.abort) s.leader_tick(in, out, tok, (p.phases & PH_PROPOSE) ? p.n_synth : 0u, p.step_index + t);
          if (s.abort) dead = true;
          else {
            mail[(2 * cur) * S] = make_uint4(out.hb | (out.ae << 1) | (s.mode_f ? SYM2_MODE : 0u), s.commit, s.maxkey, s.ph_f);
          }
        }
      }
      if (dead) mail[(2 * cur) * S] = make_uint4(SYM2_ABORT, 0u, 0u, 0u);
    } else if (!lead && (JR_SYM2_ROLES & 2)) {
      if (!dead) {
        const uint4 ma = mail[(2 * (1 - cur)) * S];
        if (ma.x & SYM2_ABORT) dead = true;
        else {
          SymMail in{}, out{};
          in.hb = ma.x & 1u; in.ae = (ma.x >> 1) & 1u;
          in.hb_commit = ma.y; in.mk = ma.z;
          if (ma.x & SYM2_IDS) {
            const uint4 mb = mail[(2 * (1 - cur) + 1) * S];
            in.ae_nb = (ma.x >> 4) & 15u;
            in.ae_id[0] = ma.w; in.ae_id[1] = mb.x; in.ae_id[2] = mb.y; in.ae_id[3] = mb.z; in.ae_id[4] = mb.w;
            s.follower_tick(in, out);
          } else {
            s.follower_tick_view(in, ma.w, (ma.x & SYM2_MODE) ? 1u : 0u, ma.z, out);
          }
          s.phase(SP_MAIL_OUT);
          if (s.abort) dead = true;
          else mail[(4 + cur) * S] = make_uint4(out.hbr | (out.hbr_has << 1) | (out.ar << 2), out.hbr_commit, out.ar_head, 0u);
        }
      }
      if (dead) mail[(4 + cur) * S] = make_uint4(SYM2_ABORT, 0u, 0u, 0u);
    }
    s.now += p.dt;
    s.phase(SP_BARRIER);
    pair_sync();
    cur ^= 1u;
  }
  s.phase(SP_LEAVE);
  const uint32_t lastb = cur ^ 1u;
  const uint4 la = mail[(2 * lastb) * S], lc = mail[(4 + lastb) * S];
  const bool ok = !dead && !((la.x | lc.x) & SYM2_ABORT);
  if (ok) {
    const int cur_last = p.cur ^ (int)((p.n_ticks - 1) & 1u);
    SymMail last{};
    if (lead) {
      last.hb = la.x & 1u; last.ae = (la.x >> 1) & 1u;
      last.hb_commit = la.y;
      if (last.ae) s.replicate(s.ph_f, s.mode_f, s.maxkey, last);
      sym_leave_leader(s, last, cur_last, rec);
    } else {
      last.hbr = lc.x & 1u; last.hbr_has = (lc.x >> 1) & 1u; last.ar = (lc.x >> 2) & 1u;
      last.hbr_commit = lc.y; last.ar_head = lc.z;
      sym_leave_followers(s, last, cur_last, rec);
    }
  }
  s.phase(SP_TRUNC);
  if (p.trunc) {
    pair_sync();
    if (ok && !lead) {
      const uint32_t lo = min(s.fcommit, la.y);
      const uint32_t floor = lo > p.trunc_margin ? lo - p.trunc_margin : 0u;
      if (floor > s.tbase) {
        for (uint32_t b = s.tbase; b < floor && b - s.tbase < d.cap; ++b)
#pragma unroll
          for (int r = 0; r < R; ++r) d.cnext[s.row(r, b)] = ABSENT;
        d.tb[g] = floor;
      }
    }
  }
  if (lead && g < d.Gp) {
    symdone[g] = ok ? 1 : 0;
    if (!ok) {
      symblk[blk] = 0;
      if (g < d.G) *(volatile uint32_t*)d.hunf = p.epoch;
    }
  }
#ifdef JR_PROFILE
  s.phase(SP_TRUNC);
  __syncthreads();
  if (d.prof)
    for (uint32_t i = threadIdx.x; i < 4 * 3 * 16 * 2; i += blockDim.x) {
      const unsigned long long v = jr_prof_smem()[i];
      if (v) atomicAdd(d.prof + (i % (3 * 16 * 2)), v);
    }
#endif
}

__global__ void sym_blocks_kernel(const uint8_t* symdone, uint8_t* symblk, uint32_t n_blocks) {
  const uint32_t b = blockIdx.x * blockDim.x + threadIdx.x;
  if (b >= n_blocks) return;
  const uint4* v = reinterpret_cast<const uint4*>(symdone + (size_t)b * GROUPS_PER_CTA);
  const uint4 x = v[0], y = v[1];
  const uint32_t all = 0x01010101u;
  symblk[b] = (x.x == all && x.y == all && x.z == all && x.w == all && y.x == all && y.y == all && y.z == all && y.w == all) ? 1 : 0;
}

#endif
}
```

Baseline: 11.88 billion.

## Carry symmetric-fold records across consecutive launches to skip re-entry checks

Double-buffers the symmetric-fold record array. At the end of sym2_kernel, each group writes its leader and follower state into the next buffer, tagged with the launch epoch, but only when an exit condition proves the state is consistent. On the next consecutive launch, sym_check_kernel can rebuild its record from the carried state and skip the full sym_enter scan of the per-replica planes. Any other API call clears the carry epoch so stale records are never used. The cost is twice the record memory, extra writes at kernel exit, and more complex invariants around validating the carry.

```diff
diff --git a/josefine_b200/csrc/engine.cu b/josefine_b200/csrc/engine.cu
--- a/josefine_b200/csrc/engine.cu
+++ b/josefine_b200/csrc/engine.cu
@@ -1179,6 +1179,8 @@
   uint8_t* symdone = nullptr;
   uint8_t* symblk = nullptr;
   uint32_t* symrec = nullptr;
+  int symrec_k = 0;
+  uint32_t carry_epoch = 0;
   bool auto_trunc = false;
   uint32_t auto_trunc_margin = 0;
   int no_fold = 0;
@@ -1277,13 +1279,16 @@
 template <int R>
 static void launch_sym_r(jr_engine* e, const StepParams& p) {
   if constexpr (R >= 2) {
+    const size_t words = (size_t)sym_record_alloc_words(R) * e->d.Gp;
+    uint32_t* rec = e->symrec + (size_t)e->symrec_k * words;
+    uint32_t* nxt = e->symrec + (size_t)(e->symrec_k ^ 1) * words;
     JR_LAUNCH(sym_check_kernel<R>, (e->d.Gp + SYM_CHECK_THREADS - 1) / SYM_CHECK_THREADS, SYM_CHECK_THREADS, e->stream, e->d, p,
-              e->symrec);
+              rec, nxt);
     if (e->sym_one_lane)
-      JR_LAUNCH(sym_kernel<R>, (e->d.Gp + SYM_LANES - 1) / SYM_LANES, SYM_LANES, e->stream, e->d, p, e->symdone, e->symrec);
+      JR_LAUNCH(sym_kernel<R>, (e->d.Gp + SYM_LANES - 1) / SYM_LANES, SYM_LANES, e->stream, e->d, p, e->symdone, rec);
     else
       JR_LAUNCH_SMEM(sym2_kernel<R>, (e->d.Gp + SYM2_GROUPS - 1) / SYM2_GROUPS, 2 * SYM2_GROUPS,
-                     (size_t)SYM2_UNITS * SYM2_GROUPS * sizeof(uint4), e->stream, e->d, p, e->symdone, e->symblk, e->symrec);
+                     (size_t)SYM2_UNITS * SYM2_GROUPS * sizeof(uint4), e->stream, e->d, p, e->symdone, e->symblk, rec, nxt);
   }
 }
 
@@ -1302,9 +1307,14 @@
   const size_t smem = step_smem_bytes(e->d);
   StepParams p = p_in;
   p.epoch = (uint32_t)(e->launches_total + 1) * 8u;
+  const uint32_t carry = e->carry_epoch;
+  e->carry_epoch = 0;
   if (fold_eligible(e, p)) {
+    p.carry = carry != 0 && carry + 8u == p.epoch ? carry : 0u;
     DISPATCH_R(e->cfg.n_replicas, (launch_sym_r<RR>(e, p)));
     CK(cudaGetLastError());
+    e->symrec_k ^= 1;
+    if (!e->sym_one_lane) e->carry_epoch = p.epoch;
     if (e->sym_one_lane) {
       JR_LAUNCH(sym_blocks_kernel, (n_blocks + 127) / 128, 128, e->stream, e->symdone, e->symblk, n_blocks);
       CK(cudaGetLastError());
@@ -1337,10 +1347,30 @@
   return JR_OK;
 }
 
+static bool enter(jr_engine* e) {
+  if (e) e->carry_epoch = 0;
+  return e != nullptr;
+}
+static bool enter_keeping_records(jr_engine* e) { return e != nullptr; }
+
 extern "C" {
 
 #ifdef JR_EMU
 int jr_is_emulation(void) { return 1; }
+uint32_t jr_emu_carry_epoch(jr_engine* e) { return e ? e->carry_epoch : 0u; }
+uint32_t jr_emu_carried_groups(jr_engine* e) {
+  if (!e) return 0;
+  cudaStreamSynchronize(e->stream);
+  const uint32_t R = e->d.R, Gp = e->d.Gp;
+  const uint32_t* t = e->symrec + (size_t)e->symrec_k * sym_record_alloc_words(R) * Gp + (size_t)sr_tag(R) * Gp;
+  uint32_t k = 0;
+  for (uint32_t g = 0; g < Gp; ++g) k += t[g] != 0 ? 1u : 0u;
+  return k;
+}
+int jr_emu_exit_carries(uint32_t fgap, uint32_t flo_in, uint32_t lo, uint32_t tb, uint32_t commit, uint32_t maxkey, uint32_t phf,
+                        uint32_t fcommit, uint32_t fhead, uint32_t fmaxkey) {
+  return sym_exit_carries(fgap, flo_in, lo, tb, commit, maxkey, phf, fcommit, fhead, fmaxkey) ? 1 : 0;
+}
 #endif
 
 const char* jr_last_error(void) { return g_err; }
@@ -1434,7 +1464,7 @@
   A(d.tb, d.Gp);
   A(e->symdone, d.Gp);
   A(e->symblk, d.Gp / GROUPS_PER_CTA);
-  A(e->symrec, (size_t)sym_record_words(d.R) * d.Gp);
+  A(e->symrec, (size_t)2 * sym_record_alloc_words(d.R) * d.Gp);
   if (d.flags & JR_F_CAPTURE_FSM) {
     const size_t reps = (size_t)cfg->n_groups * cfg->n_replicas;
     const size_t want = cfg->fsm_host_records ? cfg->fsm_host_records
@@ -1539,7 +1569,7 @@
 
 #ifdef JR_PROFILE
 jr_status jr_profile_read(jr_engine* e, unsigned long long* out96) {
-  if (!e || !out96) return JR_E_INVAL;
+  if (!enter_keeping_records(e) || !out96) return JR_E_INVAL;
   CK(cudaStreamSynchronize(e->stream));
   CK(cudaMemcpyAsync(out96, e->d.prof, 96 * sizeof(unsigned long long), cudaMemcpyDeviceToHost, e->stream));
   CK(cudaMemsetAsync(e->d.prof, 0, 96 * sizeof(unsigned long long), e->stream));
@@ -1549,7 +1579,7 @@
 #endif
 
 jr_status jr_engine_reset(jr_engine* e) {
-  if (!e) return JR_E_INVAL;
+  if (!enter(e)) return JR_E_INVAL;
   CK(cudaSetDevice(e->cfg.device));
   const Dev& d = e->d;
   const size_t plane = (size_t)d.R * d.Gp;
@@ -1558,6 +1588,7 @@
   CK(cudaMemsetAsync(d.qt, 0, plane * JR_CLIENT_QUEUE_CAP * sizeof(uint4), e->stream));
   CK(cudaMemsetAsync(e->route, 0, (size_t)d.G * sizeof(uint32_t), e->stream));
   CK(cudaMemsetAsync(d.done, 0, (size_t)(d.Gp / GROUPS_PER_CTA) * sizeof(uint32_t), e->stream));
+  CK(cudaMemsetAsync(e->symrec, 0, (size_t)2 * sym_record_alloc_words(d.R) * d.Gp * sizeof(uint32_t), e->stream));
   CK(cudaMemsetAsync(d.scatter, 0, 2 * sizeof(uint32_t), e->stream));
   e->ticket_sum = 0;
   if (e->rp.pnc)
@@ -1612,14 +1643,14 @@
 }
 
 jr_status jr_engine_set_stream(jr_engine* e, void* s) {
-  if (!e) return JR_E_INVAL;
+  if (!enter_keeping_records(e)) return JR_E_INVAL;
   CK(cudaStreamSynchronize(e->stream));
   e->stream = s ? (cudaStream_t)s : e->own_stream;
   return JR_OK;
 }
 
 jr_status jr_engine_sync(jr_engine* e) {
-  if (!e) return JR_E_INVAL;
+  if (!enter_keeping_records(e)) return JR_E_INVAL;
   CK(cudaStreamSynchronize(e->h2d));
   CK(cudaStreamSynchronize(e->stream));
   CK(cudaStreamSynchronize(e->d2h));
@@ -1845,7 +1876,7 @@
 
 
 jr_status jr_step(jr_engine* e, jr_step_args* a) {
-  if (!e || !a) return JR_E_INVAL;
+  if (!enter(e) || !a) return JR_E_INVAL;
   CK(cudaSetDevice(e->cfg.device));
   const Dev& d = e->d;
   const uint32_t R = d.R, G = d.G;
@@ -1977,7 +2008,7 @@
 }
 
 jr_status jr_run(jr_engine* e, uint64_t now0, uint32_t dt, uint32_t n_steps, uint32_t n_synth) {
-  if (!e) return JR_E_INVAL;
+  if (!enter_keeping_records(e)) return JR_E_INVAL;
   if (n_synth > 8) { set_err("n_synth <= 8"); return JR_E_INVAL; }
   CK(cudaSetDevice(e->cfg.device));
   if (n_steps == 0) return JR_OK;
@@ -2037,7 +2068,7 @@
 
 jr_status jr_run_proposals(jr_engine* e, uint64_t now0, uint32_t dt, uint32_t n_steps, const jr_proposal* proposals,
                            uint32_t flags) {
-  if (!e || !proposals) return JR_E_INVAL;
+  if (!enter_keeping_records(e) || !proposals) return JR_E_INVAL;
   if (n_steps == 0) return JR_OK;
   CK(cudaSetDevice(e->cfg.device));
   const uint32_t G = e->d.G, R = e->d.R;
@@ -2056,7 +2087,7 @@
 }
 
 jr_status jr_run_tokens(jr_engine* e, uint64_t now0, uint32_t dt, uint32_t n_steps, const uint64_t* tokens) {
-  if (!e || !tokens) return JR_E_INVAL;
+  if (!enter_keeping_records(e) || !tokens) return JR_E_INVAL;
   if (n_steps == 0) return JR_OK;
   CK(cudaSetDevice(e->cfg.device));
   const uint32_t G = e->d.G;
@@ -2083,7 +2114,7 @@
 }
 
 jr_status jr_run_token_runs(jr_engine* e, uint64_t now0, uint32_t dt, uint32_t n_steps, const jr_token_run* runs) {
-  if (!e || !runs) return JR_E_INVAL;
+  if (!enter_keeping_records(e) || !runs) return JR_E_INVAL;
   if (n_steps == 0) return JR_OK;
   CK(cudaSetDevice(e->cfg.device));
   const uint32_t G = e->d.G;
@@ -2119,7 +2150,7 @@
 }
 
 jr_status jr_drain_fsm(jr_engine* e, jr_fsm_instr* out, size_t cap, size_t* n) {
-  if (!e || !n) return JR_E_INVAL;
+  if (!enter_keeping_records(e) || !n) return JR_E_INVAL;
   CK(cudaSetDevice(e->cfg.device));
   if (!(e->d.flags & JR_F_CAPTURE_FSM)) { *n = 0; return JR_OK; }
   std::vector<jr_fsm_instr> fsm;
@@ -2308,19 +2339,19 @@
 }
 
 jr_status jr_fsm_records_async(jr_engine* e) {
-  if (!e) return JR_E_INVAL;
+  if (!enter_keeping_records(e)) return JR_E_INVAL;
   CK(cudaSetDevice(e->cfg.device));
   return fsm_records_enqueue(e);
 }
 
 jr_status jr_fsm_records_wait(jr_engine* e, const jr_fsm_record** records, jr_fsm_batch* batch) {
-  if (!e) return JR_E_INVAL;
+  if (!enter_keeping_records(e)) return JR_E_INVAL;
   CK(cudaSetDevice(e->cfg.device));
   return fsm_records_take(e, records, batch);
 }
 
 jr_status jr_fsm_responses(jr_engine* e, const jr_fsm_record** responses, jr_fsm_batch* batch) {
-  if (!e) return JR_E_INVAL;
+  if (!enter_keeping_records(e)) return JR_E_INVAL;
   if (!e->resp_cap) { set_err("engine created without JR_F_CLIENT_RESPONSES"); return JR_E_INVAL; }
   int b;
   { std::lock_guard<std::mutex> l(e->qmu); b = e->resp_b; }
@@ -2448,7 +2479,7 @@
 static jr_status many_reserve(jr_engine* e, size_t bytes) { return scratch_reserve(&e->many_buf, &e->many_cap, bytes); }
 
 jr_status jr_query_many(jr_engine* e, const uint32_t* groups, const uint32_t* nodes, size_t n, jr_replica_state* out) {
-  if (!e || !out || !groups || !nodes) return JR_E_INVAL;
+  if (!enter_keeping_records(e) || !out || !groups || !nodes) return JR_E_INVAL;
   if (n == 0) return JR_OK;
   if (n > 0x7fffffffu) return JR_E_INVAL;
   for (size_t i = 0; i < n; ++i)
@@ -2475,7 +2506,7 @@
 
 jr_status jr_chain_read_many(jr_engine* e, const uint32_t* groups, const uint32_t* nodes, const uint64_t* first_id,
                              const uint32_t* count, size_t n, jr_block* out, uint8_t* present) {
-  if (!e || !groups || !nodes || !first_id || !count) return JR_E_INVAL;
+  if (!enter_keeping_records(e) || !groups || !nodes || !first_id || !count) return JR_E_INVAL;
   if (n == 0) return JR_OK;
   if (n > 0x7fffffffu) return JR_E_INVAL;
   std::vector<uint4> reqs(n);
@@ -2512,7 +2543,7 @@
 }
 
 jr_status jr_state_digest(jr_engine* e, uint64_t* out) {
-  if (!e || !out) return JR_E_INVAL;
+  if (!enter_keeping_records(e) || !out) return JR_E_INVAL;
   CK(cudaSetDevice(e->cfg.device));
   const size_t plane = (size_t)e->d.R * e->d.Gp;
   CK(cudaMemsetAsync(e->scratch, 0, 8 * sizeof(unsigned long long), e->stream));
@@ -2535,7 +2566,7 @@
 }
 
 jr_status jr_stream_digest(jr_engine* e, uint64_t* md, uint64_t* fd, uint64_t* nm, uint64_t* nf) {
-  if (!e) return JR_E_INVAL;
+  if (!enter_keeping_records(e)) return JR_E_INVAL;
   if (!(e->d.flags & JR_F_STREAM_DIGEST)) { set_err("engine created without JR_F_STREAM_DIGEST"); return JR_E_INVAL; }
   uint64_t v[5];
   jr_status st = stream_sums(e, v);
@@ -2548,7 +2579,7 @@
 }
 
 jr_status jr_fold_count(jr_engine* e, uint64_t* n) {
-  if (!e || !n) return JR_E_INVAL;
+  if (!enter_keeping_records(e) || !n) return JR_E_INVAL;
   *n = 0;
   if (!e->last_launch_folded) return JR_OK;
   CK(cudaSetDevice(e->cfg.device));
@@ -2560,7 +2591,7 @@
 }
 
 jr_status jr_fault_count(jr_engine* e, uint64_t* n) {
-  if (!e || !n) return JR_E_INVAL;
+  if (!enter_keeping_records(e) || !n) return JR_E_INVAL;
   uint64_t v[5];
   jr_status st = stream_sums(e, v);
   if (st != JR_OK) return st;
@@ -2570,7 +2601,7 @@
 
 
 jr_status jr_compact(jr_engine* e) {
-  if (!e) return JR_E_INVAL;
+  if (!enter(e)) return JR_E_INVAL;
   CK(cudaSetDevice(e->cfg.device));
   const size_t plane = (size_t)e->d.R * e->d.Gp;
   JR_LAUNCH(compact_kernel, (unsigned)((plane + 127) / 128), 128, e->stream, e->d);
@@ -2579,7 +2610,7 @@
 }
 
 jr_status jr_truncate(jr_engine* e, uint32_t margin) {
-  if (!e) return JR_E_INVAL;
+  if (!enter(e)) return JR_E_INVAL;
   CK(cudaSetDevice(e->cfg.device));
   JR_LAUNCH(truncate_kernel, (e->d.Gp + 127) / 128, 128, e->stream, e->d, margin, (const uint8_t*)nullptr);
   CK(cudaGetLastError());
@@ -2602,7 +2633,7 @@
 }
 
 jr_status jr_set_auto_truncate(jr_engine* e, int enabled, uint32_t margin) {
-  if (!e) return JR_E_INVAL;
+  if (!enter_keeping_records(e)) return JR_E_INVAL;
   e->auto_trunc = enabled != 0;
   e->auto_trunc_margin = margin;
   return JR_OK;
@@ -2610,7 +2641,7 @@
 
 jr_status jr_chain_export_many(jr_engine* e, const uint32_t* groups, const uint32_t* nodes, size_t n,
                                jr_persisted_chain* out, jr_block* blocks, size_t cap_blocks, size_t* n_blocks) {
-  if (!e || !n_blocks || (n && (!groups || !nodes || !out))) return JR_E_INVAL;
+  if (!enter_keeping_records(e) || !n_blocks || (n && (!groups || !nodes || !out))) return JR_E_INVAL;
   *n_blocks = 0;
   if (n == 0) return JR_OK;
   if (n > 0x7fffffffu) return JR_E_INVAL;
@@ -2655,7 +2686,7 @@
 
 jr_status jr_node_restart_many(jr_engine* e, uint64_t now_ms, const jr_persisted_chain* chains, size_t n,
                                const jr_block* blocks, size_t n_blocks) {
-  if (!e || (n && !chains) || (n_blocks && !blocks)) return JR_E_INVAL;
+  if (!enter(e) || (n && !chains) || (n_blocks && !blocks)) return JR_E_INVAL;
   if (n == 0) return JR_OK;
   if (n > 0x7fffffffu) return JR_E_INVAL;
   const Dev& d = e->d;
@@ -2719,7 +2750,7 @@
 
 jr_status jr_node_restart(jr_engine* e, uint32_t group, uint32_t node, uint64_t now_ms, const jr_block* blocks,
                           size_t n_blocks, uint64_t commit, int commit_key) {
-  if (!e || group >= e->d.G || node < 1 || node > e->d.R || (n_blocks && !blocks)) return JR_E_INVAL;
+  if (!enter(e) || group >= e->d.G || node < 1 || node > e->d.R || (n_blocks && !blocks)) return JR_E_INVAL;
   if (n_blocks > e->d.cap || commit >= 0xffffffffull) return JR_E_INVAL;
   std::vector<jr_block> v(blocks, blocks + n_blocks);
   std::stable_sort(v.begin(), v.end(), [](const jr_block& a, const jr_block& b) { return a.id < b.id; });
@@ -2738,7 +2769,7 @@
 
 jr_status jr_verify_groups(jr_engine* e, const uint32_t* groups, size_t n_groups, jr_verify_report* report,
                            jr_verify_finding* findings, size_t cap, size_t* n_findings) {
-  if (!e || !report || !n_findings || (n_groups && !groups)) return JR_E_INVAL;
+  if (!enter_keeping_records(e) || !report || !n_findings || (n_groups && !groups)) return JR_E_INVAL;
   const Dev& d = e->d;
   const size_t n = groups ? n_groups : d.G;
   std::vector<uint32_t> list;
@@ -2839,7 +2870,7 @@
 }
 
 jr_status jr_engine_save_size(jr_engine* e, size_t* bytes) {
-  if (!e || !bytes) return JR_E_INVAL;
+  if (!enter_keeping_records(e) || !bytes) return JR_E_INVAL;
   size_t n = sizeof(SaveHeader);
   for (const Segment& sg : save_segments(e)) n += sg.n;
   *bytes = n;
@@ -2847,7 +2878,7 @@
 }
 
 jr_status jr_engine_save(jr_engine* e, void* buf, size_t cap) {
-  if (!e || !buf) return JR_E_INVAL;
+  if (!enter_keeping_records(e) || !buf) return JR_E_INVAL;
   size_t need = 0;
   jr_engine_save_size(e, &need);
   if (cap < need) return JR_E_CAPACITY;
@@ -2872,7 +2903,7 @@
 }
 
 jr_status jr_engine_restore(jr_engine* e, const void* buf, size_t bytes) {
-  if (!e || !buf || bytes < sizeof(SaveHeader)) return JR_E_INVAL;
+  if (!enter(e) || !buf || bytes < sizeof(SaveHeader)) return JR_E_INVAL;
   SaveHeader h;
   memcpy(&h, buf, sizeof h);
   size_t need = 0;
@@ -2900,7 +2931,7 @@
 }
 
 jr_status jr_set_alive(jr_engine* e, uint32_t group, uint32_t node, int alive) {
-  if (!e || group >= e->d.G || node < 1 || node > e->d.R) return JR_E_INVAL;
+  if (!enter(e) || group >= e->d.G || node < 1 || node > e->d.R) return JR_E_INVAL;
   CK(cudaSetDevice(e->cfg.device));
   JR_LAUNCH(set_alive_kernel, 1, 1, e->stream, e->d, group, node - 1, alive);
   CK(cudaGetLastError());
@@ -2908,7 +2939,7 @@
 }
 
 jr_status jr_kill_leaders(jr_engine* e, uint64_t salt, uint32_t permille, uint64_t* n_killed) {
-  if (!e) return JR_E_INVAL;
+  if (!enter(e)) return JR_E_INVAL;
   CK(cudaSetDevice(e->cfg.device));
   CK(cudaMemsetAsync(e->scratch, 0, sizeof(unsigned long long), e->stream));
   JR_LAUNCH(kill_leaders_kernel, (e->d.G + 127) / 128, 128, e->stream, e->d, mix64(e->d.seed ^ salt), permille, e->scratch);
@@ -2921,7 +2952,7 @@
 }
 
 jr_status jr_leader_table_device(jr_engine* e, void* dev_out) {
-  if (!e || !dev_out) return JR_E_INVAL;
+  if (!enter_keeping_records(e) || !dev_out) return JR_E_INVAL;
   CK(cudaSetDevice(e->cfg.device));
   JR_LAUNCH(leader_table_kernel, (e->d.G + 127) / 128, 128, e->stream, e->d, (jr_leader_entry*)dev_out, e->route);
   CK(cudaGetLastError());
@@ -2929,7 +2960,7 @@
 }
 
 jr_status jr_leader_table_async(jr_engine* e, jr_leader_entry* host_out) {
-  if (!e || !host_out) return JR_E_INVAL;
+  if (!enter_keeping_records(e) || !host_out) return JR_E_INVAL;
   const int b = e->tab_i;
   e->tab_i = (b + 1) % jr_engine::NBUF;
   if (e->tab_used[b]) CK(cudaStreamWaitEvent(e->stream, e->tab_free[b], 0));
@@ -2950,7 +2981,7 @@
 }
 
 jr_status jr_leader_table_wait(jr_engine* e) {
-  if (!e) return JR_E_INVAL;
+  if (!enter_keeping_records(e)) return JR_E_INVAL;
   CK(cudaSetDevice(e->cfg.device));
   int b;
   {
diff --git a/josefine_b200/csrc/raft_device.cuh b/josefine_b200/csrc/raft_device.cuh
--- a/josefine_b200/csrc/raft_device.cuh
+++ b/josefine_b200/csrc/raft_device.cuh
@@ -80,6 +80,7 @@
   uint32_t ticket_base = 0;
   const uint8_t* symdone = nullptr;
   const uint8_t* symblk = nullptr;
+  uint32_t carry = 0;
   const uint4* tok_runs = nullptr;
   const uint32_t* tok_route = nullptr;
   uint32_t tok_tick = 0;
diff --git a/josefine_b200/csrc/sym_fold.cuh b/josefine_b200/csrc/sym_fold.cuh
--- a/josefine_b200/csrc/sym_fold.cuh
+++ b/josefine_b200/csrc/sym_fold.cuh
@@ -63,6 +63,7 @@
   uint64_t last_hb;
   uint32_t tbase;
   uint32_t flo;
+  uint32_t fgap;
   uint4* rows;
   uint4* enc;
   uint32_t lcnt, fcnt;
@@ -389,7 +390,10 @@
         d.ctok[row(r, bid)] = tk;
       }
     cache_put(F0, bid, nx, tk);
-    if (bid > fmaxkey) fmaxkey = bid;
+    if (bid > fmaxkey) {
+      if (SPLIT) fgap |= bid - fmaxkey - 1u;
+      fmaxkey = bid;
+    }
     fhead = bid;
     phase(outer);
   }
@@ -439,6 +443,36 @@
   }
 };
 
+constexpr uint32_t SYM_WINDOW = 16;
+
+__device__ __forceinline__ bool sym_launch_ok(const Dev& d, const StepParams& p, uint64_t hbtime, uint32_t maxkey, uint32_t tbase) {
+  const uint64_t hbgap = ((uint64_t)d.hb / p.dt + 1) * p.dt;
+  if ((uint64_t)d.emin <= hbgap || hbtime > p.now) return false;
+  const uint64_t grow = (uint64_t)p.n_ticks * (1u + p.n_synth) + 2u;
+  return (uint64_t)maxkey + grow < (uint64_t)tbase + d.cap && (uint64_t)maxkey + grow < FS_NOTIFY_BIT;
+}
+
+template <int R>
+__device__ __forceinline__ bool sym_timers_ok(const Dev& d, const StepParams& p, uint32_t g, uint32_t L, uint32_t hb, uint64_t hbtime) {
+  uint64_t t_arr = 0;
+  if (!hb) {
+    const uint64_t due = hbtime + (uint64_t)d.hb + 1;
+    t_arr = (due > p.now ? (due - p.now + p.dt - 1) / p.dt : 0) + 1;
+  }
+  const uint64_t checked = t_arr < p.n_ticks ? t_arr : p.n_ticks;
+  if (checked) {
+    const uint64_t t_last = p.now + (checked - 1) * p.dt;
+#pragma unroll
+    for (int r = 0; r < R; ++r) {
+      if ((uint32_t)r == L) continue;
+      const uint4 b = d.p1[(size_t)r * d.Gp + g];
+      const uint64_t etime = (uint64_t)b.x | ((uint64_t)b.y << 32);
+      if (t_last >= etime && t_last - etime > (uint64_t)b.z) return false;
+    }
+  }
+  return true;
+}
+
 template <int R>
 __device__ __forceinline__ bool sym_enter(SymGroup<R, false, true>& s, SymMail& m, const StepParams& p, int prv) {
   const Dev& d = s.d;
@@ -476,7 +510,6 @@
   const uint32_t f0 = s.F0;
   s.fhead = pf.x; s.fcommit = pf.y; s.fckey = (pf.w >> 28) & 1u;
   s.fmaxkey = d.mk[s.rg(f0)];
-  const uint64_t hbgap = ((uint64_t)d.hb / p.dt + 1) * p.dt;
 #pragma unroll
   for (int r = 0; r < R; ++r) {
     if ((uint32_t)r == L) continue;
@@ -485,7 +518,7 @@
     if (p2[r].x != s.fhead || p2[r].y != s.fcommit || ((p2[r].w >> 28) & 1u) != s.fckey) return false;
     if (d.mk[s.rg(r)] != s.fmaxkey) return false;
   }
-  if ((uint64_t)d.emin <= hbgap || s.hbtime > p.now) return false;
+  if (!sym_launch_ok(d, p, s.hbtime, s.maxkey, s.tbase)) return false;
   uint32_t ph[R];
 #pragma unroll
   for (int q = 0; q < (R + 3) / 4; ++q) {
@@ -507,14 +540,11 @@
 #pragma unroll
   for (int r = 0; r < R; ++r)
     if ((uint32_t)r != L && (ph[r] != s.ph_f || ((prmask >> r) & 1u) != s.mode_f)) return false;
-  constexpr uint32_t SYM_WINDOW = 16;
   const uint32_t top = min(s.maxkey, s.fmaxkey);
   const uint32_t lo_min = max(top > SYM_WINDOW - 1u ? top - (SYM_WINDOW - 1u) : 0u, s.tbase);
   if (top < s.tbase || s.ph_f < lo_min || s.fcommit < lo_min || s.commit < lo_min || s.fhead < lo_min || s.fmaxkey > s.maxkey) return false;
   const uint32_t lo = min(min(s.ph_f, s.fcommit), min(s.commit, s.fhead));
   s.flo = lo;
-  const uint64_t grow = (uint64_t)p.n_ticks * (1u + p.n_synth) + 2u;
-  if ((uint64_t)s.maxkey + grow >= (uint64_t)s.tbase + d.cap || (uint64_t)s.maxkey + grow >= FS_NOTIFY_BIT) return false;
   {
     constexpr uint32_t B = 4;
     bool same = true;
@@ -612,23 +642,7 @@
     if (u != cnt) return false;
   }
   }
-  uint64_t t_arr = 0;
-  if (!m.hb) {
-    const uint64_t due = s.hbtime + (uint64_t)d.hb + 1;
-    t_arr = (due > p.now ? (due - p.now + p.dt - 1) / p.dt : 0) + 1;
-  }
-  const uint64_t checked = t_arr < p.n_ticks ? t_arr : p.n_ticks;
-  if (checked) {
-    const uint64_t t_last = p.now + (checked - 1) * p.dt;
-#pragma unroll
-    for (int r = 0; r < R; ++r) {
-      if ((uint32_t)r == L) continue;
-      const uint4 b = d.p1[s.rg(r)];
-      const uint64_t etime = (uint64_t)b.x | ((uint64_t)b.y << 32);
-      if (t_last >= etime && t_last - etime > (uint64_t)b.z) return false;
-    }
-  }
-  return true;
+  return sym_timers_ok<R>(d, p, s.g, L, m.hb, s.hbtime);
 }
 
 enum : uint32_t {
@@ -641,22 +655,78 @@
 __host__ __device__ constexpr uint32_t sr_draws(uint32_t R) { return SR_P2W + (R + 1) / 2; }
 __host__ __device__ constexpr uint32_t sr_idgen(uint32_t R) { return sr_draws(R) + R - 1; }
 __host__ __device__ constexpr uint32_t sym_record_words(uint32_t R) { return sr_idgen(R) + R - 1; }
+__host__ __device__ constexpr uint32_t sr_fflags(uint32_t R) { return sym_record_words(R); }
+__host__ __device__ constexpr uint32_t sr_nhb(uint32_t R) { return sym_record_words(R) + 1; }
+__host__ __device__ constexpr uint32_t sr_tag(uint32_t R) { return sym_record_words(R) + 2; }
+__host__ __device__ constexpr uint32_t sym_record_alloc_words(uint32_t R) { return sym_record_words(R) + 3; }
+
+__host__ __device__ inline bool sym_exit_carries(uint32_t fgap, uint32_t flo_in, uint32_t lo, uint32_t tb, uint32_t commit,
+                                                 uint32_t maxkey, uint32_t phf, uint32_t fcommit, uint32_t fhead, uint32_t fmaxkey) {
+  const uint32_t top = maxkey < fmaxkey ? maxkey : fmaxkey;
+  const uint32_t lo_min0 = top > SYM_WINDOW - 1u ? top - (SYM_WINDOW - 1u) : 0u;
+  const uint32_t lo_min = lo_min0 > tb ? lo_min0 : tb;
+  return fgap == 0 && lo >= flo_in && top >= tb && phf >= lo_min && fcommit >= lo_min && commit >= lo_min &&
+         fhead >= lo_min && fmaxkey <= maxkey;
+}
 
 #ifndef JR_SYM_CHECK_MINCTAS
 #define JR_SYM_CHECK_MINCTAS 5
 #endif
 constexpr uint32_t SYM_CHECK_THREADS = 128;
 template <int R>
-__global__ void __launch_bounds__(SYM_CHECK_THREADS, JR_SYM_CHECK_MINCTAS) sym_check_kernel(const Dev d, const StepParams p, uint32_t* rec) {
+__global__ void __launch_bounds__(SYM_CHECK_THREADS, JR_SYM_CHECK_MINCTAS) sym_check_kernel(const Dev d, const StepParams p, uint32_t* rec,
+                                                                                            const uint32_t* prev) {
   const uint32_t g = blockIdx.x * blockDim.x + threadIdx.x;
   if (g >= d.Gp) return;
   const size_t n = d.Gp;
   uint32_t* w = rec + g;
+  const bool cap = (d.flags & JR_F_CAPTURE_FSM) != 0;
+  const uint32_t tag = w[sr_tag(R) * n];
+  if (tag) w[sr_tag(R) * n] = 0u;
+  if (tag && tag == p.carry && g < d.G) {
+    const uint32_t lf = w[SR_FLAGS * n], ff = w[sr_fflags(R) * n];
+    const uint32_t L = (lf >> 1) & 7u;
+    const uint64_t hbtime = (uint64_t)w[SR_HBTIME * n] | ((uint64_t)w[(SR_HBTIME + 1) * n] << 32);
+    if (!sym_launch_ok(d, p, hbtime, w[SR_MAXKEY * n], w[SR_TBASE * n]) || !sym_timers_ok<R>(d, p, g, L, (lf >> 8) & 1u, hbtime)) {
+      w[SR_FLAGS * n] = 0u;
+      return;
+    }
+    bool share = cap;
+#pragma unroll
+    for (int r = 0; r < R; ++r) {
+      if ((uint32_t)r == L) continue;
+      const uint2 fc = d.fc[(size_t)r * n + g];
+      if (fc.x | fc.y) share = false;
+    }
+    const uint2 fcl = cap ? d.fc[(size_t)L * n + g] : make_uint2(0u, 0u);
+    const uint32_t* a = prev + g;
+    const uint32_t nhb = w[sr_nhb(R) * n];
+    w[SR_TERM * n] = a[SR_TERM * n]; w[(SR_TERM + 1) * n] = a[(SR_TERM + 1) * n];
+    uint32_t prmask = 0;
+#pragma unroll
+    for (int r = 0; r < R; ++r) prmask |= (((uint32_t)r == L ? (lf >> 6) : (lf >> 7)) & 1u) << r;
+#pragma unroll
+    for (int k = 0; k < (R + 1) / 2; ++k) {
+      uint32_t v = a[(SR_P2W + k) * n];
+      if ((uint32_t)k == L / 2) {
+        const uint32_t sh = 16u * (L & 1u);
+        v = (v & ~(0xffffu << sh)) | ((((v >> sh) & 0xef00u) | prmask) << sh);
+      }
+      w[(SR_P2W + k) * n] = v;
+    }
+#pragma unroll
+    for (int k = 0; k < R - 1; ++k) {
+      w[(sr_draws(R) + k) * n] = a[(sr_draws(R) + k) * n] + nhb;
+      w[(sr_idgen(R) + k) * n] = a[(sr_idgen(R) + k) * n];
+    }
+    w[SR_FLAGS * n] = lf | ff | 1u | ((share ? 1u : 0u) << 16);
+    w[SR_FC_L * n] = fcl.x; w[(SR_FC_L + 1) * n] = fcl.y;
+    return;
+  }
   SymGroup<R, false, true> s(d, g);
   SymMail m;
   if (!sym_enter(s, m, p, 1 - p.cur)) { w[SR_FLAGS * n] = 0u; return; }
   const uint32_t L = s.L;
-  const bool cap = (d.flags & JR_F_CAPTURE_FSM) != 0;
   bool share = cap;
   uint32_t hw[(R + 1) / 2];
 #pragma unroll
@@ -831,6 +901,37 @@
       else d.fc[i] = make_uint2(0u, s.fcnt);
     }
   }
+}
+
+template <int R>
+__device__ __forceinline__ void sym_carry_leader(const SymGroup<R, true>& s, const SymMail& last, uint32_t* nxt) {
+  const size_t n = s.d.Gp;
+  uint32_t* w = nxt + s.g;
+  w[SR_FLAGS * n] = (s.L << 1) | (s.ckey << 4) | (s.mode_self << 6) | (s.mode_f << 7) | (last.hb << 8) | (last.ae << 9) | (last.ae_nb << 10);
+  w[SR_HEAD * n] = s.head; w[SR_COMMIT * n] = s.commit; w[SR_IDGEN * n] = s.idgen; w[SR_MAXKEY * n] = s.maxkey;
+  w[SR_PH_SELF * n] = s.ph_self; w[SR_PH_F * n] = s.ph_f;
+  w[SR_HBTIME * n] = (uint32_t)s.hbtime; w[(SR_HBTIME + 1) * n] = (uint32_t)(s.hbtime >> 32);
+  w[SR_HB_COMMIT * n] = last.hb ? last.hb_commit : 0u;
+#pragma unroll
+  for (uint32_t k = 0; k < JR_MAX_AE_BLOCKS; ++k) w[(SR_AE_ID + k) * n] = last.ae_id[k];
+}
+
+template <int R>
+__device__ __forceinline__ void sym_carry_followers(const SymGroup<R, true>& s, const SymMail& last, uint32_t* nxt, uint32_t tb,
+                                                    uint32_t commit, uint32_t maxkey, uint32_t phf, uint32_t epoch) {
+  const size_t n = s.d.Gp;
+  uint32_t* w = nxt + s.g;
+  const uint32_t lo = min(min(phf, s.fcommit), min(commit, s.fhead));
+  if (!sym_exit_carries(s.fgap, s.flo, lo, tb, commit, maxkey, phf, s.fcommit, s.fhead, s.fmaxkey)) {
+    w[sr_tag(R) * n] = 0u;
+    return;
+  }
+  w[SR_TBASE * n] = tb;
+  w[SR_FHEAD * n] = s.fhead; w[SR_FCOMMIT * n] = s.fcommit; w[SR_FMAXKEY * n] = s.fmaxkey; w[SR_FLO * n] = lo;
+  w[SR_HBR_COMMIT * n] = last.hbr ? last.hbr_commit : 0u; w[SR_AR_HEAD * n] = last.ar ? last.ar_head : 0u;
+  w[sr_fflags(R) * n] = (s.fckey << 5) | (last.hbr << 13) | (last.hbr_has << 14) | (last.ar << 15);
+  w[sr_nhb(R) * n] = s.n_hb;
+  w[sr_tag(R) * n] = epoch;
 }
 
 template <int R>
@@ -901,7 +1002,7 @@
 #endif
 template <int R>
 __global__ void __launch_bounds__(2 * SYM2_GROUPS, JR_SYM2_MINCTAS) sym2_kernel(const Dev d, const StepParams p, uint8_t* symdone, uint8_t* symblk,
-                                                                                      const uint32_t* rec) {
+                                                                                      const uint32_t* rec, uint32_t* nxt) {
   JR_DYN_SMEM(uint4, smem);
   auto pair_sync = [] { __syncthreads(); };
   constexpr uint32_t S = SYM2_GROUPS;
@@ -914,6 +1015,7 @@
   s.lcnt = s.fcnt = 0;
   s.n_hb = 0;
   s.last_hb = 0;
+  s.fgap = 0;
   s.share = false;
   s.n_app = 1u + p.n_synth;
   s.rows = smem + gi;
@@ -1012,6 +1114,7 @@
   const uint32_t lastb = cur ^ 1u;
   const uint4 la = mail[(2 * lastb) * S], lc = mail[(4 + lastb) * S];
   const bool ok = !dead && !((la.x | lc.x) & SYM2_ABORT);
+  uint32_t floor = 0;
   if (ok) {
     const int cur_last = p.cur ^ (int)((p.n_ticks - 1) & 1u);
     SymMail last{};
@@ -1020,24 +1123,28 @@
       last.hb_commit = la.y;
       if (last.ae) s.replicate(s.ph_f, s.mode_f, s.maxkey, last);
       sym_leave_leader(s, last, cur_last, rec);
+      if (nxt) sym_carry_leader(s, last, nxt);
     } else {
       last.hbr = lc.x & 1u; last.hbr_has = (lc.x >> 1) & 1u; last.ar = (lc.x >> 2) & 1u;
       last.hbr_commit = lc.y; last.ar_head = lc.z;
       sym_leave_followers(s, last, cur_last, rec);
-    }
+      if (p.trunc) {
+        const uint32_t lo = min(s.fcommit, la.y);
+        if (lo > p.trunc_margin && lo - p.trunc_margin > s.tbase) floor = lo - p.trunc_margin;
+      }
+      if (nxt) sym_carry_followers(s, last, nxt, floor ? floor : s.tbase, la.y, la.z, la.w, p.epoch);
+    }
+  } else if (nxt && !lead && g < d.Gp) {
+    nxt[sr_tag(R) * d.Gp + g] = 0u;
   }
   s.phase(SP_TRUNC);
   if (p.trunc) {
     pair_sync();
-    if (ok && !lead) {
-      const uint32_t lo = min(s.fcommit, la.y);
-      const uint32_t floor = lo > p.trunc_margin ? lo - p.trunc_margin : 0u;
-      if (floor > s.tbase) {
-        for (uint32_t b = s.tbase; b < floor && b - s.tbase < d.cap; ++b)
-#pragma unroll
-          for (int r = 0; r < R; ++r) d.cnext[s.row(r, b)] = ABSENT;
-        d.tb[g] = floor;
-      }
+    if (floor) {
+      for (uint32_t b = s.tbase; b < floor && b - s.tbase < d.cap; ++b)
+#pragma unroll
+        for (int r = 0; r < R; ++r) d.cnext[s.row(r, b)] = ABSENT;
+      d.tb[g] = floor;
     }
   }
   if (lead && g < d.Gp) {
```

Result: faster. 12.77 billion, median of 6 (+7.5%).
